# 1601339895/Image-Restoration

Measured on AMD Instinct MI355X. Metric: Mpixels/sec train (Restormer base 256x256, bs 32/GPU), higher is better.
Workload: dtype bf16; 1 GPU; Restormer base (dim 48, blocks [4,6,6,8], 26.13M params) train step: fwd + L1 + bwd + AdamW, 256x256 patches, bs 32/GPU, bf16 activations, fp32 params/grads/optimizer; per_gpu_batch=32, global_batch=32, patch=256, parallelism=dp1, hip_graph=False

## Files before the change

### image_restoration_amd/_lib.py

```python
from __future__ import annotations

import ctypes as C
import os
from typing import Optional

HERE = os.path.dirname(os.path.abspath(__file__))
LIB_PATH = os.environ.get("MI_RESTORE_LIB") or os.path.join(HERE, "libmi_restore.so")

MI_F32, MI_BF16 = 0, 1
MI_SSIM_TILE = 32
c_i64 = C.c_int64
vp = C.c_void_p
fp = C.c_void_p


class PwDesc(C.Structure):
    _fields_ = [("x1", vp), ("x1_bs", c_i64), ("x1_gs", c_i64), ("k1", C.c_int),
                ("x2", vp), ("x2_bs", c_i64), ("x2_gs", c_i64), ("k2", C.c_int),
                ("w", fp), ("w_bs", c_i64), ("w_gs", c_i64), ("w_sm", c_i64), ("w_sk", c_i64),
                ("bias", fp), ("bias_gs", c_i64),
                ("r", vp), ("r_bs", c_i64), ("r_gs", c_i64),
                ("y", vp), ("y_bs", c_i64), ("y_gs", c_i64),
                ("m", C.c_int), ("n", c_i64), ("batch", C.c_int), ("groups", C.c_int), ("dtype", C.c_int),
                ("ln_w", fp), ("ln_b", fp), ("ln_mean", fp), ("ln_rstd", fp), ("ln_mode", C.c_int),
                ("f8", C.c_int), ("f8_sx", C.c_float), ("f8_sw", C.c_float),
                ("y_split", C.c_int), ("y2", vp), ("y2_bs", c_i64), ("y2_gs", c_i64),
                ("w_b16", vp), ("w_b16_sm", c_i64)]


class GramDesc(C.Structure):
    _fields_ = [("a", vp), ("a_bs", c_i64), ("a_gs", c_i64), ("ma", C.c_int),
                ("b", vp), ("b_bs", c_i64), ("b_gs", c_i64), ("mb", C.c_int),
                ("n", c_i64), ("batch", C.c_int), ("groups", C.c_int), ("dtype", C.c_int),
                ("sum_batch", C.c_int), ("accumulate", C.c_int),
                ("out", fp), ("out_ld", c_i64), ("out_zs", c_i64), ("sumsq", fp)]


class MdtaShape(C.Structure):
    _fields_ = [("B", C.c_int), ("C", C.c_int), ("heads", C.c_int), ("H", C.c_int), ("W", C.c_int),
                ("dtype", C.c_int), ("ks", C.c_int)]


class MdtaParams(C.Structure):
    _fields_ = [("temperature", fp), ("qkv_w", fp), ("qkv_b", fp), ("dw_w", fp), ("dw_b", fp),
                ("proj_w", fp), ("proj_b", fp)]


class MdtaGrads(C.Structure):
    _fields_ = [("temperature", fp), ("qkv_w", fp), ("qkv_b", fp), ("dw_w", fp), ("dw_b", fp),
                ("proj_w", fp), ("proj_b", fp), ("accumulate", C.c_int)]


class XmdtaShape(C.Structure):
    _fields_ = [("B", C.c_int), ("C", C.c_int), ("heads", C.c_int), ("H", C.c_int), ("W", C.c_int),
                ("dtype", C.c_int), ("ks_q", C.c_int), ("ks_kv", C.c_int)]


class XmdtaParams(C.Structure):
    _fields_ = [(n, fp) for n in ("temperature", "q_w", "q_b", "q_dw_w", "q_dw_b", "kv_w", "kv_b", "kv_dw_w", "kv_dw_b",
                                  "proj_w", "proj_b")]


class XmdtaGrads(C.Structure):
    _fields_ = [(n, fp) for n in ("temperature", "q_w", "q_b", "q_dw_w", "q_dw_b", "kv_w", "kv_b", "kv_dw_w", "kv_dw_b",
                                  "proj_w", "proj_b")] + [("accumulate", C.c_int)]


class GdfnShape(C.Structure):
    _fields_ = [("B", C.c_int), ("C", C.c_int), ("hidden", C.c_int), ("H", C.c_int), ("W", C.c_int),
                ("dtype", C.c_int), ("ks", C.c_int), ("flags", C.c_int)]


class GdfnParams(C.Structure):
    _fields_ = [("in_w", fp), ("in_b", fp), ("dw_w", fp), ("dw_b", fp), ("out_w", fp), ("out_b", fp)]


class GdfnFusedShape(C.Structure):
    _fields_ = [("B", C.c_int), ("C", C.c_int), ("hidden", C.c_int), ("H", C.c_int), ("W", C.c_int),
                ("ln_with_bias", C.c_int)]


class LnHead(C.Structure):
    _fields_ = [("w", fp), ("b", fp), ("mean", fp), ("rstd", fp), ("with_bias", C.c_int)]


class F8Scales(C.Structure):
    _fields_ = [("x1", C.c_float), ("w1", C.c_float), ("x2", C.c_float), ("w2", C.c_float)]


class LnTail(C.Structure):
    _fields_ = [("w", fp), ("b", fp), ("mean", fp), ("rstd", fp), ("dres", vp), ("dw", fp), ("db", fp)]


class GroupedProblem(C.Structure):
    _fields_ = [("x", vp), ("x_rs", c_i64), ("w", fp), ("w_sm", c_i64), ("w_sk", c_i64), ("bias", fp), ("r", vp), ("r_rs", c_i64),
                ("y", vp), ("y_rs", c_i64), ("m", C.c_int), ("k", C.c_int), ("expert", C.c_int), ("x_local", C.c_int),
                ("y_local", C.c_int), ("r_local", C.c_int)]


class GdfnGrads(C.Structure):
    _fields_ = [("in_w", fp), ("in_b", fp), ("dw_w", fp), ("dw_b", fp), ("out_w", fp), ("out_b", fp),
                ("accumulate", C.c_int)]


class TksaShape(C.Structure):
    _fields_ = [("B", C.c_int), ("C", C.c_int), ("heads", C.c_int), ("H", C.c_int), ("W", C.c_int), ("dtype", C.c_int),
                ("k1", C.c_int), ("k2", C.c_int), ("k3", C.c_int), ("k4", C.c_int)]


class TksaParams(C.Structure):
    _fields_ = [(n, fp) for n in ("attn1", "attn2", "attn3", "attn4")]


class TksaGrads(C.Structure):
    _fields_ = [(n, fp) for n in ("attn1", "attn2", "attn3", "attn4")]


MSFN_PARAM_NAMES = ("in_w", "in_b", "dw3_w", "dw3_b", "dw5_w", "dw5_b", "g3_w", "g3_b", "g5_w", "g5_b", "out_w", "out_b")


class MsfnShape(C.Structure):
    _fields_ = [("B", C.c_int), ("C", C.c_int), ("hidden", C.c_int), ("H", C.c_int), ("W", C.c_int), ("dtype", C.c_int)]


class MsfnParams(C.Structure):
    _fields_ = [(n, fp) for n in MSFN_PARAM_NAMES]


class MsfnGrads(C.Structure):
    _fields_ = [(n, fp) for n in MSFN_PARAM_NAMES] + [("accumulate", C.c_int)]


class MefcShape(C.Structure):
    _fields_ = [("B", C.c_int), ("C", C.c_int), ("H", C.c_int), ("W", C.c_int), ("dtype", C.c_int), ("steps", C.c_int)]


MEFC_STEP_FIELDS = (("sep_dw1", 4), ("sep_pw1", 4), ("sep_dw2", 4), ("sep_pw2", 4), ("dil_dw", 3), ("dil_pw", 3), ("out_w", 1))


class MefcStepParams(C.Structure):
    _fields_ = [(n, fp * k) if k > 1 else (n, fp) for n, k in MEFC_STEP_FIELDS]


class MefcStepGrads(C.Structure):
    _fields_ = [(n, fp * k) if k > 1 else (n, fp) for n, k in MEFC_STEP_FIELDS]


class MefcParams(C.Structure):
    _fields_ = [(n, fp) for n in ("fc1_w", "fc1_b", "fc2_w", "fc2_b", "pre_w")] + [("step", C.POINTER(MefcStepParams))]


class MefcGrads(C.Structure):
    _fields_ = [(n, fp) for n in ("fc1_w", "fc1_b", "fc2_w", "fc2_b", "pre_w")] + [("step", C.POINTER(MefcStepGrads)),
                                                                                     ("accumulate", C.c_int)]


class DilgateParams(C.Structure):
    _fields_ = [("w", fp * 4), ("b", fp * 4)]


class DilgateGrads(C.Structure):
    _fields_ = [("w", fp * 4), ("b", fp * 4), ("accumulate", C.c_int)]


class DblockShape(C.Structure):
    _fields_ = [("B", C.c_int), ("C", C.c_int), ("H", C.c_int), ("W", C.c_int), ("dtype", C.c_int), ("n_dil", C.c_int),
                ("dil", C.c_int * 4), ("extra", C.c_int)]


DBLOCK_FIELDS = (("norm1_w", 1), ("norm1_b", 1), ("conv1_w", 1), ("conv1_b", 1), ("extra_w", 1), ("extra_b", 1), ("br_w", 4), ("br_b", 4),
                 ("sca_w", 1), ("sca_b", 1), ("conv3_w", 1), ("conv3_b", 1), ("beta", 1), ("norm2_w", 1), ("norm2_b", 1),
                 ("conv4_w", 1), ("conv4_b", 1), ("conv5_w", 1), ("conv5_b", 1), ("gamma", 1))


class DblockParams(C.Structure):
    _fields_ = [(n, fp * k) if k > 1 else (n, fp) for n, k in DBLOCK_FIELDS]


class DblockGrads(C.Structure):
    _fields_ = [(n, fp * k) if k > 1 else (n, fp) for n, k in DBLOCK_FIELDS] + [("accumulate", C.c_int)]


class FremlpShape(C.Structure):
    _fields_ = [("B", C.c_int), ("nc", C.c_int), ("expand", C.c_int), ("H", C.c_int), ("W", C.c_int), ("dtype", C.c_int)]


class FourierUnitShape(C.Structure):
    _fields_ = [("B", C.c_int), ("c", C.c_int), ("groups", C.c_int), ("H", C.c_int), ("W", C.c_int), ("dtype", C.c_int),
                ("training", C.c_int), ("eps", C.c_float), ("momentum", C.c_float)]


FOURIER_UNIT_FIELDS = ("bn_w", "bn_b", "fdc_w", "fdc_b", "gate_w", "gate_b", "fpe_w", "fpe_b")


class FourierUnitParams(C.Structure):
    _fields_ = [(n, fp) for n in FOURIER_UNIT_FIELDS]


class FourierUnitGrads(C.Structure):
    _fields_ = [(n, fp) for n in FOURIER_UNIT_FIELDS] + [("accumulate", C.c_int)]


class SfhFfnShape(C.Structure):
    _fields_ = [("B", C.c_int), ("dim", C.c_int), ("H", C.c_int), ("W", C.c_int), ("dtype", C.c_int)]


SFH_FFN_FIELDS = ("init_w", "init_b", "c1_w", "c1_b", "c2_w", "c2_b", "c3_w", "c3_b", "fina_w", "fina_b")
SFH_LOCAL_FIELDS = ("cd1_w", "cd1_b", "cd2_w", "cd2_b")


class SfhFfnParams(C.Structure):
    _fields_ = [(n, fp) for n in SFH_FFN_FIELDS]


class SfhFfnGrads(C.Structure):
    _fields_ = [(n, fp) for n in SFH_FFN_FIELDS] + [("accumulate", C.c_int)]


class SfhLocalShape(C.Structure):
    _fields_ = SfhFfnShape._fields_


class SfhLocalParams(C.Structure):
    _fields_ = [(n, fp) for n in SFH_LOCAL_FIELDS]


class SfhLocalGrads(C.Structure):
    _fields_ = [(n, fp) for n in SFH_LOCAL_FIELDS] + [("accumulate", C.c_int)]


class SfhMixerShape(C.Structure):
    _fields_ = [("B", C.c_int), ("dim", C.c_int), ("H", C.c_int), ("W", C.c_int), ("dtype", C.c_int), ("training", C.c_int),
                ("eps", C.c_float), ("momentum", C.c_float)]


SFH_GLOBAL_FIELDS = ("init_w", "init_b", "fina_w", "fina_b") + FOURIER_UNIT_FIELDS
SFH_MIXER_FIELDS = SFH_LOCAL_FIELDS + SFH_GLOBAL_FIELDS + ("cac_w", "cac_b", "ca1_w", "ca1_b", "ca2_w", "ca2_b", "conv_w", "conv_b")


class SfhGlobalParams(C.Structure):
    _fields_ = [(n, fp) for n in SFH_GLOBAL_FIELDS]


class SfhGlobalGrads(C.Structure):
    _fields_ = [(n, fp) for n in SFH_GLOBAL_FIELDS] + [("accumulate", C.c_int)]


class SfhMixerParams(C.Structure):
    _fields_ = [(n, fp) for n in SFH_MIXER_FIELDS]


class SfhMixerGrads(C.Structure):
    _fields_ = [(n, fp) for n in SFH_MIXER_FIELDS] + [("accumulate", C.c_int)]


class Bn2dShape(C.Structure):
    _fields_ = [("B", C.c_int), ("C", C.c_int), ("H", C.c_int), ("W", C.c_int), ("dtype", C.c_int), ("training", C.c_int),
                ("eps", C.c_float), ("momentum", C.c_float)]


class EblockShape(C.Structure):
    _fields_ = DblockShape._fields_


EBLOCK_FIELDS = (("norm1_w", 1), ("norm1_b", 1), ("extra_w", 1), ("extra_b", 1), ("conv1_w", 1), ("conv1_b", 1), ("br_w", 4), ("br_b", 4),
                 ("sca_w", 1), ("sca_b", 1), ("conv3_w", 1), ("conv3_b", 1), ("beta", 1), ("norm2_w", 1), ("norm2_b", 1),
                 ("fre_w1", 1), ("fre_b1", 1), ("fre_w2", 1), ("fre_b2", 1), ("gamma", 1))


class EblockParams(C.Structure):
    _fields_ = [(n, fp * k) if k > 1 else (n, fp) for n, k in EBLOCK_FIELDS]


class EblockGrads(C.Structure):
    _fields_ = [(n, fp * k) if k > 1 else (n, fp) for n, k in EBLOCK_FIELDS] + [("accumulate", C.c_int)]


SIGNATURES = {
    "mi_version": (C.c_int, []),
    "mi_last_error": (C.c_char_p, []),
    "mi_env_reload": (C.c_int, []),
    "mi_deferred_begin": (C.c_int, [vp, C.c_size_t]),
    "mi_deferred_record": (C.c_int, [C.c_int]),
    "mi_deferred_pending": (C.c_int, []),
    "mi_deferred_high_water": (C.c_size_t, []),
    "mi_deferred_flush": (C.c_int, [vp]),
    "mi_deferred_end": (C.c_int, []),
    "mi_ln_fwd": (C.c_int, [vp, fp, fp, vp, fp, fp, C.c_int, C.c_int, c_i64, C.c_int, C.c_int, vp]),
    "mi_ln_fwd_eps": (C.c_int, [vp, fp, fp, vp, fp, fp, C.c_int, C.c_int, c_i64, C.c_int, C.c_float, C.c_int, vp]),
    "mi_ln_bwd_workspace": (C.c_size_t, [C.c_int, C.c_int, c_i64]),
    "mi_ln_bwd": (C.c_int, [vp, vp, fp, fp, fp, vp, vp, fp, fp, C.c_int, C.c_int, c_i64, C.c_int, C.c_int, C.c_int,
                            vp, vp]),
    "mi_ln_plan": (C.c_int, [C.c_int, C.c_int, c_i64, C.c_int, C.c_int, C.c_int, C.POINTER(C.c_int)]),
    "mi_dwconv_fwd": (C.c_int, [vp, fp, fp, vp, C.c_int, C.c_int, C.c_int, C.c_int, C.c_int, C.c_int, vp]),
    "mi_dwconv_gate_fwd": (C.c_int, [vp, fp, fp, vp, vp, C.c_int, C.c_int, C.c_int, C.c_int, C.c_int, C.c_int, vp]),
    "mi_dwconv_bwd_workspace": (C.c_size_t, [C.c_int, C.c_int, C.c_int, C.c_int, C.c_int]),
    "mi_dwconv_bwd": (C.c_int, [vp, vp, fp, vp, fp, fp, C.c_int, C.c_int, C.c_int, C.c_int, C.c_int, C.c_int, C.c_int,
                                vp, vp]),
    "mi_dwconv_gate_bwd": (C.c_int, [vp, vp, vp, fp, vp, fp, fp, C.c_int, C.c_int, C.c_int, C.c_int, C.c_int, C.c_int,
                                     C.c_int, vp, vp]),
    "mi_dwconv_gate_recompute_ok": (C.c_int, [C.c_int, C.c_int, C.c_int]),
    "mi_dwconv_plan": (C.c_int, [C.c_int, C.c_int, C.c_int, C.c_int, C.c_int, C.c_int, C.POINTER(C.c_int)]),
    "mi_dwconv_gate_bwd_recompute": (C.c_int, [vp, vp, fp, fp, vp, fp, fp, C.c_int, C.c_int, C.c_int, C.c_int, C.c_int,
                                               C.c_int, C.c_int, vp, vp]),
    "mi_pw_gemm_workspace": (C.c_size_t, [C.POINTER(PwDesc)]),
    "mi_pw_gemm": (C.c_int, [C.POINTER(PwDesc), vp, vp]),
    "mi_pw_cache_enable": (C.c_int, [vp, C.c_size_t, vp, vp]),
    "mi_pw_cache_refresh": (C.c_int, [vp]),
    "mi_pw_cache_invalidate": (C.c_int, []),
    "mi_pw_cache_pending": (C.c_int, []),
    "mi_gram_workspace": (C.c_size_t, [C.POINTER(GramDesc)]),
    "mi_gram": (C.c_int, [C.POINTER(GramDesc), vp, vp]),
    "mi_gram_plan": (C.c_int, [C.POINTER(GramDesc), C.POINTER(c_i64)]),
    "mi_mdta_saved_bytes": (C.c_size_t, [C.POINTER(MdtaShape)]),
    "mi_mdta_workspace": (C.c_size_t, [C.POINTER(MdtaShape)]),
    "mi_mdta_fwd": (C.c_int, [C.POINTER(MdtaShape), C.POINTER(MdtaParams), vp, vp, vp, vp, vp, vp]),
    "mi_mdta_bwd": (C.c_int, [C.POINTER(MdtaShape), C.POINTER(MdtaParams), vp, vp, vp, C.POINTER(MdtaGrads), vp, vp,
                              vp]),
    "mi_xmdta_saved_bytes": (C.c_size_t, [C.POINTER(XmdtaShape)]),
    "mi_xmdta_workspace": (C.c_size_t, [C.POINTER(XmdtaShape)]),
    "mi_xmdta_fwd": (C.c_int, [C.POINTER(XmdtaShape), C.POINTER(XmdtaParams), vp, vp, vp, vp, vp, vp, vp]),
    "mi_xmdta_bwd": (C.c_int, [C.POINTER(XmdtaShape), C.POINTER(XmdtaParams), vp, vp, vp, vp, vp, C.POINTER(XmdtaGrads), vp,
                               vp, vp]),
    "mi_gdfn_saved_bytes": (C.c_size_t, [C.POINTER(GdfnShape)]),
    "mi_gdfn_workspace": (C.c_size_t, [C.POINTER(GdfnShape)]),
    "mi_pw_gemm_ln_ok": (C.c_int, [C.POINTER(PwDesc)]),
    "mi_mdta_fwd_ln_ok": (C.c_int, [C.POINTER(MdtaShape)]),
    "mi_mdta_fwd_ln": (C.c_int, [C.POINTER(MdtaShape), C.POINTER(MdtaParams), C.POINTER(LnHead), vp, vp, vp, vp, vp, vp]),
    "mi_gdfn_fwd_ln_ok": (C.c_int, [C.POINTER(GdfnShape)]),
    "mi_gdfn_fwd_ln": (C.c_int, [C.POINTER(GdfnShape), C.POINTER(GdfnParams), C.POINTER(LnHead), vp, vp, vp, vp, vp, vp]),
    "mi_pw_gemm_f8_ok": (C.c_int, [C.POINTER(PwDesc)]),
    "mi_pw_gemm_split_ok": (C.c_int, [C.POINTER(PwDesc)]),
    "mi_pw_plan": (C.c_int, [C.POINTER(PwDesc), C.POINTER(c_i64)]),
    "mi_mdta_fwd_f8_ok": (C.c_int, [C.POINTER(MdtaShape), C.c_int]),
    "mi_mdta_fwd_f8": (C.c_int, [C.POINTER(MdtaShape), C.POINTER(MdtaParams), C.POINTER(LnHead), C.POINTER(F8Scales), vp, vp, vp,
                                 vp, vp]),
    "mi_gdfn_fwd_f8_ok": (C.c_int, [C.POINTER(GdfnShape), C.c_int]),
    "mi_gdfn_fwd_f8": (C.c_int, [C.POINTER(GdfnShape), C.POINTER(GdfnParams), C.POINTER(LnHead), C.POINTER(F8Scales), vp, vp, vp,
                                 vp, vp]),
    "mi_box_down": (C.c_int, [vp, vp, C.c_int, C.c_int, C.c_int, C.c_int, C.c_int, C.c_int, vp]),
    "mi_fre_rect": (C.c_int, [fp, fp, fp, vp, C.c_int, C.c_int, C.c_int, C.c_int, C.c_int, C.c_int, vp]),
    "mi_fre_split_coef_bytes": (C.c_size_t, [C.c_int, C.c_int]),
    "mi_fre_split_workspace": (C.c_size_t, [C.c_int, C.c_int, C.c_int, C.c_int]),
    "mi_fre_split_max_hw": (C.c_int, []),
    "mi_fre_split_fwd": (C.c_int, [vp, vp, vp, vp, fp, C.c_int, C.c_int, C.c_int, C.c_int, C.c_int, vp]),
    "mi_fre_split_bwd": (C.c_int, [vp, vp, fp, vp, vp, vp, C.c_int, C.c_int, C.c_int, C.c_int, C.c_int, vp, vp]),
    "mi_chan_maxmean_fwd": (C.c_int, [vp, vp, vp, C.c_int, C.c_int, c_i64, C.c_int, vp]),
    "mi_chan_maxmean_bwd": (C.c_int, [vp, vp, vp, C.c_int, C.c_int, c_i64, C.c_int, vp]),
    "mi_plane_max_fwd": (C.c_int, [vp, fp, vp, C.c_int, c_i64, C.c_int, vp]),
    "mi_pool_pair_bwd": (C.c_int, [fp, fp, vp, vp, C.c_int, c_i64, C.c_int, vp]),
    "mi_chan_gate_fwd": (C.c_int, [fp, fp, fp, fp, fp, fp, C.c_int, C.c_int, C.c_int, vp]),
    "mi_chan_gate_bwd": (C.c_int, [fp, fp, fp, fp, fp, fp, fp, fp, fp, fp, fp, C.c_int, C.c_int, C.c_int, C.c_int, vp]),
    "mi_refine_mix_fwd": (C.c_int, [vp, vp, vp, fp, vp, C.c_int, C.c_int, c_i64, C.c_int, vp]),
    "mi_refine_mix_bwd": (C.c_int, [vp, vp, vp, fp, vp, vp, vp, vp, fp, C.c_int, C.c_int, c_i64, C.c_int, vp]),
    "mi_scale_add_fwd": (C.c_int, [vp, vp, fp, fp, vp, C.c_int, C.c_int, c_i64, C.c_int, vp]),
    "mi_scale_add_bwd": (C.c_int, [vp, vp, fp, fp, vp, vp, vp, fp, fp, C.c_int, C.c_int, c_i64, C.c_int, C.c_int, vp]),
    "mi_bwd_tail_ok": (C.c_int, [C.c_int, C.c_int, c_i64, C.c_int]),
    "mi_bwd_tail_workspace": (C.c_size_t, [C.c_int, C.c_int]),
    "mi_bwd_tail_plan": (C.c_int, [C.c_int, C.c_int, C.c_int, c_i64, C.c_int, C.POINTER(c_i64)]),
    "mi_bwd_tail": (C.c_int, [vp, C.c_int, vp, C.c_int, vp, fp, fp, fp, fp, fp, vp, fp, fp, fp, C.c_int, c_i64, C.c_int,
                              C.c_int, vp, vp]),
    "mi_mdta_bwd_ln_ok": (C.c_int, [C.POINTER(MdtaShape), C.c_int]),
    "mi_mdta_bwd_ln_workspace": (C.c_size_t, [C.POINTER(MdtaShape)]),
    "mi_mdta_bwd_ln": (C.c_int, [C.POINTER(MdtaShape), C.POINTER(MdtaParams), C.POINTER(LnTail), vp, vp, vp,
                                 C.POINTER(MdtaGrads), vp, vp, vp]),
    "mi_gdfn_bwd_ln_ok": (C.c_int, [C.POINTER(GdfnShape), C.c_int]),
    "mi_gdfn_bwd_ln_workspace": (C.c_size_t, [C.POINTER(GdfnShape)]),
    "mi_gdfn_bwd_ln": (C.c_int, [C.POINTER(GdfnShape), C.POINTER(GdfnParams), C.POINTER(LnTail), vp, vp, vp,
                                 C.POINTER(GdfnGrads), vp, vp, vp]),
    "mi_gdfn_fwd": (C.c_int, [C.POINTER(GdfnShape), C.POINTER(GdfnParams), vp, vp, vp, vp, vp, vp]),
    "mi_gdfn_bwd": (C.c_int, [C.POINTER(GdfnShape), C.POINTER(GdfnParams), vp, vp, vp, C.POINTER(GdfnGrads), vp, vp,
                              vp]),
    "mi_tksa_saved_bytes": (C.c_size_t, [C.POINTER(TksaShape)]),
    "mi_tksa_workspace": (C.c_size_t, [C.POINTER(TksaShape)]),
    "mi_tksa_fwd": (C.c_int, [C.POINTER(TksaShape), C.POINTER(MdtaParams), C.POINTER(TksaParams), vp, vp, vp, vp, vp, fp, vp]),
    "mi_tksa_bwd": (C.c_int, [C.POINTER(TksaShape), C.POINTER(MdtaParams), C.POINTER(TksaParams), vp, vp, vp, C.POINTER(MdtaGrads),
                              C.POINTER(TksaGrads), vp, vp, vp]),
    "mi_msfn_saved_bytes": (C.c_size_t, [C.POINTER(MsfnShape)]),
    "mi_msfn_workspace": (C.c_size_t, [C.POINTER(MsfnShape)]),
    "mi_msfn_fwd": (C.c_int, [C.POINTER(MsfnShape), C.POINTER(MsfnParams), vp, vp, vp, vp, vp, vp]),
    "mi_msfn_bwd": (C.c_int, [C.POINTER(MsfnShape), C.POINTER(MsfnParams), vp, vp, vp, C.POINTER(MsfnGrads), vp, vp, vp]),
    "mi_mefc_saved_bytes": (C.c_size_t, [C.POINTER(MefcShape)]),
    "mi_mefc_workspace": (C.c_size_t, [C.POINTER(MefcShape)]),
    "mi_mefc_fwd": (C.c_int, [C.POINTER(MefcShape), C.POINTER(MefcParams), vp, vp, vp, vp, vp]),
    "mi_mefc_bwd": (C.c_int, [C.POINTER(MefcShape), C.POINTER(MefcParams), vp, vp, vp, vp, C.POINTER(MefcGrads), vp, vp, vp]),
    "mi_dilgate_plan": (C.c_int, [C.c_int, C.c_int, C.c_int, C.c_int, C.c_int, C.c_int, C.POINTER(C.c_int), C.POINTER(c_i64)]),
    "mi_dilgate_fwd_workspace": (C.c_size_t, [C.c_int, C.c_int, C.c_int, C.c_int]),
    "mi_dilgate_fwd": (C.c_int, [vp, C.POINTER(DilgateParams), vp, fp, C.c_int, C.c_int, C.c_int, C.c_int, C.c_int, C.POINTER(C.c_int),
                                 C.c_int, vp, vp]),
    "mi_dilgate_bwd_workspace": (C.c_size_t, [C.c_int, C.c_int, C.c_int, C.c_int, C.c_int, C.c_int]),
    "mi_dilgate_bwd": (C.c_int, [vp, fp, vp, C.POINTER(DilgateParams), vp, C.POINTER(DilgateGrads), C.c_int, C.c_int, C.c_int, C.c_int,
                                 C.c_int, C.POINTER(C.c_int), C.c_int, vp, vp]),
    "mi_pairconv3x3_fwd": (C.c_int, [vp, fp, fp, vp, C.c_int, C.c_int, C.c_int, C.c_int, C.c_int, vp]),
    "mi_pairconv3x3_bwd_workspace": (C.c_size_t, [C.c_int, C.c_int, C.c_int, C.c_int]),
    "mi_pairconv3x3_bwd": (C.c_int, [vp, vp, fp, vp, fp, fp, C.c_int, C.c_int, C.c_int, C.c_int, C.c_int, C.c_int, vp, vp]),
    "mi_dblock_saved_bytes": (C.c_size_t, [C.POINTER(DblockShape)]),
    "mi_dblock_workspace": (C.c_size_t, [C.POINTER(DblockShape)]),
    "mi_dblock_fwd": (C.c_int, [C.POINTER(DblockShape), C.POINTER(DblockParams), vp, vp, vp, vp, vp]),
    "mi_dblock_bwd": (C.c_int, [C.POINTER(DblockShape), C.POINTER(DblockParams), vp, vp, vp, C.POINTER(DblockGrads), vp, vp, vp]),
    "mi_gdfn_fused_ok": (C.c_int, [C.POINTER(GdfnFusedShape)]),
    "mi_gdfn_fused_pack_bytes": (C.c_size_t, [C.POINTER(GdfnFusedShape)]),
    "mi_gdfn_fused_pack": (C.c_int, [C.POINTER(GdfnFusedShape), fp, fp, C.POINTER(GdfnParams), vp, vp]),
    "mi_gdfn_fused_fwd": (C.c_int, [C.POINTER(GdfnFusedShape), vp, vp, vp, fp, fp, vp]),
    "mi_gdfn_fused_fwd_train_ok": (C.c_int, [C.POINTER(GdfnFusedShape)]),
    "mi_gdfn_fused_fwd_train": (C.c_int, [C.POINTER(GdfnFusedShape), vp, vp, vp, fp, fp, vp, vp]),
    "mi_gdfn_fused_fwd_f8": (C.c_int, [C.POINTER(GdfnFusedShape), vp, C.POINTER(F8Scales), vp, vp, vp]),
    "mi_gdfn_fused_plan": (C.c_int, [C.POINTER(GdfnFusedShape), C.c_int, C.POINTER(c_i64)]),
    "mi_mdta_fused_ok": (C.c_int, [C.POINTER(MdtaShape)]),
    "mi_mdta_fused_pays": (C.c_int, [C.POINTER(MdtaShape)]),
    "mi_mdta_fused_pack_bytes": (C.c_size_t, [C.POINTER(MdtaShape)]),
    "mi_mdta_fused_pack": (C.c_int, [C.POINTER(MdtaShape), fp, fp, C.POINTER(MdtaParams), vp, vp]),
    "mi_mdta_fused_workspace": (C.c_size_t, [C.POINTER(MdtaShape)]),
    "mi_mdta_fused_plan": (C.c_int, [C.POINTER(MdtaShape), C.POINTER(c_i64)]),
    "mi_mdta_fused_fwd": (C.c_int, [C.POINTER(MdtaShape), C.POINTER(MdtaParams), vp, C.c_int, vp, vp, vp, fp, fp, vp, vp]),
    "mi_adamw_step": (C.c_int, [fp, fp, fp, fp, c_i64, C.c_float, C.c_float, C.c_float, C.c_float, C.c_float, C.c_int,
                                C.c_float, fp, vp]),
    "mi_grad_sumsq_workspace": (C.c_size_t, [c_i64]),
    "mi_grad_sumsq": (C.c_int, [fp, c_i64, fp, vp, vp]),
    "mi_adamw_step_ex": (C.c_int, [fp, fp, fp, fp, fp, c_i64, C.c_float, C.c_float, C.c_float, C.c_float, C.c_float, C.c_int,
                                   C.c_float, fp, fp, C.c_float, fp, C.c_float, vp]),
    "mi_rows_gather": (C.c_int, [vp, vp, vp, C.c_int, c_i64, C.c_int, vp]),
    "mi_rows_gather_scaled": (C.c_int, [fp, vp, fp, vp, C.c_int, c_i64, C.c_int, vp]),
    "mi_rows_scatter_add": (C.c_int, [vp, vp, fp, vp, C.c_int, C.c_int, c_i64, C.c_int, C.c_int, vp]),
    "mi_rows_dot_workspace": (C.c_size_t, [C.c_int, c_i64]),
    "mi_rows_dot": (C.c_int, [fp, vp, vp, fp, C.c_int, c_i64, C.c_int, vp, vp]),
    "mi_glue3x3_ok": (C.c_int, [C.c_int, C.c_int]),
    "mi_conv3x3_ok": (C.c_int, [C.c_int, C.c_int, C.c_int]),
    "mi_conv3x3_pack_bytes": (C.c_size_t, [C.c_int, C.c_int]),
    "mi_conv3x3_pack": (C.c_int, [fp, C.c_int, C.c_int, C.c_int, vp, vp]),
    "mi_conv3x3_fwd": (C.c_int, [vp, vp, C.c_int64, fp, vp, C.c_int64, vp, C.c_int64, C.c_int, C.c_int, C.c_int, C.c_int, C.c_int, vp]),
    "mi_conv3x3_wgrad_workspace": (C.c_size_t, [C.c_int, C.c_int, C.c_int, C.c_int, C.c_int]),
    "mi_conv3x3_wgrad": (C.c_int, [vp, C.c_int64, vp, C.c_int64, fp, C.c_int, C.c_int, C.c_int, C.c_int, C.c_int, C.c_int, vp, vp]),
    "mi_conv3x3_plan": (C.c_int, [C.c_int, C.c_int, C.c_int, C.c_int, C.c_int, C.POINTER(c_i64)]),
    "mi_chan_sum_workspace": (C.c_size_t, [C.c_int, C.c_int64]),
    "mi_chan_sum": (C.c_int, [vp, fp, C.c_int, C.c_int, C.c_int64, C.c_int, C.c_int, vp, vp]),
    "mi_chan_sum_plan": (C.c_int, [C.c_int, C.c_int, C.c_int64, C.c_int, C.c_int, C.POINTER(c_i64)]),
    "mi_attn_small_plan": (C.c_int, [C.c_int, C.c_int, C.c_int, C.POINTER(c_i64)]),
    "mi_attn_small_fwd": (C.c_int, [fp, fp, fp, fp, fp, fp, fp, fp, vp, vp, C.c_int, C.c_int, C.c_int, vp]),
    "mi_attn_small_bwd": (C.c_int, [fp, fp, fp, fp, fp, fp, fp, fp, fp, vp, C.c_int, C.c_int, C.c_int, vp]),
    "mi_im2col3x3": (C.c_int, [vp, vp, C.c_int, C.c_int, C.c_int, C.c_int, C.c_int, C.c_int, vp]),
    "mi_col2im3x3": (C.c_int, [vp, fp, vp, vp, C.c_int, C.c_int, C.c_int, C.c_int, C.c_int, C.c_int, vp]),
    "mi_glue3x3_plan": (C.c_int, [c_i64, C.c_int, C.c_int, C.c_int, C.c_int, C.POINTER(c_i64)]),
    "mi_grouped_pw_gemm": (C.c_int, [C.POINTER(GroupedProblem), C.c_int, vp, vp, C.c_int, c_i64, C.c_int, vp]),
    "mi_moe_route_fwd": (C.c_int, [fp, fp, fp, fp, fp, fp, fp, fp, vp, fp, fp, vp, vp, vp, fp, vp, vp, C.c_int, C.c_int, C.c_int,
                                   C.c_int, C.c_int, C.c_int, vp]),
    "mi_moe_route_bwd": (C.c_int, [fp, fp, fp, fp, fp, fp, fp, vp, fp, fp, vp, fp, fp, fp, fp, fp, C.c_int, C.c_int, C.c_int,
                                   C.c_int, C.c_int, C.c_int, vp]),
    "mi_patch_circconv": (C.c_int, [vp, c_i64, vp, c_i64, vp, c_i64, C.c_int, C.c_int, C.c_int, C.c_int, C.c_int, C.c_int, C.c_int, vp]),
    "mi_gelu_gap_fwd": (C.c_int, [vp, fp, C.c_int, C.c_int, c_i64, C.c_int, vp]),
    "mi_gelu_gap_bwd": (C.c_int, [vp, fp, vp, C.c_int, C.c_int, c_i64, C.c_int, vp]),
    "mi_ewise_fwd": (C.c_int, [vp, c_i64, vp, c_i64, vp, c_i64, c_i64, C.c_int, C.c_int, vp]),
    "mi_ewise_bwd": (C.c_int, [vp, c_i64, vp, c_i64, vp, vp, c_i64, vp, c_i64, c_i64, c_i64, C.c_int, C.c_int, vp]),
    "mi_pixel_shuffle2": (C.c_int, [vp, c_i64, vp, c_i64, C.c_int, C.c_int, C.c_int, C.c_int, C.c_int, C.c_int, vp]),
    "mi_copy_rows": (C.c_int, [vp, c_i64, vp, c_i64, c_i64, c_i64, C.c_int, vp]),
    "mi_pixel_shuffle2_plan": (C.c_int, [C.c_int, C.c_int, C.c_int, C.c_int, c_i64, c_i64, C.c_int, C.c_int, C.POINTER(c_i64)]),
    "mi_copy_rows_plan": (C.c_int, [c_i64, c_i64, c_i64, c_i64, C.c_int, C.c_int, C.POINTER(c_i64)]),
    "mi_patch_batch": (C.c_int, [vp, vp, vp, vp, vp, vp, vp, vp, fp, fp, vp, vp, C.c_int, C.c_int, C.c_int, vp]),
    "mi_psnr_ssim_workspace": (C.c_size_t, [C.c_int, C.c_int, C.c_int, C.c_int]),
    "mi_psnr_ssim": (C.c_int, [vp, vp, fp, fp, C.c_int, C.c_int, C.c_int, C.c_int, C.c_int, vp, vp]),
    "mi_gap_fwd": (C.c_int, [vp, fp, C.c_int, C.c_int, c_i64, C.c_int, vp]),
    "mi_gap_bwd": (C.c_int, [fp, vp, C.c_int, C.c_int, c_i64, C.c_int, vp]),
    "mi_cast": (C.c_int, [vp, C.c_int, vp, C.c_int, c_i64, vp]),
    "mi_l1_loss": (C.c_int, [vp, vp, vp, fp, c_i64, C.c_float, C.c_int, vp]),
    "mi_fft_l1_workspace": (C.c_size_t, [C.c_int, C.c_int, C.c_int, C.c_int]),
    "mi_fft_l1_plan": (C.c_int, [C.c_int, C.c_int, C.c_int, C.c_int, C.c_int, C.c_int, C.POINTER(c_i64)]),
    "mi_fft_l1_loss": (C.c_int, [vp, vp, vp, fp, C.c_int, C.c_int, C.c_int, C.c_int, C.c_float, C.c_int, vp, vp]),
# ... 85 lines not shown
```

### image_restoration_amd/csrc/common.h

```cpp
#pragma once
#include <hip/hip_runtime.h>
#include <stdint.h>
#include <stdio.h>
#include <string.h>
#include <type_traits>

#include "../../include/mi_restore.h"

namespace mi {

typedef __bf16 bf16;
typedef unsigned short u16;
typedef __attribute__((ext_vector_type(2))) float f32x2;
typedef __attribute__((ext_vector_type(4))) float f32x4;
typedef __attribute__((ext_vector_type(2))) unsigned int u32x2;
typedef __attribute__((ext_vector_type(4))) unsigned int u32x4;
typedef __attribute__((ext_vector_type(4))) short s16x4;
typedef __attribute__((ext_vector_type(8))) short s16x8;

template <bool F8> struct MfmaOp;
template <> struct MfmaOp<false> {
  using Frag = s16x8;
  static __device__ __forceinline__ void enter() {}
  static __device__ __forceinline__ Frag cvt(const s16x8 v, float) { return v; }
  static __device__ __forceinline__ f32x4 mma(Frag a, Frag b, f32x4 c) { return __builtin_amdgcn_mfma_f32_16x16x32_bf16(a, b, c, 0, 0, 0); }
};
template <> struct MfmaOp<true> {
  using Frag = long;
  typedef short s16x2_t __attribute__((ext_vector_type(2)));
  typedef __bf16 bf16x2_t __attribute__((ext_vector_type(2)));
  static __device__ __forceinline__ void enter() { __builtin_amdgcn_s_setreg((0 << 11) | (23 << 6) | 1, 1); }
  static __device__ __forceinline__ Frag cvt(const s16x8 v, float scale) {
    s16x2_t lo = {0, 0}, hi = {0, 0};
    lo = __builtin_amdgcn_cvt_scalef32_pk_fp8_bf16(lo, __builtin_bit_cast(bf16x2_t, (s16x2_t){v[0], v[1]}), scale, false);
    lo = __builtin_amdgcn_cvt_scalef32_pk_fp8_bf16(lo, __builtin_bit_cast(bf16x2_t, (s16x2_t){v[2], v[3]}), scale, true);
    hi = __builtin_amdgcn_cvt_scalef32_pk_fp8_bf16(hi, __builtin_bit_cast(bf16x2_t, (s16x2_t){v[4], v[5]}), scale, false);
    hi = __builtin_amdgcn_cvt_scalef32_pk_fp8_bf16(hi, __builtin_bit_cast(bf16x2_t, (s16x2_t){v[6], v[7]}), scale, true);
    return (long)(unsigned long)(unsigned)__builtin_bit_cast(int, lo) | ((long)__builtin_bit_cast(int, hi) << 32);
  }
  static __device__ __forceinline__ f32x4 mma(Frag a, Frag b, f32x4 c) { return __builtin_amdgcn_mfma_f32_16x16x32_fp8_fp8(a, b, c, 0, 0, 0); }
};

#define MI_ENV_LIST(X)                                                                                                       \
  X(MI_BT_WIDE) X(MI_BT_DEBUG) X(MI_DW_LDS) X(MI_FG_CFG) X(MI_FG_DEBUG) X(MI_FG_NOXCD) X(MI_GRAM_FOLD) X(MI_GRAM_WANT)      \
  X(MI_GRAM_RECT) X(MI_GRAM_LDS) X(MI_GRAM_STREAM_ALL) X(MI_LN_FORM) X(MI_CO_STREAM) X(MI_ATTN_DQK_SPLIT)    \
  X(MI_PW_DMA) X(MI_PW_TM_EVEN) X(MI_PW_WAVE) X(MI_PW_CHUNKED) X(MI_PW_XWIDE) X(MI_PW_WAVE_WIDE) X(MI_PW_DIRECT)             \
  X(MI_PW_WAVE_TPW) X(MI_PW_XCD) X(MI_PW_TPB) X(MI_PW_B16) X(MI_FM_DEBUG) X(MI_FM_CFG) X(MI_NO_FUSED_MDTA) X(MI_NO_PW_LDS) X(MI_PW_LDS)
enum EnvId {
#define MI_ENV_ENUM(n) E_##n,
  MI_ENV_LIST(MI_ENV_ENUM)
#undef MI_ENV_ENUM
  E_ENV_COUNT
};
const char* env_get(int id);
#define MI_ENV(n) ::mi::env_get(::mi::E_##n)

void set_error(const char* fmt, ...);
#define MI_CHECK_ARG(cond, ...)                \
  do {                                         \
    if (!(cond)) {                             \
      mi::set_error(__VA_ARGS__);              \
      return MI_ERR_ARG;                       \
    }                                          \
  } while (0)
#define MI_CHECK_HIP(expr)                                                          \
  do {                                                                              \
    hipError_t e_ = (expr);                                                         \
    if (e_ != hipSuccess) {                                                         \
      mi::set_error("%s failed: %s (%s:%d)", #expr, hipGetErrorString(e_), __FILE__, __LINE__); \
      return MI_ERR_HIP;                                                            \
    }                                                                               \
  } while (0)
#define MI_LAUNCH_CHECK() MI_CHECK_HIP(hipGetLastError())
#define MI_TRY(expr)          \
  do {                        \
    int rc_ = (expr);         \
    if (rc_ != MI_OK) return rc_; \
  } while (0)

static inline bool aligned16(const void* p) { return (reinterpret_cast<uintptr_t>(p) & 15u) == 0; }
static inline size_t align_up(size_t v, size_t a) { return (v + a - 1) / a * a; }
static inline int cdiv(int64_t a, int64_t b) { return (int)((a + b - 1) / b); }
static inline int cdiv_cap(int64_t a, int64_t b, int cap) { const int64_t n = (a + b - 1) / b; return n < cap ? (int)n : cap; }
static inline size_t dtype_size(int dt) { return dt == MI_BF16 ? 2 : 4; }

template <typename T, typename F> static inline int call_typed(F& f) {
  if constexpr (std::is_void<decltype(f(T{}))>::value) {
    f(T{});
    MI_LAUNCH_CHECK();
    return MI_OK;
  } else {
    return f(T{});
  }
}
template <typename F> static inline int with_dtype(int dtype, const char* who, F&& f) {
  if (dtype == MI_F32) return call_typed<float>(f);
  if (dtype == MI_BF16) return call_typed<bf16>(f);
  set_error("%s: bad dtype %d", who, dtype);
  return MI_ERR_ARG;
}

struct Carver {
  char* base;
  size_t off;
  explicit Carver(void* p) : base(static_cast<char*>(p)), off(0) {}
  template <typename U = void>
  U* take(size_t bytes) {
    size_t o = off;
    off = align_up(off + bytes, 256);
    return base ? reinterpret_cast<U*>(base + o) : nullptr;
  }
};

#if defined(__HIPCC__)

__device__ __forceinline__ float to_f32(float v) { return v; }
__device__ __forceinline__ float to_f32(bf16 v) { return (float)v; }
__device__ __forceinline__ float bf16_bits_to_f32(unsigned int bits16) { return __uint_as_float(bits16 << 16); }

template <typename T> struct Cvt;
template <> struct Cvt<float> {
  static __device__ __forceinline__ float from(float v) { return v; }
};
template <> struct Cvt<bf16> {
  static __device__ __forceinline__ bf16 from(float v) { return (bf16)v; }
};

__device__ __forceinline__ unsigned int cvt_pk_bf16(float a, float b) {
  typedef __bf16 bf16x2_t __attribute__((ext_vector_type(2)));
  const f32x2 v = {a, b};
  return __builtin_bit_cast(unsigned int, __builtin_convertvector(v, bf16x2_t));
}
template <typename T> __device__ __forceinline__ float ld1(const T* p) { return to_f32(*p); }
template <typename T> __device__ __forceinline__ void st1(T* p, float v) { *p = Cvt<T>::from(v); }

#ifndef MI_NT_ST
#define MI_NT_ST 1
#endif
#if MI_NT_ST
#define MI_STREAM_ST(ptr, val) __builtin_nontemporal_store((val), (ptr))
#else
#define MI_STREAM_ST(ptr, val) (*(ptr) = (val))
#endif
#ifndef MI_NT_LD
#define MI_NT_LD 1
#endif
#if MI_NT_LD
#define MI_STREAM_LD(ptr) __builtin_nontemporal_load(ptr)
#define MI_STREAM_DMA_AUX 2
#else
#define MI_STREAM_LD(ptr) (*(ptr))
#define MI_STREAM_DMA_AUX 0
#endif

template <typename T, int V> struct Vec;
template <> struct Vec<float, 1> {
  static __device__ __forceinline__ void ld(const float* p, float* o) { o[0] = p[0]; }
  static __device__ __forceinline__ void st(float* p, const float* v) { p[0] = v[0]; }
};
template <> struct Vec<float, 2> {
  static __device__ __forceinline__ void ld(const float* p, float* o) {
    f32x2 t = *reinterpret_cast<const f32x2*>(p); o[0] = t[0]; o[1] = t[1];
  }
  static __device__ __forceinline__ void st(float* p, const float* v) {
    f32x2 t = {v[0], v[1]}; *reinterpret_cast<f32x2*>(p) = t;
  }
};
template <> struct Vec<float, 4> {
  static __device__ __forceinline__ void ld(const float* p, float* o) {
    f32x4 t = MI_STREAM_LD(reinterpret_cast<const f32x4*>(p)); o[0] = t[0]; o[1] = t[1]; o[2] = t[2]; o[3] = t[3];
  }
  static __device__ __forceinline__ void st(float* p, const float* v) {
    f32x4 t = {v[0], v[1], v[2], v[3]}; MI_STREAM_ST(reinterpret_cast<f32x4*>(p), t);
  }
};
template <> struct Vec<bf16, 1> {
  static __device__ __forceinline__ void ld(const bf16* p, float* o) { o[0] = (float)p[0]; }
  static __device__ __forceinline__ void st(bf16* p, const float* v) { p[0] = (bf16)v[0]; }
};
template <> struct Vec<bf16, 2> {
  static __device__ __forceinline__ void ld(const bf16* p, float* o) {
    unsigned int t = *reinterpret_cast<const unsigned int*>(p);
    o[0] = bf16_bits_to_f32(t & 0xffffu); o[1] = bf16_bits_to_f32(t >> 16);
  }
  static __device__ __forceinline__ void st(bf16* p, const float* v) { *reinterpret_cast<unsigned int*>(p) = cvt_pk_bf16(v[0], v[1]); }
};
template <> struct Vec<bf16, 4> {
  static __device__ __forceinline__ void ld(const bf16* p, float* o) {
    u32x2 t = MI_STREAM_LD(reinterpret_cast<const u32x2*>(p));
    o[0] = bf16_bits_to_f32(t[0] & 0xffffu); o[1] = bf16_bits_to_f32(t[0] >> 16);
    o[2] = bf16_bits_to_f32(t[1] & 0xffffu); o[3] = bf16_bits_to_f32(t[1] >> 16);
  }
  static __device__ __forceinline__ void st(bf16* p, const float* v) {
    u32x2 t;
#pragma unroll
    for (int i = 0; i < 2; ++i) t[i] = cvt_pk_bf16(v[2 * i], v[2 * i + 1]);
    MI_STREAM_ST(reinterpret_cast<u32x2*>(p), t);
  }
};
template <> struct Vec<bf16, 8> {
  static __device__ __forceinline__ void ld(const bf16* p, float* o) {
    u32x4 t = MI_STREAM_LD(reinterpret_cast<const u32x4*>(p));
#pragma unroll
    for (int i = 0; i < 4; ++i) { o[2 * i] = bf16_bits_to_f32(t[i] & 0xffffu); o[2 * i + 1] = bf16_bits_to_f32(t[i] >> 16); }
  }
  static __device__ __forceinline__ void st(bf16* p, const float* v) {
    u32x4 t;
#pragma unroll
    for (int i = 0; i < 4; ++i) t[i] = cvt_pk_bf16(v[2 * i], v[2 * i + 1]);
    MI_STREAM_ST(reinterpret_cast<u32x4*>(p), t);
  }
};

__device__ __forceinline__ float wave_sum(float v) {
#define MI_DPP_ADD(ctrl, rmask)                                                                                   \
  v += __builtin_bit_cast(float, __builtin_amdgcn_update_dpp(0, __builtin_bit_cast(int, v), ctrl, rmask, 0xf, false))
  MI_DPP_ADD(0x111, 0xf);
  MI_DPP_ADD(0x112, 0xf);
  MI_DPP_ADD(0x114, 0xf);
  MI_DPP_ADD(0x118, 0xf);
  MI_DPP_ADD(0x142, 0xa);
  MI_DPP_ADD(0x143, 0xc);
#undef MI_DPP_ADD
  return __builtin_bit_cast(float, __builtin_amdgcn_readlane(__builtin_bit_cast(int, v), 63));
}
__device__ __forceinline__ float wave_max(float v) {
#define MI_DPP_MAX(ctrl, rmask)                                                                                    \
  v = fmaxf(v, __builtin_bit_cast(float, __builtin_amdgcn_update_dpp(__builtin_bit_cast(int, v), __builtin_bit_cast(int, v), \
                                                                     ctrl, rmask, 0xf, false)))
  MI_DPP_MAX(0x111, 0xf);
  MI_DPP_MAX(0x112, 0xf);
  MI_DPP_MAX(0x114, 0xf);
  MI_DPP_MAX(0x118, 0xf);
  MI_DPP_MAX(0x142, 0xa);
  MI_DPP_MAX(0x143, 0xc);
#undef MI_DPP_MAX
  return __builtin_bit_cast(float, __builtin_amdgcn_readlane(__builtin_bit_cast(int, v), 63));
}

#define MI_ROW16_STEP(OP, ctrl)                                                                                    \
  v = OP(v, __builtin_bit_cast(float, __builtin_amdgcn_update_dpp(__builtin_bit_cast(int, v), __builtin_bit_cast(int, v), \
                                                                  ctrl, 0xf, 0xf, true)))
__device__ __forceinline__ float row16_sum(float v) {
#define MI_ADDF(a, b) ((a) + (b))
  MI_ROW16_STEP(MI_ADDF, 0xB1); MI_ROW16_STEP(MI_ADDF, 0x4E); MI_ROW16_STEP(MI_ADDF, 0x141); MI_ROW16_STEP(MI_ADDF, 0x140);
#undef MI_ADDF
  return v;
}
__device__ __forceinline__ float row16_max(float v) {
  MI_ROW16_STEP(fmaxf, 0xB1); MI_ROW16_STEP(fmaxf, 0x4E); MI_ROW16_STEP(fmaxf, 0x141); MI_ROW16_STEP(fmaxf, 0x140);
  return v;
}
#undef MI_ROW16_STEP

__device__ __forceinline__ void gelu_parts(float x, float& cdf, float& pdf) {
  const float z = fabsf(x) * 0.70710678118654752440f;
  const float t = __builtin_amdgcn_rcpf(1.0f + 0.3275911f * z);
  const float e = __expf(-z * z);
  const float poly = t * (0.254829592f + t * (-0.284496736f + t * (1.421413741f + t * (-1.453152027f + t * 1.061405429f))));
  const float q = 0.5f * poly * e;
  cdf = x >= 0.f ? 1.0f - q : q;
  pdf = 0.39894228040143267794f * e;
}
__device__ __forceinline__ void gelu_parts2(f32x2 x, f32x2& cdf, f32x2& pdf) {
#pragma clang fp contract(off)
  const f32x2 ax = {fabsf(x[0]), fabsf(x[1])};
  const f32x2 z = ax * 0.70710678118654752440f;
  const f32x2 den = __builtin_elementwise_fma(z, (f32x2){0.3275911f, 0.3275911f}, (f32x2){1.0f, 1.0f});
  const f32x2 t = {__builtin_amdgcn_rcpf(den[0]), __builtin_amdgcn_rcpf(den[1])};
  const f32x2 a = (z * -z) * 1.44269504088896340736f;
  const f32x2 e = {__builtin_amdgcn_exp2f(a[0]), __builtin_amdgcn_exp2f(a[1])};
  f32x2 p = __builtin_elementwise_fma(t, (f32x2){1.061405429f, 1.061405429f}, (f32x2){-1.453152027f, -1.453152027f});
  p = __builtin_elementwise_fma(t, p, (f32x2){1.421413741f, 1.421413741f});
  p = __builtin_elementwise_fma(t, p, (f32x2){-0.284496736f, -0.284496736f});
  p = __builtin_elementwise_fma(t, p, (f32x2){0.254829592f, 0.254829592f});
  const f32x2 hp = (t * p) * 0.5f;
  const f32x2 q = hp * e;
  const f32x2 omq = __builtin_elementwise_fma(-e, hp, (f32x2){1.0f, 1.0f});
  cdf[0] = x[0] >= 0.f ? omq[0] : q[0];
  cdf[1] = x[1] >= 0.f ? omq[1] : q[1];
  pdf = e * 0.39894228040143267794f;
}
__device__ __forceinline__ float gelu_erf(float x) {
  float cdf, pdf;
  gelu_parts(x, cdf, pdf);
  return x * cdf;
}
template <typename T> __device__ __forceinline__ float gelu_fwd(float x) { return gelu_erf(x); }
#ifndef MI_GELU_EXACT
template <> __device__ __forceinline__ float gelu_fwd<bf16>(float x) {
  const float u = x * (-2.3083120f - 0.1004116f * x * x);
  return x * __builtin_amdgcn_rcpf(1.0f + __builtin_amdgcn_exp2f(u));
}
#endif
__device__ __forceinline__ float gelu_erf_grad(float x) {
  float cdf, pdf;
  gelu_parts(x, cdf, pdf);
  return cdf + x * pdf;
}

#endif

enum KernelId {
  K_LN_FWD = 0, K_LN_BWD, K_DW_FWD, K_DW_GATE_FWD, K_DW_BWD_DATA, K_DW_GATE_BWD_DATA, K_DW_WGRAD, K_PW_GEMM, K_GRAM,
  K_GRAM_REDUCE, K_ATTN_FOLD, K_ATTN_BWD_SMALL, K_REDUCE_ROWS, K_CHAN_SUM, K_ADAMW, K_CAST, K_L1, K_PW_PACK, K_GAP,
  K_IM2COL, K_COL2IM, K_GDFN_FUSED_FWD, K_GDFN_FUSED_BWD, K_MDTA_FUSED_A, K_FUSED_PACK, K_MOE_ROUTE, K_CIRCCONV, K_EWISE, K_CONV3X3, K_GRAM_QK, K_PW_AV, K_BWD_TAIL, K_BWD_TAIL_FIN, K_ADAIR, K_SUMSQ, K_ADAMW_CLIP, K_ADAMW_EMA,
  K_TKSA_ATTN, K_TKSA_FOLD, K_TKSA_BWD, K_TKSA_DWO, K_MSFN_S1, K_MSFN_S2, K_MSFN_S1_BWD, K_MSFN_S2_BWD,
  K_MEFC_STA, K_MEFC_STB, K_MEFC_STA_BWD, K_MEFC_STB_BWD, K_MEFC_WGRAD, K_MEFC_FOLD, K_MEFC_FOLD_BWD, K_MEFC_HEAD, K_MEFC_HEAD_BWD,
  K_MEFC_EW, K_DK_GATE_FWD, K_DK_GATE_BWD_DZ, K_DK_GATE_BWD_DX, K_DK_PAIR, K_DK_PAIR_WGRAD, K_DK_FOLD, K_DK_FOLD_BWD, K_COUNT
};
struct ProfScope {
  hipStream_t st; int kid; bool on;
  ProfScope(hipStream_t stream, int kernel_id, double bytes, double flops);
  ~ProfScope();
};

float* deferred_take(size_t nfloats, hipStream_t st);
bool deferred_owns(const void* p);
bool deferred_reduce_rows(const float* part, float* out, int64_t rows, int64_t cols, int64_t part_ld, int accumulate, float scale,
                          float* out2 = nullptr, int64_t split = 0);

constexpr int REDUCE_GROUPS = 32;
static inline bool reduce_rows_two_stage(int64_t rows) { return rows > 4 * REDUCE_GROUPS; }
int launch_reduce_rows(const float* part, float* out, int64_t rows, int64_t cols, int64_t part_ld,
                       int accumulate, float scale, hipStream_t st, float* tmp = nullptr, float* out2 = nullptr,
                       int64_t split = 0);

}
```

### image_restoration_amd/csrc/internal.h

```cpp
#pragma once
#include <initializer_list>

#include "common.h"

namespace mi {
struct PwK {
  const void* x1; int64_t x1_bs, x1_gs; int k1;
  const void* x2; int64_t x2_bs, x2_gs; int k2;
  const float* w; int64_t w_bs, w_gs, w_sm, w_sk;
  const float* bias; int64_t bias_gs;
  const void* r; int64_t r_bs, r_gs;
  void* y; int64_t y_bs, y_gs;
  int m; int64_t n; int groups; int vec_ok;
  void* y2; int64_t y2_bs, y2_gs; int y_split;
};
enum PwFamily { PW_CHUNKED = 0, PW_RESIDENT, PW_DMA, PW_XRES, PW_STREAM, PW_XWIDE, PW_LDS };
enum PwWeights { PW_W_PACK = 0, PW_W_B16, PW_W_F32 };
struct PwPlan {
  int family;
  int tm, m_tiles, k_chunks;
  bool f8, ln;
  bool vec_ok;
  int slices, per_batch, per_group, chunk_elems;
  int64_t slice_elems;
  size_t bytes;
  size_t lds_image;
  dim3 grid, block; size_t lds;
  int tpw, tpb, n_slabs, slabs_per, xcd_map;
  int weights;
  bool cacheable;
  size_t ws_bytes() const { return family == PW_LDS ? align_up(lds_image, 256) : bytes; }
};
enum GramFamily { GRAM_LDS = 0, GRAM_STREAM };
enum GramFinish { GRAM_DIRECT = 0, GRAM_REDUCE_FEW4, GRAM_REDUCE_FEW16, GRAM_REDUCE };
struct GramPlan {
  int family;
  int fa, fb; bool ss;
  int unit, units, per_split;
  int splits, tiles_a, tiles_b, Z, fold;
  bool vec_ok;
  dim3 grid, block;
  size_t part_bytes, ss_bytes;
  int finish;
  bool deferrable;
  int images, total, zo;
  size_t ws_bytes() const { return part_bytes + ss_bytes; }
};
template <typename... P, typename... A>
static inline int launch_dyn_lds(void (*kernel)(P...), dim3 grid, dim3 block, size_t lds, hipStream_t st, A... args) {
  if (lds > 64 * 1024) MI_CHECK_HIP(hipFuncSetAttribute((const void*)kernel, hipFuncAttributeMaxDynamicSharedMemorySize, (int)lds));
  hipLaunchKernelGGL(kernel, grid, block, lds, st, args...);
  MI_LAUNCH_CHECK();
  return MI_OK;
}
int launch_attn_fold(const float* graw, const float* ss, const float* temperature, const float* wo, float* P, float* A,
                     float* nrm, float* M, int B, int C, int heads, hipStream_t st, void* Mb = nullptr, void* Mtb = nullptr);
int launch_attn_bwd_small(const float* dM, const float* A, const float* P, const float* nrm, const float* temperature,
                          const float* wo, float* dwo_part, float* dtemp_part, float* wd, float* scratch,
                          int B, int C, int heads, hipStream_t st, void* wdb = nullptr);
size_t attn_bwd_scratch_floats(int B, int C, int heads);
struct TopkArgs { const float* w[4]; int k[4]; };
int tksa_check(int C, int heads, const int* k);
int launch_tksa_fold(const float* graw, const float* ss, const float* temperature, const TopkArgs& tk, const float* wo, float* P,
                     float* S, float* A, float* nrm, float* M, float* scores, int B, int C, int heads, hipStream_t st, void* Mb,
                     void* Mtb);
int launch_tksa_bwd(const float* dM, const float* A, const float* S, const float* P, const float* nrm, const float* temperature,
                    const TopkArgs& tk, const float* wo, float* dwo_part, float* dtemp_part, float* dattn_part, float* wd, int B,
                    int C, int heads, hipStream_t st, void* wdb);
int msfn_splits(int H, int W);
size_t msfn_part_floats(int B, int hd, int H, int W);
int launch_msfn_s1_fwd(const void* h0, const float* w3, const float* b3, const float* w5, const float* b5, void* a, void* b, int B,
                       int hd, int H, int W, int dtype, hipStream_t st);
int launch_msfn_s2_fwd(const void* a, const void* b, const float* g3w, const float* g3b, const float* g5w, const float* g5b, void* y,
                       int B, int hd, int H, int W, int dtype, hipStream_t st);
int launch_msfn_s2_bwd(const void* dY, const void* y, const void* a, const void* b, const float* g3w, const float* g5w, void* dza,
                       void* dzb, float* g_g3w, float* g_g3b, float* g_g5w, float* g_g5b, int accumulate, float* part, int B, int hd,
                       int H, int W, int dtype, hipStream_t st);
int launch_msfn_s1_bwd(const void* dza, const void* dzb, const void* h0, const float* w3, const float* w5, void* dh0, float* g_w3,
                       float* g_b3, float* g_w5, float* g_b5, int accumulate, float* part, int B, int hd, int H, int W, int dtype,
                       hipStream_t st);
size_t chan_sum_workspace(int C, int64_t N);
int launch_chan_sum(const void* x, float* out, int B, int C, int64_t N, int dtype, int accumulate, void* ws, hipStream_t st);
#if defined(__HIPCC__)
template <int NV>
__device__ __forceinline__ float block_sum4(const float (&v)[NV], float* red) {
  const int wv = threadIdx.x >> 6, lane = threadIdx.x & 63;
#pragma unroll
  for (int n = 0; n < NV; ++n) {
    const float s = wave_sum(v[n]);
    if (lane == 0) red[wv * NV + n] = s;
  }
  __syncthreads();
  const int n = threadIdx.x;
  return n < NV ? (red[n] + red[NV + n]) + (red[2 * NV + n] + red[3 * NV + n]) : 0.f;
}
#endif

enum { IN_PLAIN = 0, IN_GATE_BWD = 1 };
struct DwArgs {
  const void* in;
  const void* gy;
  const float* w;
  const float* bias;
  void* out;
  void* gate;
  int Cc, H, W, hidden, tiles_x;
};
bool dws_eligible(int H, int W, int ks);
int dws_partial_rows(int B, int H, int W, int64_t planes);
void dws_plan(int H, int W, int64_t planes, int* band, int* nb, int* lpr, int* uni);
int dws_fwd(const DwArgs& a, int B, bool gate, bool flip, int dtype, hipStream_t st);
int dws_bwd(const DwArgs& dya, const void* xin, float* part, int B, bool want_dx, int* rows_out, int dtype, hipStream_t st);
int dws_gate_bwd(const DwArgs& a, const void* xin, float* part, int B, bool want_dw, int* rows_out, int dtype,
                 hipStream_t st);
int dws_gate_bwd_recompute(const DwArgs& a, float* part, int B, bool want_dw, int* rows_out, int dtype, hipStream_t st);
struct BtPlan {
  bool covered, pays;
  int C, NW, MPW, rows, mpad;
  int grid, launch;
  int64_t tiles_per_image, tiles;
  int passes, active;
  size_t lds, ws_bytes;
};
BtPlan bwd_tail_plan(int M, int C, int B, int64_t N, int dtype);
bool bwd_tail_ok(int M, int C, int64_t N, int dtype);
bool bwd_tail_pays(int M, int C);
size_t bwd_tail_workspace(int M, int C);
int launch_bwd_tail(const void* dy, int M, const void* x, int C, const void* dres, const float* mean, const float* rstd,
                    const float* w, const float* gamma, const float* beta, void* dx, float* dw, float* dgamma, float* dbeta,
                    int B, int64_t N, int accumulate, void* ws, hipStream_t st);
#define MI_HIDDEN __attribute__((visibility("hidden")))
MI_HIDDEN int pw_lds_tm(int M);
MI_HIDDEN size_t pw_lds_lds_bytes(int tm);
MI_HIDDEN int pw_lds_launch(const mi_pw_desc* d, const PwPlan& pl, void* ws, hipStream_t st);
int fused_gdfn_fwd_save(const mi_gdfn_fused_shape* s, const void* pack, const void* y, void* out, float* mean, float* rstd,
                        void* h0, void* g, hipStream_t st);
enum FgEntry { FG_INFER = 0, FG_TRAIN, FG_F8 };
enum FgFamily { FG_TILE = 0, FG_FOURTH };
struct FgPlan {
  bool covered;
  int family;
  int C, th, tw, pc, nw; bool save, f8;
  int nch, ngr;
  int tiles_x, tiles_y, S;
  int64_t grid; int block; size_t lds;
  bool xcd_pairs;
  size_t pack_bytes; int pack_pc;
};
MI_HIDDEN FgPlan fg_plan(const mi_gdfn_fused_shape* s, int entry);
enum FmForm { FM_ROUND3 = 0, FM_FOURTH };
struct FmPlan {
  bool covered, pays;
  int kind, form;
  int C, heads, th, nw;
  int tiles_x, tiles_y, S;
  int64_t grid; int block; size_t lds;
  int part_mult;
  size_t part_bytes, ws_bytes, pack_bytes;
};
MI_HIDDEN FmPlan fm_plan(const mi_mdta_shape* s);

static inline size_t fbytes(size_t n) { return align_up(n * sizeof(float), 256); }
static inline size_t tbytes(size_t n, int dt) { return align_up(n * dtype_size(dt), 256); }
static inline size_t max_of(std::initializer_list<size_t> v) {
  size_t m = 0;
  for (size_t x : v) m = x > m ? x : m;
  return m;
}
static inline mi_pw_desc conv1x1(const void* x, int K, const float* w, bool transposed, int w_ld, const float* bias,
                                 const void* res, void* y, int M, int B, int64_t N, int dtype, int64_t x_bs = 0, int64_t y_bs = 0) {
  mi_pw_desc d;
  memset(&d, 0, sizeof(d));
  d.x1 = x; d.x1_bs = x_bs ? x_bs : (int64_t)K * N; d.k1 = K;
  d.w = w;
  if (transposed) { d.w_sm = 1; d.w_sk = w_ld; } else { d.w_sm = w_ld; d.w_sk = 1; }
  d.bias = bias;
  d.r = res; d.r_bs = (int64_t)M * N;
  d.y = y; d.y_bs = y_bs ? y_bs : (int64_t)M * N;
  d.m = M; d.n = N; d.batch = B; d.groups = 1; d.dtype = dtype;
  return d;
}
static inline mi_pw_desc per_image(mi_pw_desc d, const void* w_b16 = nullptr) {
  d.w_bs = (int64_t)d.m * d.k1;
  if (w_b16) { d.w_b16 = w_b16; d.w_b16_sm = d.k1; }
  return d;
}
static inline mi_gram_desc wgrad_gram(const void* dy, int m, const void* x, int k, int B, int64_t N, int dtype, float* out,
                                      int accumulate, int sum_batch = 1, int64_t dy_bs = 0, int64_t x_bs = 0) {
  mi_gram_desc g;
  memset(&g, 0, sizeof(g));
  g.a = dy; g.a_bs = dy_bs ? dy_bs : (int64_t)m * N; g.ma = m;
  g.b = x; g.b_bs = x_bs ? x_bs : (int64_t)k * N; g.mb = k;
  g.n = N; g.batch = B; g.groups = 1; g.dtype = dtype;
  g.sum_batch = sum_batch; g.accumulate = accumulate; g.out = out; g.out_ld = k; g.out_zs = sum_batch ? 0 : (int64_t)m * k;
  return g;
}
static void* const PROBE_PTR = (void*)256;
static inline mi_pw_desc probe1x1(int K, int M, bool transposed, int B, int64_t N, int dtype, int64_t x_bs = 0, int64_t y_bs = 0) {
  return conv1x1(PROBE_PTR, K, (const float*)PROBE_PTR, transposed, transposed ? M : K, nullptr, nullptr, PROBE_PTR, M, B, N, dtype,
                 x_bs, y_bs);
}
static inline mi_gram_desc probe_wgrad(int m, int k, int B, int64_t N, int dtype, int sum_batch = 1, int64_t dy_bs = 0,
                                       int64_t x_bs = 0) {
  return wgrad_gram(PROBE_PTR, m, PROBE_PTR, k, B, N, dtype, (float*)PROBE_PTR, 0, sum_batch, dy_bs, x_bs);
}
static inline size_t pw_ws_bytes(const mi_pw_desc& d) { return mi_pw_gemm_workspace(&d); }
static inline size_t gram_ws_bytes(const mi_gram_desc& d) { return mi_gram_workspace(&d); }
__attribute__((visibility("hidden")))
int conv1x1_bwd_input(const void* dy, int M, const void* x, int K, const float* w, float* dw, float* db, void* dx, int B, int64_t N,
                      int dtype, int accumulate, void* gram_ws, void* cs_ws, void* pw_ws, hipStream_t st, bool fork);
}
```

### image_restoration_amd/csrc/modules.hip

```cpp
#include <stdlib.h>

#include "internal.h"

namespace mi {

struct CoStream {
  hipStream_t side = nullptr;
  hipEvent_t fork = nullptr, join = nullptr;
};
static bool co_stream_enabled() {
  const char* e = MI_ENV(MI_CO_STREAM);
  return e && atoi(e) == 1;
}
static CoStream* co_stream() {
  static thread_local CoStream cs[16];
  int dev = 0;
  if (hipGetDevice(&dev) != hipSuccess || dev < 0 || dev >= 16) return nullptr;
  CoStream& c = cs[dev];
  if (!c.side) {
    if (hipStreamCreateWithFlags(&c.side, hipStreamNonBlocking) != hipSuccess) return nullptr;
    if (hipEventCreateWithFlags(&c.fork, hipEventDisableTiming) != hipSuccess) return nullptr;
    if (hipEventCreateWithFlags(&c.join, hipEventDisableTiming) != hipSuccess) return nullptr;
  }
  return &c;
}
static hipStream_t co_fork(hipStream_t st) {
  if (!co_stream_enabled()) return st;
  CoStream* c = co_stream();
  if (!c) return st;
  if (hipEventRecord(c->fork, st) != hipSuccess || hipStreamWaitEvent(c->side, c->fork, 0) != hipSuccess) return st;
  return c->side;
}
static int co_join(hipStream_t side, hipStream_t st) {
  if (side == st) return MI_OK;
  CoStream* c = co_stream();
  MI_CHECK_ARG(c != nullptr, "co_join: side stream lost");
  MI_CHECK_HIP(hipEventRecord(c->join, side));
  MI_CHECK_HIP(hipStreamWaitEvent(st, c->join, 0));
  return MI_OK;
}
int conv1x1_bwd_input(const void* dy, int M, const void* x, int K, const float* w, float* dw, float* db, void* dx, int B, int64_t N,
                      int dtype, int accumulate, void* gram_ws, void* cs_ws, void* pw_ws, hipStream_t st, bool fork) {
  const mi_gram_desc g = wgrad_gram(dy, M, x, K, B, N, dtype, dw, accumulate);
  const mi_pw_desc d = conv1x1(dy, M, w, true, K, nullptr, nullptr, dx, K, B, N, dtype);
  const hipStream_t sd = fork ? co_fork(st) : st;
  int rc = mi_gram(&g, gram_ws, sd);
  if (rc == MI_OK && db) rc = launch_chan_sum(dy, db, B, M, N, dtype, accumulate, cs_ws, sd);
  if (rc == MI_OK) rc = mi_pw_gemm(&d, pw_ws, st);
  const int joined = co_join(sd, st);
  return rc != MI_OK ? rc : joined;
}
static int conv1x1_bwd_output(const void* dy, int M, const void* x, int K, const float* w, float* dw, float* db, void* dx, int B,
                              int64_t N, int dtype, int accumulate, void* gram_ws, void* cs_ws, void* pw_ws, hipStream_t st) {
  if (db) MI_TRY(launch_chan_sum(dy, db, B, M, N, dtype, accumulate, cs_ws, st));
  const mi_gram_desc g = wgrad_gram(dy, M, x, K, B, N, dtype, dw, accumulate);
  MI_TRY(mi_gram(&g, gram_ws, st));
  const mi_pw_desc d = conv1x1(dy, M, w, true, K, nullptr, nullptr, dx, K, B, N, dtype);
  return mi_pw_gemm(&d, pw_ws, st);
}

struct QkvView { const void* q; int64_t q_bs; const void* k; int64_t k_bs; const void* v; int64_t v_bs; };
struct AttnDims { int B, C, heads, dtype; int64_t N; };
struct AttnSaved { float* A; float* P; float* nrm; float* M; void* Mb; void* Mtb; };
struct AttnScratch {
  float* graw; float* ss; float* dM; float* dwo_part; float* dtemp_part; float* wd; float* attn_scr; void* wdb;
  void* gram_ws; void* pw_ws; void* cs_ws;
};

static void attn_saved_carve(Carver& cv, const AttnDims& d, AttnSaved* r) {
  const size_t C = d.C, B = d.B, c = C / d.heads, Z = B * d.heads;
  r->A = cv.take<float>(fbytes(Z * c * c));
  r->P = cv.take<float>(fbytes(Z * c * c));
  r->nrm = cv.take<float>(fbytes(Z * 2 * c));
  r->M = cv.take<float>(fbytes(B * C * C));
  r->Mb = cv.take(B * C * C * 2);
  r->Mtb = cv.take(B * C * C * 2);
}

static mi_gram_desc attn_qk_gram(const AttnDims& d, const QkvView& v, float* graw, float* ss) {
  const int c = d.C / d.heads;
  mi_gram_desc g;
  memset(&g, 0, sizeof(g));
  g.a = v.q; g.a_bs = v.q_bs; g.a_gs = (int64_t)c * d.N; g.ma = c;
  g.b = v.k; g.b_bs = v.k_bs; g.b_gs = (int64_t)c * d.N; g.mb = c;
  g.n = d.N; g.batch = d.B; g.groups = d.heads; g.dtype = d.dtype;
  g.out = graw; g.out_ld = c; g.out_zs = (int64_t)c * c; g.sumsq = ss;
  return g;
}
static mi_gram_desc attn_dm_gram(const AttnDims& d, const void* dout, const QkvView& v, float* dM) {
  mi_gram_desc g;
  memset(&g, 0, sizeof(g));
  g.a = dout; g.a_bs = (int64_t)d.C * d.N; g.ma = d.C;
  g.b = v.v; g.b_bs = v.v_bs; g.mb = d.C;
  g.n = d.N; g.batch = d.B; g.groups = 1; g.dtype = d.dtype;
  g.out = dM; g.out_ld = d.C; g.out_zs = (int64_t)d.C * d.C;
  return g;
}
static mi_pw_desc attn_dqk_desc(const AttnDims& d, const QkvView& v, const float* w, int row0, int rows, void* y, int64_t y_bs,
                                const void* wb = nullptr) {
  const int c = d.C / d.heads;
  mi_pw_desc dd;
  memset(&dd, 0, sizeof(dd));
  dd.x1 = v.k; dd.x1_bs = v.k_bs; dd.x1_gs = (int64_t)c * d.N; dd.k1 = c;
  dd.x2 = v.q; dd.x2_bs = v.q_bs; dd.x2_gs = (int64_t)c * d.N; dd.k2 = c;
  dd.w = w + (int64_t)row0 * 2 * c; dd.w_bs = (int64_t)d.heads * 2 * c * 2 * c; dd.w_gs = (int64_t)2 * c * 2 * c; dd.w_sm = 2 * c; dd.w_sk = 1;
  if (wb) { dd.w_b16 = (const char*)wb + (int64_t)row0 * 2 * c * 2; dd.w_b16_sm = 2 * c; }
  dd.y = y; dd.y_bs = y_bs; dd.y_gs = (int64_t)c * d.N;
  dd.m = rows; dd.n = d.N; dd.batch = d.B; dd.groups = d.heads; dd.dtype = d.dtype;
  return dd;
}
static mi_pw_desc attn_dqk_merged(const AttnDims& d, const QkvView& v, const float* w, void* dq, int64_t dq_bs, void* dk, int64_t dk_bs,
                                  const void* wb = nullptr) {
  const int c = d.C / d.heads;
  mi_pw_desc dd = attn_dqk_desc(d, v, w, 0, 2 * c, dq, dq_bs, wb);
  dd.y_split = c; dd.y2 = dk; dd.y2_bs = dk_bs; dd.y2_gs = (int64_t)c * d.N;
  return dd;
}

static void attn_scratch_carve(Carver& cv, const AttnDims& d, AttnScratch* w) {
  const size_t C = d.C, B = d.B, c = C / d.heads, Z = B * d.heads;
  w->graw = cv.take<float>(fbytes(Z * c * c));
  w->ss = cv.take<float>(fbytes(Z * 2 * c));
  w->dM = cv.take<float>(fbytes(B * C * C));
  w->dwo_part = cv.take<float>(fbytes(B * C * C));
  w->dtemp_part = cv.take<float>(fbytes(Z));
  w->wd = cv.take<float>(fbytes(Z * 2 * c * 2 * c));
  w->wdb = cv.take(Z * 2 * c * 2 * c * 2);
  w->attn_scr = cv.take<float>(fbytes(attn_bwd_scratch_floats((int)B, (int)C, d.heads)));
  w->gram_ws = nullptr; w->pw_ws = nullptr; w->cs_ws = nullptr;
}
static const QkvView PROBE_QKV{PROBE_PTR, 0, PROBE_PTR, 0, PROBE_PTR, 0};
static size_t attn_gram_ws_bytes(const AttnDims& d) {
  float* const p = (float*)PROBE_PTR;
  return max_of({gram_ws_bytes(attn_qk_gram(d, PROBE_QKV, p, p)), gram_ws_bytes(attn_dm_gram(d, PROBE_PTR, PROBE_QKV, p))});
}
static size_t attn_pw_ws_bytes(const AttnDims& d) {
  const float* const p = (const float*)PROBE_PTR;
  return max_of({pw_ws_bytes(per_image(probe1x1(d.C, d.C, false, d.B, d.N, d.dtype))),
                 pw_ws_bytes(attn_dqk_desc(d, PROBE_QKV, p, 0, d.C / d.heads, PROBE_PTR, 0)),
                 pw_ws_bytes(attn_dqk_merged(d, PROBE_QKV, p, PROBE_PTR, 0, PROBE_PTR, 0))});
}

struct TopkHook { TopkArgs tk; float* S; float* scores; float* dattn_part; float* g_attn[4]; };

static int attn_core_fwd(const AttnDims& d, const QkvView& v, const float* temperature, const float* proj_w,
                         const float* proj_b, const void* residual, void* out, const AttnSaved& sv, const AttnScratch& w,
                         void* stream, const mi_f8_scales* f8 = nullptr, const TopkHook* tk = nullptr) {
  hipStream_t st = (hipStream_t)stream;
  mi_gram_desc g = attn_qk_gram(d, v, w.graw, w.ss);
  MI_TRY(mi_gram(&g, w.gram_ws, stream));
  if (tk)
    MI_TRY(launch_tksa_fold(w.graw, w.ss, temperature, tk->tk, proj_w, sv.P, tk->S, sv.A, sv.nrm, sv.M, tk->scores, d.B, d.C,
                            d.heads, st, sv.Mb, sv.Mtb));
  else
    MI_TRY(launch_attn_fold(w.graw, w.ss, temperature, proj_w, sv.P, sv.A, sv.nrm, sv.M, d.B, d.C, d.heads, st, sv.Mb, sv.Mtb));
  mi_pw_desc d2 = per_image(conv1x1(v.v, d.C, sv.M, false, d.C, proj_b, residual, out, d.C, d.B, d.N, d.dtype, v.v_bs), sv.Mb);
  if (f8) { d2.f8 = 1; d2.f8_sx = f8->x2; d2.f8_sw = f8->w2; }
  return mi_pw_gemm(&d2, w.pw_ws, stream);
}

static int attn_core_bwd(const AttnDims& d, const QkvView& v, const void* dout, void* dq, int64_t dq_bs, void* dk,
                         int64_t dk_bs, void* dv, int64_t dv_bs, const AttnSaved& sv, const float* temperature,
                         const float* proj_w, float* g_temperature, float* g_proj_w, float* g_proj_b, int acc,
                         const AttnScratch& w, void* stream, const TopkHook* tk = nullptr) {
  hipStream_t st = (hipStream_t)stream;
  const int B = d.B, C = d.C, hd = d.heads;
  if (g_proj_b) MI_TRY(launch_chan_sum(dout, g_proj_b, B, C, d.N, d.dtype, acc, w.cs_ws, st));
  mi_gram_desc g1 = attn_dm_gram(d, dout, v, w.dM);
  MI_TRY(mi_gram(&g1, w.gram_ws, stream));
  float* dwo_part = w.dwo_part;
  float* dtemp_part = w.dtemp_part;
  if (acc) {
    float* a1 = deferred_take((size_t)B * C * C, st);
    float* a2 = a1 ? deferred_take((size_t)B * hd, st) : nullptr;
    if (a1 && a2) { dwo_part = a1; dtemp_part = a2; }
  }
  if (tk) {
    MI_TRY(launch_tksa_bwd(w.dM, sv.A, tk->S, sv.P, sv.nrm, temperature, tk->tk, proj_w, dwo_part, dtemp_part, tk->dattn_part, w.wd,
                           B, C, hd, st, w.wdb));
    for (int m = 0; m < 4; ++m)
      MI_TRY(launch_reduce_rows(tk->dattn_part + m, tk->g_attn[m], (int64_t)B * hd, 1, 4, acc, 1.0f, st));
  } else {
    MI_TRY(launch_attn_bwd_small(w.dM, sv.A, sv.P, sv.nrm, temperature, proj_w, dwo_part, dtemp_part, w.wd,
                                 w.attn_scr, B, C, hd, st, w.wdb));
  }
  MI_TRY(launch_reduce_rows(dwo_part, g_proj_w, B, (int64_t)C * C, (int64_t)C * C, acc, 1.0f, st));
  MI_TRY(launch_reduce_rows(dtemp_part, g_temperature, B, hd, hd, acc, 1.0f, st));
  const int c = C / hd;
  mi_pw_desc dd = attn_dqk_merged(d, v, w.wd, dq, dq_bs, dk, dk_bs, w.wdb);
  if (mi_pw_gemm_split_ok(&dd) && !MI_ENV(MI_ATTN_DQK_SPLIT)) {
    MI_TRY(mi_pw_gemm(&dd, w.pw_ws, stream));
  } else {
    dd = attn_dqk_desc(d, v, w.wd, 0, c, dq, dq_bs, w.wdb);
    MI_TRY(mi_pw_gemm(&dd, w.pw_ws, stream));
    dd = attn_dqk_desc(d, v, w.wd, c, c, dk, dk_bs, w.wdb);
    MI_TRY(mi_pw_gemm(&dd, w.pw_ws, stream));
  }
  mi_pw_desc dvd = per_image(conv1x1(dout, C, sv.M, true, C, nullptr, nullptr, dv, C, B, d.N, d.dtype, 0, dv_bs), sv.Mtb);
  return mi_pw_gemm(&dvd, w.pw_ws, stream);
}

struct MdtaSaved { void* qkv0; void* qkv; AttnSaved at; size_t bytes; };
static AttnDims mdta_dims(const mi_mdta_shape* s) { return AttnDims{s->B, s->C, s->heads, s->dtype, (int64_t)s->H * s->W}; }
static MdtaSaved mdta_saved_layout(const mi_mdta_shape* s, void* base) {
  const size_t N = (size_t)s->H * s->W, C = s->C, B = s->B;
  Carver cv(base);
  MdtaSaved r;
  r.qkv0 = cv.take(tbytes(B * 3 * C * N, s->dtype));
  r.qkv = cv.take(tbytes(B * 3 * C * N, s->dtype));
  attn_saved_carve(cv, mdta_dims(s), &r.at);
  r.bytes = cv.off;
  return r;
}
static QkvView mdta_view(const mi_mdta_shape* s, const void* qkv) {
  const int64_t N = (int64_t)s->H * s->W, bs = 3 * (int64_t)s->C * N;
  const size_t es = dtype_size(s->dtype), plane = (size_t)s->C * N * es;
  return QkvView{qkv, bs, (const char*)qkv + plane, bs, (const char*)qkv + 2 * plane, bs};
}

struct MdtaWs { AttnScratch at; MdtaSaved inf; void* dqkv; void* dqkv0; void* dw_ws; size_t bytes; };
static MdtaWs mdta_ws_layout(const mi_mdta_shape* s, void* base) {
  const size_t N = (size_t)s->H * s->W, C = s->C, B = s->B;
  const AttnDims d = mdta_dims(s);
  Carver cv(base);
  MdtaWs w;
  attn_scratch_carve(cv, d, &w.at);
  w.at.gram_ws = cv.take(max_of({attn_gram_ws_bytes(d), gram_ws_bytes(probe_wgrad(3 * d.C, d.C, d.B, d.N, d.dtype))}));
  w.at.pw_ws = cv.take(max_of({pw_ws_bytes(probe1x1(d.C, 3 * d.C, false, d.B, d.N, d.dtype)),
                               pw_ws_bytes(probe1x1(3 * d.C, d.C, true, d.B, d.N, d.dtype)), attn_pw_ws_bytes(d)}));
  w.dw_ws = cv.take(mi_dwconv_bwd_workspace((int)B, 3 * (int)C, s->H, s->W, s->ks));
  w.at.cs_ws = cv.take(chan_sum_workspace(3 * (int)C, (int64_t)N));
  size_t mark = cv.off;
  w.inf = mdta_saved_layout(s, base ? (char*)base + mark : nullptr);
  w.dqkv = base ? (char*)base + mark : nullptr;
  w.dqkv0 = base ? (char*)base + mark + tbytes(B * 3 * C * N, s->dtype) : nullptr;
  size_t bwd_big = 2 * tbytes(B * 3 * C * N, s->dtype);
  w.bytes = mark + max_of({w.inf.bytes, bwd_big});
  return w;
}

static int mdta_check(const mi_mdta_shape* s) {
  MI_CHECK_ARG(s, "mdta: null shape");
  MI_CHECK_ARG(s->B > 0 && s->C > 0 && s->heads > 0 && s->H > 0 && s->W > 0, "mdta: bad shape");
  MI_CHECK_ARG(s->C % s->heads == 0, "mdta: C=%d not divisible by heads=%d", s->C, s->heads);
  MI_CHECK_ARG(s->dtype == MI_F32 || s->dtype == MI_BF16, "mdta: bad dtype %d", s->dtype);
  MI_CHECK_ARG(s->ks == 3 || s->ks == 5 || s->ks == 7, "mdta: bad depthwise kernel size %d", s->ks);
  return MI_OK;
}

struct XmdtaSaved { void* q0; void* q; void* kv0; void* kv; AttnSaved at; size_t bytes; };
static AttnDims xmdta_dims(const mi_xmdta_shape* s) { return AttnDims{s->B, s->C, s->heads, s->dtype, (int64_t)s->H * s->W}; }
static XmdtaSaved xmdta_saved_layout(const mi_xmdta_shape* s, void* base) {
  const size_t N = (size_t)s->H * s->W, C = s->C, B = s->B;
  Carver cv(base);
  XmdtaSaved r;
  r.q0 = cv.take(tbytes(B * C * N, s->dtype));
  r.q = cv.take(tbytes(B * C * N, s->dtype));
  r.kv0 = cv.take(tbytes(B * 2 * C * N, s->dtype));
  r.kv = cv.take(tbytes(B * 2 * C * N, s->dtype));
  attn_saved_carve(cv, xmdta_dims(s), &r.at);
  r.bytes = cv.off;
  return r;
}
static QkvView xmdta_view(const mi_xmdta_shape* s, const void* q, const void* kv) {
  const int64_t N = (int64_t)s->H * s->W;
  const size_t plane = (size_t)s->C * N * dtype_size(s->dtype);
  return QkvView{q, (int64_t)s->C * N, kv, 2 * (int64_t)s->C * N, (const char*)kv + plane, 2 * (int64_t)s->C * N};
}
struct XmdtaWs { AttnScratch at; XmdtaSaved inf; void* dq; void* dq0; void* dkv; void* dkv0; void* dw_ws; size_t bytes; };
static XmdtaWs xmdta_ws_layout(const mi_xmdta_shape* s, void* base) {
  const size_t N = (size_t)s->H * s->W, C = s->C, B = s->B;
  const AttnDims d = xmdta_dims(s);
  Carver cv(base);
  XmdtaWs w;
  attn_scratch_carve(cv, d, &w.at);
  w.at.gram_ws = cv.take(max_of({attn_gram_ws_bytes(d), gram_ws_bytes(probe_wgrad(2 * d.C, d.C, d.B, d.N, d.dtype))}));
  w.at.pw_ws = cv.take(max_of({pw_ws_bytes(probe1x1(d.C, 2 * d.C, false, d.B, d.N, d.dtype)),
                               pw_ws_bytes(probe1x1(2 * d.C, d.C, true, d.B, d.N, d.dtype)), attn_pw_ws_bytes(d)}));
  const int ksm = s->ks_q > s->ks_kv ? s->ks_q : s->ks_kv;
  w.dw_ws = cv.take(mi_dwconv_bwd_workspace((int)B, 2 * (int)C, s->H, s->W, ksm));
  w.at.cs_ws = cv.take(chan_sum_workspace(2 * (int)C, (int64_t)N));
  size_t mark = cv.off;
  w.inf = xmdta_saved_layout(s, base ? (char*)base + mark : nullptr);
  Carver big(base ? (char*)base + mark : nullptr);
  w.dq = big.take(tbytes(B * C * N, s->dtype));
  w.dq0 = big.take(tbytes(B * C * N, s->dtype));
  w.dkv = big.take(tbytes(B * 2 * C * N, s->dtype));
  w.dkv0 = big.take(tbytes(B * 2 * C * N, s->dtype));
  w.bytes = mark + max_of({w.inf.bytes, big.off});
  return w;
}
static int xmdta_check(const mi_xmdta_shape* s) {
  MI_CHECK_ARG(s, "xmdta: null shape");
  MI_CHECK_ARG(s->B > 0 && s->C > 0 && s->heads > 0 && s->H > 0 && s->W > 0, "xmdta: bad shape");
  MI_CHECK_ARG(s->C % s->heads == 0, "xmdta: C=%d not divisible by heads=%d", s->C, s->heads);
  MI_CHECK_ARG(s->dtype == MI_F32 || s->dtype == MI_BF16, "xmdta: bad dtype %d", s->dtype);
  MI_CHECK_ARG((s->ks_q == 3 || s->ks_q == 5 || s->ks_q == 7) && (s->ks_kv == 3 || s->ks_kv == 5 || s->ks_kv == 7),
               "xmdta: bad depthwise kernel sizes %d/%d", s->ks_q, s->ks_kv);
  return MI_OK;
}

struct GdfnSaved { void* h0; void* h1; void* g; size_t bytes; };
static bool gdfn_recompute(const mi_gdfn_shape* s) {
  return !(s->flags & 1) && mi_dwconv_gate_recompute_ok(s->H, s->W, s->ks) != 0;
}
static GdfnSaved gdfn_saved_layout(const mi_gdfn_shape* s, void* base) {
  const size_t N = (size_t)s->H * s->W, B = s->B, h = s->hidden;
  Carver cv(base);
  GdfnSaved r;
  r.h0 = cv.take(tbytes(B * 2 * h * N, s->dtype));
  r.h1 = gdfn_recompute(s) ? nullptr : cv.take(tbytes(B * 2 * h * N, s->dtype));
  r.g = cv.take(tbytes(B * h * N, s->dtype));
  r.bytes = cv.off;
  return r;
}
struct GdfnWs { void* gram_ws; void* pw_ws; void* dw_ws; void* cs_ws; GdfnSaved inf; void* dg; void* dh0; size_t bytes; };
static GdfnWs gdfn_ws_layout(const mi_gdfn_shape* s, void* base) {
  const int B = s->B, C = s->C, h = s->hidden, dt = s->dtype;
  const int64_t N = (int64_t)s->H * s->W;
  Carver cv(base);
  GdfnWs w;
  w.gram_ws = cv.take(max_of({gram_ws_bytes(probe_wgrad(C, h, B, N, dt)), gram_ws_bytes(probe_wgrad(2 * h, C, B, N, dt))}));
  w.pw_ws = cv.take(max_of({pw_ws_bytes(probe1x1(C, 2 * h, false, B, N, dt)), pw_ws_bytes(probe1x1(2 * h, C, true, B, N, dt))}));
  w.dw_ws = cv.take(mi_dwconv_bwd_workspace(B, 2 * h, s->H, s->W, s->ks));
  w.cs_ws = cv.take(chan_sum_workspace(2 * h > C ? 2 * h : C, N));
  size_t mark = cv.off;
  w.inf = gdfn_saved_layout(s, base ? (char*)base + mark : nullptr);
  w.dg = base ? (char*)base + mark : nullptr;
  w.dh0 = base ? (char*)base + mark + tbytes((size_t)B * h * N, dt) : nullptr;
  size_t bwd_big = tbytes((size_t)B * h * N, dt) + tbytes((size_t)B * 2 * h * N, dt);
  w.bytes = mark + max_of({w.inf.bytes, bwd_big});
  return w;
}
static int gdfn_check(const mi_gdfn_shape* s) {
  MI_CHECK_ARG(s, "gdfn: null shape");
  MI_CHECK_ARG(s->B > 0 && s->C > 0 && s->hidden > 0 && s->H > 0 && s->W > 0, "gdfn: bad shape");
  MI_CHECK_ARG(s->dtype == MI_F32 || s->dtype == MI_BF16, "gdfn: bad dtype %d", s->dtype);
  MI_CHECK_ARG(s->ks == 3 || s->ks == 5 || s->ks == 7, "gdfn: bad depthwise kernel size %d", s->ks);
  return MI_OK;
}

static mi_mdta_shape tksa_mdta_shape(const mi_tksa_shape* s) { return mi_mdta_shape{s->B, s->C, s->heads, s->H, s->W, s->dtype, 3}; }
static int tksa_shape_check(const mi_tksa_shape* s) {
  MI_CHECK_ARG(s, "tksa: null shape");
  const mi_mdta_shape m = tksa_mdta_shape(s);
  MI_TRY(mdta_check(&m));
  const int k[4] = {s->k1, s->k2, s->k3, s->k4};
  return tksa_check(s->C, s->heads, k);
}
static size_t tksa_scores_bytes(const mi_mdta_shape* s) {
  const size_t c = s->C / s->heads;
  return fbytes((size_t)s->B * s->heads * c * c);
}
struct TksaWs { float* S_inf; float* dattn_part; size_t bytes; };
static TksaWs tksa_ws_tail(const mi_mdta_shape* s, size_t m_bytes, void* base) {
  Carver cv(base ? (char*)base + align_up(m_bytes, 256) : nullptr);
  TksaWs w;
  w.S_inf = cv.take<float>(tksa_scores_bytes(s));
  w.dattn_part = cv.take<float>(fbytes((size_t)s->B * s->heads * 4));
  w.bytes = align_up(m_bytes, 256) + cv.off;
  return w;
}

}

using namespace mi;

extern "C" size_t mi_mdta_saved_bytes(const mi_mdta_shape* s) {
  if (mdta_check(s) != MI_OK) return 0;
  return mdta_saved_layout(s, nullptr).bytes;
}
extern "C" size_t mi_mdta_workspace(const mi_mdta_shape* s) {
  if (mdta_check(s) != MI_OK) return 0;
  return mdta_ws_layout(s, nullptr).bytes;
}

static void ln_head_apply(mi_pw_desc* d, const mi_ln_head* ln) {
  if (!ln) return;
  d->ln_w = ln->w; d->ln_b = ln->with_bias ? ln->b : nullptr; d->ln_mean = ln->mean; d->ln_rstd = ln->rstd;
  d->ln_mode = ln->with_bias ? 1 : 2;
}
static int ln_head_check(const mi_ln_head* ln, const char* who) {
  MI_CHECK_ARG(ln && ln->w && (!ln->with_bias || ln->b) && ((ln->mean == nullptr) == (ln->rstd == nullptr)),
               "%s: LayerNorm head needs w (and b for WithBias); mean / rstd both or neither", who);
  return MI_OK;
}
static int mdta_fwd_impl(const char* who, const mi_mdta_shape* s, const mi_mdta_params* p, const void* x, const void* residual,
                         void* out, void* saved, void* ws, void* stream, const mi_ln_head* ln, const mi_f8_scales* f8 = nullptr,
                         const TopkHook* topk = nullptr) {
  MI_TRY(mdta_check(s));
  MI_CHECK_ARG(p && x && out && ws, "%s: null pointer", who);
  MI_CHECK_ARG(p->temperature && p->qkv_w && p->dw_w && p->proj_w, "%s: null parameter", who);
  const int B = s->B, C = s->C, dt = s->dtype;
  const int64_t N = (int64_t)s->H * s->W;
  MdtaWs w = mdta_ws_layout(s, ws);
  MdtaSaved sv = saved ? mdta_saved_layout(s, saved) : w.inf;
  TopkHook hk;
  if (topk) {
    hk = *topk;
    hk.S = saved ? (float*)((char*)saved + sv.bytes) : tksa_ws_tail(s, w.bytes, ws).S_inf;
    topk = &hk;
  }
  mi_pw_desc d1 = conv1x1(x, C, p->qkv_w, false, C, p->qkv_b, nullptr, sv.qkv0, 3 * C, B, N, dt);
  ln_head_apply(&d1, ln);
  if (f8) { d1.f8 = 1; d1.f8_sx = f8->x1; d1.f8_sw = f8->w1; }
  MI_TRY(mi_pw_gemm(&d1, w.at.pw_ws, stream));
  MI_TRY(mi_dwconv_fwd(sv.qkv0, p->dw_w, p->dw_b, sv.qkv, B, 3 * C, s->H, s->W, s->ks, dt, stream));
  return attn_core_fwd(mdta_dims(s), mdta_view(s, sv.qkv), p->temperature, p->proj_w, p->proj_b, residual, out, sv.at, w.at,
                       stream, f8, topk);
}
extern "C" int mi_mdta_fwd(const mi_mdta_shape* s, const mi_mdta_params* p, const void* x, const void* residual, void* out,
                           void* saved, void* ws, void* stream) {
  return mdta_fwd_impl("mdta_fwd", s, p, x, residual, out, saved, ws, stream, nullptr);
}
extern "C" int mi_mdta_fwd_ln_ok(const mi_mdta_shape* s) {
  if (mdta_check(s) != MI_OK) return 0;
  const mi_pw_desc d = probe1x1(s->C, 3 * s->C, false, s->B, (int64_t)s->H * s->W, s->dtype);
  return mi_pw_gemm_ln_ok(&d);
}
extern "C" int mi_mdta_fwd_ln(const mi_mdta_shape* s, const mi_mdta_params* p, const mi_ln_head* ln, const void* x,
                              const void* residual, void* out, void* saved, void* ws, void* stream) {
  MI_TRY(ln_head_check(ln, "mdta_fwd_ln"));
  MI_CHECK_ARG(mi_mdta_fwd_ln_ok(s), "mdta_fwd_ln: shape not covered (bf16, C <= 128, H*W %% 64 == 0)");
  return mdta_fwd_impl("mdta_fwd", s, p, x, residual, out, saved, ws, stream, ln);
}

static int f8_check(const mi_f8_scales* f, const char* who) {
  MI_CHECK_ARG(f && f->x1 > 0.f && f->w1 > 0.f && f->x2 > 0.f && f->w2 > 0.f, "%s: fp8 scales must be positive", who);
  return MI_OK;
}
extern "C" int mi_mdta_fwd_f8_ok(const mi_mdta_shape* s, int with_ln) {
  if (mdta_check(s) != MI_OK || s->dtype != MI_BF16) return 0;
  const int64_t N = (int64_t)s->H * s->W;
  const mi_pw_desc d1 = probe1x1(s->C, 3 * s->C, false, s->B, N, s->dtype);
  const mi_pw_desc d2 = per_image(probe1x1(s->C, s->C, false, s->B, N, s->dtype, 3 * (int64_t)s->C * N));
  if (with_ln && !mi_pw_gemm_ln_ok(&d1)) return 0;
  return mi_pw_gemm_f8_ok(&d1) && mi_pw_gemm_f8_ok(&d2);
}
extern "C" int mi_mdta_fwd_f8(const mi_mdta_shape* s, const mi_mdta_params* p, const mi_ln_head* ln, const mi_f8_scales* f8,
                              const void* x, const void* residual, void* out, void* ws, void* stream) {
  MI_TRY(f8_check(f8, "mdta_fwd_f8"));
  if (ln) MI_TRY(ln_head_check(ln, "mdta_fwd_f8"));
  MI_CHECK_ARG(mi_mdta_fwd_f8_ok(s, ln != nullptr), "mdta_fwd_f8: shape not covered (bf16, both projections on a wave-owned form)");
  return mdta_fwd_impl("mdta_fwd", s, p, x, residual, out, nullptr, ws, stream, ln, f8);
}

static int mdta_bwd_impl(const char* who, const mi_mdta_shape* s, const mi_mdta_params* p, const void* x, const void* dout,
                         void* dx, const mi_mdta_grads* gr, const void* saved, void* ws, void* stream, const mi_ln_tail* ln,
                         const TopkHook* topk = nullptr) {
  MI_TRY(mdta_check(s));
  MI_CHECK_ARG(p && x && dout && dx && gr && saved && ws, "%s: null pointer", who);
  MI_CHECK_ARG(gr->temperature && gr->qkv_w && gr->dw_w && gr->proj_w, "%s: null gradient buffer", who);
  hipStream_t st = (hipStream_t)stream;
  const int B = s->B, C = s->C, dt = s->dtype, acc = gr->accumulate;
  const int64_t N = (int64_t)s->H * s->W, bs = 3 * (int64_t)C * N;
  const size_t plane = (size_t)C * N * dtype_size(dt);
  MdtaWs w = mdta_ws_layout(s, ws);
  MdtaSaved sv = mdta_saved_layout(s, const_cast<void*>(saved));
  TopkHook hk;
  if (topk) {
    hk = *topk;
    hk.S = (float*)((char*)const_cast<void*>(saved) + sv.bytes);
    hk.dattn_part = tksa_ws_tail(s, w.bytes, ws).dattn_part;
    topk = &hk;
  }
  char* dq = (char*)w.dqkv;
  MI_TRY(attn_core_bwd(mdta_dims(s), mdta_view(s, sv.qkv), dout, dq, bs, dq + plane, bs, dq + 2 * plane, bs, sv.at,
                       p->temperature, p->proj_w, gr->temperature, gr->proj_w, gr->proj_b, acc, w.at, stream, topk));
  MI_TRY(mi_dwconv_bwd(w.dqkv, sv.qkv0, p->dw_w, w.dqkv0, gr->dw_w, gr->dw_b, B, 3 * C, s->H, s->W, s->ks, acc, dt, w.dw_ws,
                       stream));
  if (ln)
    return launch_bwd_tail(w.dqkv0, 3 * C, x, C, ln->dres, ln->mean, ln->rstd, p->qkv_w, ln->w, ln->b, dx, gr->qkv_w, ln->dw,
                           ln->db, B, N, acc, (char*)ws + align_up(w.bytes, 256), st);
  return conv1x1_bwd_input(w.dqkv0, 3 * C, x, C, p->qkv_w, gr->qkv_w, gr->qkv_b, dx, B, N, dt, acc, w.at.gram_ws, w.at.cs_ws,
                           w.at.pw_ws, st, true);
// ... 100 lines not shown
  MI_TRY(mi_dwconv_gate_fwd(sv.h0, p->dw_w, p->dw_b, (saved && !gdfn_recompute(s)) ? sv.h1 : nullptr, sv.g, B, 2 * h, s->H,
                            s->W, s->ks, dt, stream));
  mi_pw_desc d2 = conv1x1(sv.g, h, p->out_w, false, h, p->out_b, residual, out, C, B, N, dt);
  if (f8) { d2.f8 = 1; d2.f8_sx = f8->x2; d2.f8_sw = f8->w2; }
  MI_TRY(mi_pw_gemm(&d2, w.pw_ws, stream));
  return MI_OK;
}
extern "C" int mi_gdfn_fwd(const mi_gdfn_shape* s, const mi_gdfn_params* p, const void* x, const void* residual, void* out,
                           void* saved, void* ws, void* stream) {
  return gdfn_fwd_impl(s, p, x, residual, out, saved, ws, stream, nullptr);
}
extern "C" int mi_gdfn_fwd_ln_ok(const mi_gdfn_shape* s) {
  if (gdfn_check(s) != MI_OK) return 0;
  const mi_pw_desc d = probe1x1(s->C, 2 * s->hidden, false, s->B, (int64_t)s->H * s->W, s->dtype);
  return mi_pw_gemm_ln_ok(&d);
}
extern "C" int mi_gdfn_fwd_ln(const mi_gdfn_shape* s, const mi_gdfn_params* p, const mi_ln_head* ln, const void* x,
                              const void* residual, void* out, void* saved, void* ws, void* stream) {
  MI_TRY(ln_head_check(ln, "gdfn_fwd_ln"));
  MI_CHECK_ARG(mi_gdfn_fwd_ln_ok(s), "gdfn_fwd_ln: shape not covered (bf16, C <= 128, H*W %% 64 == 0)");
  return gdfn_fwd_impl(s, p, x, residual, out, saved, ws, stream, ln);
}

extern "C" int mi_gdfn_fwd_f8_ok(const mi_gdfn_shape* s, int with_ln) {
  if (gdfn_check(s) != MI_OK || s->dtype != MI_BF16) return 0;
  const int64_t N = (int64_t)s->H * s->W;
  const mi_pw_desc d1 = probe1x1(s->C, 2 * s->hidden, false, s->B, N, s->dtype);
  const mi_pw_desc d2 = probe1x1(s->hidden, s->C, false, s->B, N, s->dtype);
  if (with_ln && !mi_pw_gemm_ln_ok(&d1)) return 0;
  return mi_pw_gemm_f8_ok(&d1) && mi_pw_gemm_f8_ok(&d2);
}
extern "C" int mi_gdfn_fwd_f8(const mi_gdfn_shape* s, const mi_gdfn_params* p, const mi_ln_head* ln, const mi_f8_scales* f8,
                              const void* x, const void* residual, void* out, void* ws, void* stream) {
  MI_TRY(f8_check(f8, "gdfn_fwd_f8"));
  if (ln) MI_TRY(ln_head_check(ln, "gdfn_fwd_f8"));
  MI_CHECK_ARG(mi_gdfn_fwd_f8_ok(s, ln != nullptr), "gdfn_fwd_f8: shape not covered (bf16, both projections on a wave-owned form)");
  return gdfn_fwd_impl(s, p, x, residual, out, nullptr, ws, stream, ln, f8);
}

extern "C" int mi_gdfn_fused_fwd_train_ok(const mi_gdfn_fused_shape* f) {
  return fg_plan(f, FG_TRAIN).covered ? 1 : 0;
}
extern "C" int mi_gdfn_fused_fwd_train(const mi_gdfn_fused_shape* f, const void* pack, const void* y, void* out, float* mean,
                                       float* rstd, void* saved, void* stream) {
  MI_CHECK_ARG(mi_gdfn_fused_fwd_train_ok(f), "gdfn_fused_fwd_train: shape not covered (mi_gdfn_fused_fwd_train_ok)");
  MI_CHECK_ARG(saved, "gdfn_fused_fwd_train: null saved blob");
  mi_gdfn_shape s = {f->B, f->C, f->hidden, f->H, f->W, MI_BF16, 3, 0};
  GdfnSaved sv = gdfn_saved_layout(&s, saved);
  return fused_gdfn_fwd_save(f, pack, y, out, mean, rstd, sv.h0, sv.g, (hipStream_t)stream);
}

static int gdfn_bwd_impl(const mi_gdfn_shape* s, const mi_gdfn_params* p, const void* x, const void* dout, void* dx,
                         const mi_gdfn_grads* gr, const void* saved, void* ws, void* stream, const mi_ln_tail* ln) {
  MI_TRY(gdfn_check(s));
  MI_CHECK_ARG(p && x && dout && dx && gr && saved && ws, "gdfn_bwd: null pointer");
  MI_CHECK_ARG(gr->in_w && gr->dw_w && gr->out_w, "gdfn_bwd: null gradient buffer");
  hipStream_t st = (hipStream_t)stream;
  const int B = s->B, C = s->C, h = s->hidden, dt = s->dtype, acc = gr->accumulate;
  const int64_t N = (int64_t)s->H * s->W;
  GdfnWs w = gdfn_ws_layout(s, ws);
  GdfnSaved sv = gdfn_saved_layout(s, const_cast<void*>(saved));
  MI_TRY(conv1x1_bwd_output(dout, C, sv.g, h, p->out_w, gr->out_w, gr->out_b, w.dg, B, N, dt, acc, w.gram_ws, w.cs_ws, w.pw_ws, st));
  if (gdfn_recompute(s))
    MI_TRY(mi_dwconv_gate_bwd_recompute(w.dg, sv.h0, p->dw_w, p->dw_b, w.dh0, gr->dw_w, gr->dw_b, B, 2 * h, s->H, s->W, s->ks,
                                        acc, dt, w.dw_ws, stream));
  else
    MI_TRY(mi_dwconv_gate_bwd(w.dg, sv.h1, sv.h0, p->dw_w, w.dh0, gr->dw_w, gr->dw_b, B, 2 * h, s->H, s->W, s->ks, acc, dt,
                              w.dw_ws, stream));
  if (ln)
    return launch_bwd_tail(w.dh0, 2 * h, x, C, ln->dres, ln->mean, ln->rstd, p->in_w, ln->w, ln->b, dx, gr->in_w, ln->dw, ln->db,
                           B, N, acc, (char*)ws + align_up(w.bytes, 256), st);
  return conv1x1_bwd_input(w.dh0, 2 * h, x, C, p->in_w, gr->in_w, gr->in_b, dx, B, N, dt, acc, w.gram_ws, w.cs_ws, w.pw_ws, st, true);
}
extern "C" int mi_gdfn_bwd(const mi_gdfn_shape* s, const mi_gdfn_params* p, const void* x, const void* dout, void* dx,
                           const mi_gdfn_grads* gr, const void* saved, void* ws, void* stream) {
  return gdfn_bwd_impl(s, p, x, dout, dx, gr, saved, ws, stream, nullptr);
}
extern "C" int mi_gdfn_bwd_ln_ok(const mi_gdfn_shape* s, int in_bias) {
  if (gdfn_check(s) != MI_OK || in_bias) return 0;
  return bwd_tail_ok(2 * s->hidden, s->C, (int64_t)s->H * s->W, s->dtype) && bwd_tail_pays(2 * s->hidden, s->C) ? 1 : 0;
}
extern "C" size_t mi_gdfn_bwd_ln_workspace(const mi_gdfn_shape* s) {
  if (!mi_gdfn_bwd_ln_ok(s, 0)) return 0;
  return align_up(gdfn_ws_layout(s, nullptr).bytes, 256) + bwd_tail_workspace(2 * s->hidden, s->C);
}
extern "C" int mi_gdfn_bwd_ln(const mi_gdfn_shape* s, const mi_gdfn_params* p, const mi_ln_tail* ln, const void* x,
                              const void* dout, void* dx, const mi_gdfn_grads* gr, const void* saved, void* ws, void* stream) {
  MI_TRY(ln_tail_check(ln, "gdfn_bwd_ln"));
  MI_CHECK_ARG(gr && !gr->in_b && mi_gdfn_bwd_ln_ok(s, 0), "gdfn_bwd_ln: shape not covered (bf16, C 48/96, H*W %% 64 == 0, no project_in bias)");
  return gdfn_bwd_impl(s, p, x, dout, dx, gr, saved, ws, stream, ln);
}

static TopkHook tksa_hook(const mi_tksa_shape* s, const mi_tksa_params* tp, float* scores, const mi_tksa_grads* tg) {
  TopkHook hk;
  memset(&hk, 0, sizeof(hk));
  hk.tk.w[0] = tp->attn1; hk.tk.w[1] = tp->attn2; hk.tk.w[2] = tp->attn3; hk.tk.w[3] = tp->attn4;
  hk.tk.k[0] = s->k1; hk.tk.k[1] = s->k2; hk.tk.k[2] = s->k3; hk.tk.k[3] = s->k4;
  hk.scores = scores;
  if (tg) { hk.g_attn[0] = tg->attn1; hk.g_attn[1] = tg->attn2; hk.g_attn[2] = tg->attn3; hk.g_attn[3] = tg->attn4; }
  return hk;
}

extern "C" size_t mi_tksa_saved_bytes(const mi_tksa_shape* s) {
  if (tksa_shape_check(s) != MI_OK) return 0;
  const mi_mdta_shape ms = tksa_mdta_shape(s);
  return mdta_saved_layout(&ms, nullptr).bytes + tksa_scores_bytes(&ms);
}
extern "C" size_t mi_tksa_workspace(const mi_tksa_shape* s) {
  if (tksa_shape_check(s) != MI_OK) return 0;
  const mi_mdta_shape ms = tksa_mdta_shape(s);
  return tksa_ws_tail(&ms, mdta_ws_layout(&ms, nullptr).bytes, nullptr).bytes;
}

extern "C" int mi_tksa_fwd(const mi_tksa_shape* s, const mi_mdta_params* p, const mi_tksa_params* tp, const void* x,
                           const void* residual, void* out, void* saved, void* ws, float* scores, void* stream) {
  MI_TRY(tksa_shape_check(s));
  MI_CHECK_ARG(tp, "tksa_fwd: null pointer");
  MI_CHECK_ARG(tp->attn1 && tp->attn2 && tp->attn3 && tp->attn4, "tksa_fwd: null attn1..4");
  const mi_mdta_shape ms = tksa_mdta_shape(s);
  const TopkHook hk = tksa_hook(s, tp, scores, nullptr);
  return mdta_fwd_impl("tksa_fwd", &ms, p, x, residual, out, saved, ws, stream, nullptr, nullptr, &hk);
}

extern "C" int mi_tksa_bwd(const mi_tksa_shape* s, const mi_mdta_params* p, const mi_tksa_params* tp, const void* x,
                           const void* dout, void* dx, const mi_mdta_grads* gr, const mi_tksa_grads* tg, const void* saved, void* ws,
                           void* stream) {
  MI_TRY(tksa_shape_check(s));
  MI_CHECK_ARG(tp && tg, "tksa_bwd: null pointer");
  MI_CHECK_ARG(tp->attn1 && tp->attn2 && tp->attn3 && tp->attn4, "tksa_bwd: null attn1..4");
  MI_CHECK_ARG(tg->attn1 && tg->attn2 && tg->attn3 && tg->attn4, "tksa_bwd: null attn1..4 gradient buffer");
  const mi_mdta_shape ms = tksa_mdta_shape(s);
  const TopkHook hk = tksa_hook(s, tp, nullptr, tg);
  return mdta_bwd_impl("tksa_bwd", &ms, p, x, dout, dx, gr, saved, ws, stream, nullptr, &hk);
}

struct MsfnSaved { void* h0; void* a; void* b; void* y; size_t bytes; };
static MsfnSaved msfn_saved_layout(const mi_msfn_shape* s, void* base) {
  const size_t n = (size_t)s->B * 2 * s->hidden * s->H * s->W;
  Carver cv(base);
  MsfnSaved r;
  r.h0 = cv.take(tbytes(n, s->dtype));
  r.a = cv.take(tbytes(n, s->dtype));
  r.b = cv.take(tbytes(n, s->dtype));
  r.y = cv.take(tbytes(n, s->dtype));
  r.bytes = cv.off;
  return r;
}
struct MsfnWs { void* gram_ws; void* pw_ws; void* cs_ws; float* part; MsfnSaved inf; void* dY; void* dza; void* dzb; size_t bytes; };
static MsfnWs msfn_ws_layout(const mi_msfn_shape* s, void* base) {
  const int B = s->B, C = s->C, h2 = 2 * s->hidden, dt = s->dtype;
  const int64_t N = (int64_t)s->H * s->W;
  Carver cv(base);
  MsfnWs w;
  w.gram_ws = cv.take(max_of({gram_ws_bytes(probe_wgrad(C, h2, B, N, dt)), gram_ws_bytes(probe_wgrad(h2, C, B, N, dt))}));
  w.pw_ws = cv.take(max_of({pw_ws_bytes(probe1x1(C, h2, false, B, N, dt)), pw_ws_bytes(probe1x1(h2, C, false, B, N, dt)),
                            pw_ws_bytes(probe1x1(C, h2, true, B, N, dt)), pw_ws_bytes(probe1x1(h2, C, true, B, N, dt))}));
  w.cs_ws = cv.take(chan_sum_workspace(h2 > C ? h2 : C, N));
  w.part = cv.take<float>(fbytes(msfn_part_floats(B, s->hidden, s->H, s->W)));
  const size_t mark = cv.off;
  w.inf = msfn_saved_layout(s, base ? (char*)base + mark : nullptr);
  Carver big(base ? (char*)base + mark : nullptr);
  const size_t plane = tbytes((size_t)B * h2 * N, dt);
  w.dY = big.take(plane);
  w.dza = big.take(plane);
  w.dzb = big.take(plane);
  w.bytes = mark + max_of({w.inf.bytes, big.off});
  return w;
}
static int msfn_check(const mi_msfn_shape* s) {
  MI_CHECK_ARG(s, "msfn: null shape");
  MI_CHECK_ARG(s->B > 0 && s->C > 0 && s->hidden > 0 && s->H > 0 && s->W > 0, "msfn: bad shape");
  MI_CHECK_ARG(2 * s->hidden <= 65535, "msfn: hidden=%d too large (2*hidden <= 65535)", s->hidden);
  MI_CHECK_ARG(s->dtype == MI_F32 || s->dtype == MI_BF16, "msfn: bad dtype %d", s->dtype);
  return MI_OK;
}

extern "C" size_t mi_msfn_saved_bytes(const mi_msfn_shape* s) {
  if (msfn_check(s) != MI_OK) return 0;
  return msfn_saved_layout(s, nullptr).bytes;
}
extern "C" size_t mi_msfn_workspace(const mi_msfn_shape* s) {
  if (msfn_check(s) != MI_OK) return 0;
  return msfn_ws_layout(s, nullptr).bytes;
}

extern "C" int mi_msfn_fwd(const mi_msfn_shape* s, const mi_msfn_params* p, const void* x, const void* residual, void* out,
                           void* saved, void* ws, void* stream) {
  MI_TRY(msfn_check(s));
  MI_CHECK_ARG(p && x && out && ws, "msfn_fwd: null pointer");
  MI_CHECK_ARG(p->in_w && p->dw3_w && p->dw5_w && p->g3_w && p->g5_w && p->out_w, "msfn_fwd: null parameter");
  hipStream_t st = (hipStream_t)stream;
  const int B = s->B, C = s->C, hd = s->hidden, dt = s->dtype;
  const int64_t N = (int64_t)s->H * s->W;
  MsfnWs w = msfn_ws_layout(s, ws);
  MsfnSaved sv = saved ? msfn_saved_layout(s, saved) : w.inf;
  mi_pw_desc d1 = conv1x1(x, C, p->in_w, false, C, p->in_b, nullptr, sv.h0, 2 * hd, B, N, dt);
  MI_TRY(mi_pw_gemm(&d1, w.pw_ws, stream));
  MI_TRY(launch_msfn_s1_fwd(sv.h0, p->dw3_w, p->dw3_b, p->dw5_w, p->dw5_b, sv.a, sv.b, B, hd, s->H, s->W, dt, st));
  MI_TRY(launch_msfn_s2_fwd(sv.a, sv.b, p->g3_w, p->g3_b, p->g5_w, p->g5_b, sv.y, B, hd, s->H, s->W, dt, st));
  mi_pw_desc d2 = conv1x1(sv.y, 2 * hd, p->out_w, false, 2 * hd, p->out_b, residual, out, C, B, N, dt);
  return mi_pw_gemm(&d2, w.pw_ws, stream);
}

extern "C" int mi_msfn_bwd(const mi_msfn_shape* s, const mi_msfn_params* p, const void* x, const void* dout, void* dx,
                           const mi_msfn_grads* gr, const void* saved, void* ws, void* stream) {
  MI_TRY(msfn_check(s));
  MI_CHECK_ARG(p && x && dout && dx && gr && saved && ws, "msfn_bwd: null pointer");
  MI_CHECK_ARG(p->in_w && p->dw3_w && p->dw5_w && p->g3_w && p->g5_w && p->out_w, "msfn_bwd: null parameter");
  MI_CHECK_ARG(gr->in_w && gr->dw3_w && gr->dw5_w && gr->g3_w && gr->g5_w && gr->out_w, "msfn_bwd: null gradient buffer");
  hipStream_t st = (hipStream_t)stream;
  const int B = s->B, C = s->C, hd = s->hidden, dt = s->dtype, acc = gr->accumulate;
  const int64_t N = (int64_t)s->H * s->W;
  MsfnWs w = msfn_ws_layout(s, ws);
  MsfnSaved sv = msfn_saved_layout(s, const_cast<void*>(saved));
  MI_TRY(conv1x1_bwd_output(dout, C, sv.y, 2 * hd, p->out_w, gr->out_w, gr->out_b, w.dY, B, N, dt, acc, w.gram_ws, w.cs_ws, w.pw_ws,
                            st));
  MI_TRY(launch_msfn_s2_bwd(w.dY, sv.y, sv.a, sv.b, p->g3_w, p->g5_w, w.dza, w.dzb, gr->g3_w, gr->g3_b, gr->g5_w, gr->g5_b, acc,
                            w.part, B, hd, s->H, s->W, dt, st));
  void* dh0 = w.dY;
  MI_TRY(launch_msfn_s1_bwd(w.dza, w.dzb, sv.h0, p->dw3_w, p->dw5_w, dh0, gr->dw3_w, gr->dw3_b, gr->dw5_w, gr->dw5_b, acc, w.part,
                            B, hd, s->H, s->W, dt, st));
  return conv1x1_bwd_input(dh0, 2 * hd, x, C, p->in_w, gr->in_w, gr->in_b, dx, B, N, dt, acc, w.gram_ws, w.cs_ws, w.pw_ws, st, true);
}
```

### image_restoration_amd/csrc/util.hip

```cpp
#include <stdarg.h>
#include <stdlib.h>

#include <atomic>
#include <algorithm>
#include <mutex>
#include <unordered_map>
#include <vector>

#include "common.h"

namespace mi {

static thread_local char g_err[512] = "";
void set_error(const char* fmt, ...) {
  va_list ap;
  va_start(ap, fmt);
  vsnprintf(g_err, sizeof(g_err), fmt, ap);
  va_end(ap);
}

struct EnvTable { char val[E_ENV_COUNT][48]; bool set[E_ENV_COUNT]; };
static EnvTable g_env;
static std::once_flag g_env_once;
static void env_load() {
  static const char* const names[E_ENV_COUNT] = {
#define MI_ENV_NAME(n) #n,
      MI_ENV_LIST(MI_ENV_NAME)
#undef MI_ENV_NAME
  };
  for (int i = 0; i < E_ENV_COUNT; ++i) {
    const char* e = getenv(names[i]);
    g_env.set[i] = e != nullptr && e[0] != 0;
    g_env.val[i][0] = 0;
    if (e) { strncpy(g_env.val[i], e, sizeof(g_env.val[i]) - 1); g_env.val[i][sizeof(g_env.val[i]) - 1] = 0; }
  }
}
const char* env_get(int id) {
  std::call_once(g_env_once, env_load);
  return (id >= 0 && id < E_ENV_COUNT && g_env.set[id]) ? g_env.val[id] : nullptr;
}

struct ProfRec { int kid; double bytes, flops; hipEvent_t e0, e1; };
static std::mutex g_prof_mu;
static std::vector<ProfRec> g_prof_recs;
static std::atomic<int> g_prof_on{0};
static const char* const g_kernel_names[K_COUNT] = {
    "ln_fwd", "ln_bwd", "dwconv_fwd", "dwconv_gate_fwd", "dwconv_bwd_data", "dwconv_gate_bwd_data", "dwconv_wgrad",
    "pw_gemm", "gram", "gram_reduce", "attn_fold", "attn_bwd_small", "reduce_rows", "chan_sum", "adamw", "cast", "l1_loss",
    "pw_pack", "gap", "im2col3x3", "col2im3x3", "gdfn_fused_fwd", "gdfn_fused_bwd", "mdta_fused_a", "fused_pack", "moe_route", "patch_circconv", "ewise", "conv3x3", "mdta_qk", "mdta_av", "bwd_tail", "bwd_tail_finish", "adair_fre", "grad_sumsq",
    "adamw_clip", "adamw_clip_ema", "tksa_attn", "tksa_fold", "tksa_bwd", "tksa_dwo", "msfn_stencil1", "msfn_stencil2",
    "msfn_stencil1_bwd", "msfn_stencil2_bwd", "mefc_stencil_a", "mefc_stencil_b", "mefc_stencil_a_bwd", "mefc_stencil_b_bwd",
    "mefc_dw_wgrad", "mefc_fold", "mefc_fold_bwd", "mefc_head", "mefc_head_bwd", "mefc_ewise",
    "darkir_dilgate_fwd", "darkir_dilgate_bwd_dz", "darkir_dilgate_bwd_dx", "darkir_pairconv", "darkir_pairconv_wgrad", "darkir_fold",
    "darkir_fold_bwd"};

ProfScope::ProfScope(hipStream_t stream, int kernel_id, double bytes, double flops)
    : st(stream), kid(kernel_id), on(g_prof_on.load(std::memory_order_relaxed) != 0) {
  if (!on) return;
  ProfRec r{kernel_id, bytes, flops, nullptr, nullptr};
  if (hipEventCreate(&r.e0) != hipSuccess || hipEventCreate(&r.e1) != hipSuccess) { on = false; return; }
  (void)hipEventRecord(r.e0, st);
  std::lock_guard<std::mutex> lk(g_prof_mu);
  g_prof_recs.push_back(r);
  kid = (int)g_prof_recs.size() - 1;
}
ProfScope::~ProfScope() {
  if (!on) return;
  std::lock_guard<std::mutex> lk(g_prof_mu);
  if (kid >= 0 && kid < (int)g_prof_recs.size()) (void)hipEventRecord(g_prof_recs[kid].e1, st);
}

__global__ __launch_bounds__(256) void reduce_rows_kernel(const float* __restrict__ part, float* __restrict__ out,
                                                          int64_t rows, int64_t cols, int64_t ld, int accumulate,
                                                          float scale, int64_t rpg, int64_t out_gs,
                                                          float* __restrict__ out2, int64_t split) {
  __shared__ float sm[8][32];
  const int cx = threadIdx.x & 31, ph = threadIdx.x >> 5;
  const int64_t c = (int64_t)blockIdx.x * 32 + cx;
  const int64_t r_begin = (int64_t)blockIdx.y * rpg;
  int64_t r_end = r_begin + rpg;
  if (r_end > rows) r_end = rows;
  float a0 = 0.f, a1 = 0.f, a2 = 0.f, a3 = 0.f;
  if (c < cols) {
    int64_t r = r_begin + ph;
    for (; r + 24 < r_end; r += 32) {
      a0 += part[r * ld + c];
      a1 += part[(r + 8) * ld + c];
      a2 += part[(r + 16) * ld + c];
      a3 += part[(r + 24) * ld + c];
    }
    for (; r < r_end; r += 8) a0 += part[r * ld + c];
  }
  sm[ph][cx] = (a0 + a1) + (a2 + a3);
  __syncthreads();
  if (ph == 0 && c < cols) {
    float t = 0.f;
#pragma unroll
    for (int k = 0; k < 8; ++k) t += sm[k][cx];
    float* o = (out2 && c >= split) ? out2 + (c - split) : out + (int64_t)blockIdx.y * out_gs + c;
    *o = (accumulate ? *o : 0.f) + scale * t;
  }
}

int launch_reduce_rows(const float* part, float* out, int64_t rows, int64_t cols, int64_t part_ld, int accumulate,
                       float scale, hipStream_t st, float* tmp, float* out2, int64_t split) {
  if (cols <= 0) return MI_OK;
  if (deferred_reduce_rows(part, out, rows, cols, part_ld, accumulate, scale, out2, split)) return MI_OK;
  if (tmp && reduce_rows_two_stage(rows)) {
    const int64_t rpg = (rows + REDUCE_GROUPS - 1) / REDUCE_GROUPS;
    {
      ProfScope ps(st, K_REDUCE_ROWS, (double)(rows + REDUCE_GROUPS) * cols * 4, (double)rows * cols);
      hipLaunchKernelGGL(reduce_rows_kernel, dim3(cdiv(cols, 32), REDUCE_GROUPS), dim3(256), 0, st, part, tmp, rows, cols,
                         part_ld, 0, 1.0f, rpg, cols, (float*)nullptr, (int64_t)0);
    }
    MI_LAUNCH_CHECK();
    part = tmp; rows = REDUCE_GROUPS; part_ld = cols;
  }
  ProfScope ps(st, K_REDUCE_ROWS, (double)(rows + 1) * cols * 4, (double)rows * cols);
  hipLaunchKernelGGL(reduce_rows_kernel, dim3(cdiv(cols, 32), 1), dim3(256), 0, st, part, out, rows, cols, part_ld,
                     accumulate, scale, rows, (int64_t)0, out2, split);
  MI_LAUNCH_CHECK();
  return MI_OK;
}

struct DrJob {
  const float* part; float* tmp; float* out; float* out2;
  int64_t rows, cols, ld, split, rpg;
  int groups, accumulate; float scale;
  int blk1, blk2;
};
constexpr int DR_MAX_JOBS = 2048;
constexpr size_t DR_TABLE_BYTES = DR_MAX_JOBS * sizeof(DrJob);
static struct {
  std::mutex mu;
  bool active = false;
  bool recording = false;
  char* arena = nullptr;
  size_t bytes = 0, off = 0;
  std::vector<DrJob> jobs;
  DrJob* host_tab[2] = {nullptr, nullptr};
  hipEvent_t copied[2] = {nullptr, nullptr};
  int flip = 0;
  int nblk1 = 0, nblk2 = 0;
  size_t high = 0;
  std::unordered_map<const float*, int> out_gen;
  std::vector<int> gen_blocks;
} g_dr;

static bool stream_capturing(hipStream_t st) {
  hipStreamCaptureStatus cs = hipStreamCaptureStatusNone;
  if (hipStreamIsCapturing(st, &cs) != hipSuccess) { (void)hipGetLastError(); return false; }
  return cs != hipStreamCaptureStatusNone;
}

float* deferred_take(size_t nfloats, hipStream_t st) {
  {
    std::lock_guard<std::mutex> lk(g_dr.mu);
    if (!g_dr.active || !g_dr.recording) return nullptr;
  }
  if (stream_capturing(st)) return nullptr;
  std::lock_guard<std::mutex> lk(g_dr.mu);
  if (!g_dr.active || !g_dr.recording || g_dr.jobs.size() + 1 >= (size_t)DR_MAX_JOBS) return nullptr;
  const size_t need = align_up(nfloats * sizeof(float), 256);
  if (g_dr.off + need > g_dr.bytes) return nullptr;
  float* p = reinterpret_cast<float*>(g_dr.arena + g_dr.off);
  g_dr.off += need;
  if (g_dr.off > g_dr.high) g_dr.high = g_dr.off;
  return p;
}
bool deferred_owns(const void* p) {
  std::lock_guard<std::mutex> lk(g_dr.mu);
  return g_dr.active && (const char*)p >= g_dr.arena + DR_TABLE_BYTES && (const char*)p < g_dr.arena + g_dr.bytes;
}
bool deferred_reduce_rows(const float* part, float* out, int64_t rows, int64_t cols, int64_t part_ld, int accumulate, float scale,
                          float* out2, int64_t split) {
  if (cols <= 0 || rows <= 0) return false;
  if (!deferred_owns(part)) return false;
  DrJob j;
  j.part = part; j.out = out; j.out2 = out2; j.rows = rows; j.cols = cols; j.ld = part_ld; j.split = split;
  j.accumulate = accumulate; j.scale = scale;
  j.groups = 1; j.rpg = rows; j.tmp = nullptr;
  std::lock_guard<std::mutex> lk(g_dr.mu);
  if (!g_dr.active || g_dr.jobs.size() >= (size_t)DR_MAX_JOBS) return false;
  int gen = 0;
  for (const float* o : {(const float*)out, (const float*)out2}) {
    if (!o) continue;
    auto it = g_dr.out_gen.find(o);
    if (it != g_dr.out_gen.end() && it->second + 1 > gen) gen = it->second + 1;
  }
  g_dr.out_gen[out] = gen;
  if (out2) g_dr.out_gen[out2] = gen;
  if ((int)g_dr.gen_blocks.size() <= gen) g_dr.gen_blocks.resize(gen + 1, 0);
  j.blk2 = gen;
  j.blk1 = g_dr.gen_blocks[gen];
  g_dr.gen_blocks[gen] += (int)cdiv(cols, 256);
  g_dr.nblk1 += (int)cdiv(cols, 256);
  g_dr.jobs.push_back(j);
  return true;
}

__global__ __launch_bounds__(256) void deferred_reduce_kernel(const DrJob* __restrict__ jobs, int njobs) {
  const int bid = blockIdx.x;
  int lo = 0, hi = njobs - 1;
  while (lo < hi) {
    const int mid = (lo + hi + 1) >> 1;
    if (jobs[mid].blk1 <= bid) lo = mid; else hi = mid - 1;
  }
// ... 387 lines not shown
```

### image_restoration_amd/ops.py

```python
from __future__ import annotations

import ctypes as C
import functools
import os
from typing import Optional, Sequence, Tuple

import torch

from . import _lib as L

Tensor = torch.Tensor


def _dtype_code(dtype: torch.dtype) -> int:
    if dtype == torch.float32:
        return L.MI_F32
    if dtype == torch.bfloat16:
        return L.MI_BF16
    raise TypeError(f"activations must be float32 or bfloat16, got {dtype}")


def _dt(t: Tensor) -> int:
    return _dtype_code(t.dtype)

# ... 158 lines not shown
    L.check(L.lib().mi_dwconv_gate_bwd(_p(dg), _p(y), _p(x), _p(w), _p(dx), _p(dw), _p(db), B, C2, H, W, ks, 0, _dt(x),
                                       _p(ws), _stream()), "dwconv_gate_bwd")
    return dx, dw, db


def dwconv_gate_recompute_ok(H: int, W: int, ks: int) -> bool:
    return bool(L.lib().mi_dwconv_gate_recompute_ok(H, W, ks))


DWCONV_PLAN_OPS = {"fwd": 0, "gate_fwd": 1, "bwd": 2, "gate_bwd": 3}


def dwconv_plan(B: int, C: int, H: int, W: int, ks: int, op: str) -> dict:
    out = (L.C.c_int * 6)()
    L.check(L.lib().mi_dwconv_plan(B, C, H, W, ks, DWCONV_PLAN_OPS[op], out), "dwconv_plan")
    if out[0] == 1:
        return {"family": "stream", "band": out[1], "nb": out[2], "lpr": out[3], "uni": bool(out[4]), "rows": out[5]}
    return {"family": "lds", "th": out[1], "bands": out[2], "tw": out[3], "uni": False, "rpt": out[5]}


def dwconv_gate_bwd_recompute(dg: Tensor, x: Tensor, w: Tensor, bias: Optional[Tensor]):
    _gpu(dg, x, w, bias)
    B, C2, H, W = x.shape
    ks = w.shape[-1]
    dx = torch.empty_like(x)
    dw = torch.empty_like(w)
    db = torch.empty(C2, dtype=torch.float32, device=x.device) if bias is not None else None
    ws = _ws(L.lib().mi_dwconv_bwd_workspace(B, C2, H, W, ks), x.device)
    L.check(L.lib().mi_dwconv_gate_bwd_recompute(_p(dg), _p(x), _p(w), _p(bias), _p(dx), _p(dw), _p(db), B, C2, H, W, ks, 0,
                                                 _dt(x), _p(ws), _stream()), "dwconv_gate_bwd_recompute")
    return dx, dw, db


def conv1x1(x: Tensor, w: Tensor, bias: Optional[Tensor] = None, residual: Optional[Tensor] = None,
            transposed: bool = False, x2: Optional[Tensor] = None, out: Optional[Tensor] = None,
            f8: Optional[Tuple[float, float]] = None) -> Tensor:
    _gpu(x, w, bias, residual, x2)
    _f32(w, "1x1 weight"); _f32(bias, "1x1 bias")
    B, K1, H, W = x.shape
    K2 = 0 if x2 is None else x2.shape[1]
    N = H * W
    w2 = w.reshape(w.shape[0], -1)
    M = w2.shape[1] if transposed else w2.shape[0]
    assert (w2.shape[0] if transposed else w2.shape[1]) == K1 + K2, "weight/input channel mismatch"
    y = torch.empty((B, M, H, W), dtype=x.dtype, device=x.device) if out is None else out
    assert y.shape == (B, M, H, W) and y.is_contiguous() and y.dtype == x.dtype
    d = L.PwDesc()
    d.x1, d.x1_bs, d.x1_gs, d.k1 = _p(x), K1 * N, 0, K1
    d.x2, d.x2_bs, d.x2_gs, d.k2 = _p(x2), K2 * N, 0, K2
    d.w, d.w_bs, d.w_gs = _p(w2), 0, 0
    d.w_sm, d.w_sk = (1, w2.shape[1]) if transposed else (w2.shape[1], 1)
    d.bias, d.bias_gs = _p(bias), 0
    d.r, d.r_bs, d.r_gs = _p(residual), M * N, 0
    d.y, d.y_bs, d.y_gs = _p(y), M * N, 0
    d.m, d.n, d.batch, d.groups, d.dtype = M, N, B, 1, _dt(x)
    if f8 is not None:
        d.f8, d.f8_sx, d.f8_sw = 1, float(f8[0]), float(f8[1])
    pw_gemm_desc(d, x.device)
    return y


def pw_gemm_desc(d: "L.PwDesc", device) -> None:
    ws = _ws(L.lib().mi_pw_gemm_workspace(C.byref(d)), device)
    L.check(L.lib().mi_pw_gemm(C.byref(d), _p(ws), _stream()), "pw_gemm")


PW_FAMILIES = ("chunked", "resident", "dma", "xres", "stream", "xwide", "lds")
PW_WEIGHTS = ("pack", "b16", "f32")
PW_PROBE = 256


def pw_probe(M: int, K: int, N: int, dtype: torch.dtype, B: int = 1, groups: int = 1, K2: int = 0, per_image: bool = False,
             transposed: bool = False, residual: bool = False, misalign: int = 0) -> "L.PwDesc":
    d = L.PwDesc()
    kt = K + K2
    d.x1, d.x1_bs, d.x1_gs, d.k1 = PW_PROBE + misalign, groups * K * N, K * N, K
    if K2:
        d.x2, d.x2_bs, d.x2_gs, d.k2 = PW_PROBE, groups * K2 * N, K2 * N, K2
    d.w, d.w_bs, d.w_gs = PW_PROBE, (groups * M * kt if per_image else 0), (M * kt if groups > 1 else 0)
    d.w_sm, d.w_sk = (1, M) if transposed else (kt, 1)
    if residual:
        d.r = PW_PROBE + misalign
    d.r_bs, d.r_gs = groups * M * N, M * N
    d.y, d.y_bs, d.y_gs = PW_PROBE + misalign, groups * M * N, M * N
    d.m, d.n, d.batch, d.groups, d.dtype = M, N, B, groups, _dtype_code(dtype)
    return d


def pw_plan(d: "L.PwDesc") -> dict:
    out = (L.c_i64 * 18)()
    L.check(L.lib().mi_pw_plan(C.byref(d), out), "pw_plan")
    return {"family": PW_FAMILIES[out[0]], "tm": out[1], "kb": out[2], "f8": bool(out[3]), "ln": bool(out[4]),
            "grid": (out[5], out[6], out[7]), "block": out[8], "lds": out[9], "tpw": out[10], "tpb": out[11], "n_slabs": out[12],
            "slabs_per": out[13], "xcd_map": bool(out[14]), "weights": PW_WEIGHTS[out[15]], "cacheable": bool(out[16]),
            "workspace": out[17]}


GRAM_FAMILIES = ("lds", "stream")
GRAM_FINISH = ("direct", "few4", "few16", "general")


def gram_probe(ma: int, mb: int, N: int, dtype: torch.dtype, B: int = 1, groups: int = 1, sum_batch: bool = False, sumsq: bool = False,
               accumulate: bool = False, out_ld: int = 0, misalign: int = 0) -> "L.GramDesc":
    d = L.GramDesc()
    d.a, d.a_bs, d.a_gs, d.ma = PW_PROBE + misalign, groups * ma * N, ma * N, ma
    d.b, d.b_bs, d.b_gs, d.mb = PW_PROBE, groups * mb * N, mb * N, mb
    d.n, d.batch, d.groups, d.dtype = N, B, groups, _dtype_code(dtype)
    d.sum_batch, d.accumulate = int(sum_batch), int(accumulate)
    d.out, d.out_ld, d.out_zs, d.sumsq = PW_PROBE, out_ld or mb, ma * mb, (PW_PROBE if sumsq else None)
    return d


def gram_desc(a: Tensor, b: Tensor, groups: int = 1, sum_batch: bool = False, want_sumsq: bool = False, out: Optional[Tensor] = None,
              accumulate: bool = False, ss: Optional[Tensor] = None) -> "L.GramDesc":
    B, Ca, H, W = a.shape
    d = gram_probe(Ca // groups, b.shape[1] // groups, H * W, a.dtype, B=B, groups=groups, sum_batch=sum_batch, sumsq=want_sumsq,
                   accumulate=accumulate)
    d.a, d.b = _p(a), _p(b)
    if out is not None:
        d.out = _p(out)
    if ss is not None:
        d.sumsq = _p(ss)
    return d


def gram_plan(d: "L.GramDesc") -> dict:
    out = (L.c_i64 * 22)()
    L.check(L.lib().mi_gram_plan(C.byref(d), out), "gram_plan")
    return {"family": GRAM_FAMILIES[out[0]], "fa": out[1], "fb": out[2], "sumsq": bool(out[3]), "unit": out[4], "units": out[5],
            "per_split": out[6], "splits": out[7], "tiles_a": out[8], "tiles_b": out[9], "Z": out[10], "fold": out[11],
            "vec_ok": bool(out[12]), "grid": (out[13], out[14], out[15]), "block": out[16], "part_bytes": out[17], "ss_bytes": out[18],
            "finish": GRAM_FINISH[out[19]], "deferrable": bool(out[20]), "workspace": out[21]}


def gram(a: Tensor, b: Tensor, groups: int = 1, sum_batch: bool = False, want_sumsq: bool = False,
         out: Optional[Tensor] = None, accumulate: bool = False):
    _gpu(a, b, out)
    B, Ca, H, W = a.shape
    ma, mb = Ca // groups, b.shape[1] // groups
    Z = groups if sum_batch else B * groups
    if out is None:
        if accumulate:
            raise ValueError("gram: accumulate needs the output buffer")
        out = torch.empty((Z, ma, mb), dtype=torch.float32, device=a.device)
    elif out.dtype != torch.float32 or out.numel() != Z * ma * mb:
        raise ValueError(f"gram: out must be float32 with {Z * ma * mb} elements")
    ss = torch.empty((B * groups, ma + mb), dtype=torch.float32, device=a.device) if want_sumsq else None
    d = gram_desc(a, b, groups, sum_batch, want_sumsq, out, accumulate, ss)
    ws = _ws(L.lib().mi_gram_workspace(C.byref(d)), a.device)
    L.check(L.lib().mi_gram(C.byref(d), _p(ws), _stream()), "gram")
    return (out, ss) if want_sumsq else out


def conv1x1_dgrad_panel(dy: Tensor, w2: Tensor, k0: int, k: int) -> Tensor:
    B, M, H, W = dy.shape
    N = H * W
    dx = torch.empty((B, k, H, W), dtype=dy.dtype, device=dy.device)
    d = L.PwDesc()
    d.x1, d.x1_bs, d.k1 = _p(dy), M * N, M
    d.w = _p(w2) + 4 * k0
    d.w_sm, d.w_sk = 1, w2.shape[1]
    d.y, d.y_bs = _p(dx), k * N
    d.m, d.n, d.batch, d.groups, d.dtype = k, N, B, 1, _dt(dy)
    pw_gemm_desc(d, dy.device)
    return dx


def wgrad_panel_desc(dy: Tensor, xp: Tensor, dw2: Tensor, k0: int, accumulate: bool) -> "L.GramDesc":
    d = gram_desc(dy, xp, 1, True, accumulate=accumulate)
    d.out, d.out_ld = _p(dw2) + 4 * k0, dw2.shape[1]
    return d


def conv1x1_wgrad_panels(dy: Tensor, x1: Tensor, x2: Optional[Tensor], dw2: Tensor, accumulate: bool) -> None:
    B, M, H, W = dy.shape
    N = H * W
    k0 = 0
    for xp in (x1, x2):
        if xp is None:
            continue
        k = xp.shape[1]
        d = wgrad_panel_desc(dy, xp, dw2, k0, accumulate)
        ws = _blob(L.lib().mi_gram_workspace(C.byref(d)), dy.device)
        L.check(L.lib().mi_gram(C.byref(d), _p(ws), _stream()), "gram(wgrad panel)")
        k0 += k


MdtaParamsT = Tuple[Tensor, Tensor, Optional[Tensor], Tensor, Optional[Tensor], Tensor, Optional[Tensor]]
GdfnParamsT = Tuple[Tensor, Optional[Tensor], Tensor, Optional[Tensor], Tensor, Optional[Tensor]]


def _mdta_shape(x: Tensor, heads: int, ks: int) -> L.MdtaShape:
    B, Cc, H, W = x.shape
    return L.MdtaShape(B, Cc, heads, H, W, _dt(x), ks)


def _mdta_params(p: Sequence[Optional[Tensor]]) -> L.MdtaParams:
    return _f32_struct(L.MdtaParams, p, "MDTA parameter")


def mdta_saved_bytes(x: Tensor, heads: int, ks: int) -> int:
    return int(L.lib().mi_mdta_saved_bytes(C.byref(_mdta_shape(x, heads, ks))))


LnHeadT = Tuple[Tensor, Optional[Tensor], bool]


def _ln_head(ln: LnHeadT, x: Tensor):
    w, b, want_stats = ln
    _gpu(w, b)
    _f32(w, "LayerNorm weight"); _f32(b, "LayerNorm bias")
    mean = rstd = None
    if want_stats:
        mean = torch.empty((x.shape[0], x.shape[2] * x.shape[3]), dtype=torch.float32, device=x.device)
        rstd = torch.empty_like(mean)
    return L.LnHead(_p(w), _p(b), _p(mean), _p(rstd), int(b is not None)), mean, rstd


def mdta_fwd_ln_ok(x: Tensor, heads: int, ks: int) -> bool:
    if not x.is_cuda:
        return False
    s = _mdta_shape(x, heads, ks)
    return bool(L.lib().mi_mdta_fwd_ln_ok(C.byref(s)))


F8ScalesT = Tuple[float, float, float, float]


def mdta_fwd_f8_ok(x: Tensor, heads: int, ks: int, with_ln: bool) -> bool:
    if not x.is_cuda or x.dtype != torch.bfloat16:
        return False
    s = _mdta_shape(x, heads, ks)
    return bool(L.lib().mi_mdta_fwd_f8_ok(C.byref(s), int(with_ln)))


def mdta_fwd(x: Tensor, residual: Optional[Tensor], params: MdtaParamsT, heads: int, need_saved: bool,
             ln: Optional[LnHeadT] = None, f8: Optional[F8ScalesT] = None):
    _gpu(x, residual, *params)
    ks = params[3].shape[-1]
    s = _mdta_shape(x, heads, ks)
    lib = L.lib()
    out = torch.empty_like(x)
    if f8 is not None:
        if need_saved or (ln is not None and ln[2]):
            raise ValueError("fp8 projections are an inference path: nothing can be saved")
        ws = _ws(lib.mi_mdta_workspace(C.byref(s)), x.device)
        lh = _ln_head(ln, x)[0] if ln is not None else None
        L.check(lib.mi_mdta_fwd_f8(C.byref(s), C.byref(_mdta_params(params)), C.byref(lh) if lh is not None else None,
                                   C.byref(L.F8Scales(*[float(v) for v in f8])), _p(x), _p(residual), _p(out), _p(ws),
                                   _stream()), "mdta_fwd_f8")
        return out
    saved = _blob(lib.mi_mdta_saved_bytes(C.byref(s)), x.device) if need_saved else None
    ws = _ws(lib.mi_mdta_workspace(C.byref(s)), x.device)
    pp = _mdta_params(params)
    if ln is None:
        L.check(lib.mi_mdta_fwd(C.byref(s), C.byref(pp), _p(x), _p(residual), _p(out), _p(saved), _p(ws), _stream()),
                "mdta_fwd")
        return out, saved
    lh, mean, rstd = _ln_head(ln, x)
    L.check(lib.mi_mdta_fwd_ln(C.byref(s), C.byref(pp), C.byref(lh), _p(x), _p(residual), _p(out), _p(saved), _p(ws),
                               _stream()), "mdta_fwd_ln")
    return out, saved, mean, rstd


LnTailT = Tuple[Tensor, Tensor, Tensor, Tensor, Optional[Tensor], Tensor, Tensor]


def _ln_tail(ln: LnTailT, like: Tensor) -> L.LnTail:
    w, b, mean, rstd, dres, dw, db = ln
    _gpu(w, b, mean, rstd, dres, dw, db)
    for t_ in (w, b, mean, rstd, dw, db):
        _f32(t_, "LayerNorm tail tensor")
    if dres is not None and (dres.shape != like.shape or dres.dtype != like.dtype):
        raise ValueError("LayerNorm tail: dres must match the block input")
    return L.LnTail(_p(w), _p(b), _p(mean), _p(rstd), _p(dres), _p(dw), _p(db))


def mdta_bwd_ln_ok(x: Tensor, heads: int, ks: int, qkv_bias: bool) -> bool:
    if not x.is_cuda:
        return False
    s = _mdta_shape(x, heads, ks)
    return bool(L.lib().mi_mdta_bwd_ln_ok(C.byref(s), int(qkv_bias)))


def mdta_bwd(x: Tensor, dout: Tensor, params: MdtaParamsT, heads: int, saved: Tensor,
             grads: Sequence[Optional[Tensor]], accumulate: bool, ln: Optional[LnTailT] = None) -> Tensor:
    _gpu(x, dout, saved, *params, *grads)
    ks = params[3].shape[-1]
    s = _mdta_shape(x, heads, ks)
    lib = L.lib()
    dx = torch.empty_like(x)
    pp = _mdta_params(params)
    gg = _f32_struct(L.MdtaGrads, grads, "MDTA gradient", int(accumulate))
    if ln is None:
        ws = _ws(lib.mi_mdta_workspace(C.byref(s)), x.device)
        L.check(lib.mi_mdta_bwd(C.byref(s), C.byref(pp), _p(x), _p(dout), _p(dx), C.byref(gg), _p(saved), _p(ws), _stream()),
                "mdta_bwd")
    else:
        lt = _ln_tail(ln, x)
        ws = _ws(lib.mi_mdta_bwd_ln_workspace(C.byref(s)), x.device)
        L.check(lib.mi_mdta_bwd_ln(C.byref(s), C.byref(pp), C.byref(lt), _p(x), _p(dout), _p(dx), C.byref(gg), _p(saved),
                                   _p(ws), _stream()), "mdta_bwd_ln")
    return dx


def _xmdta_shape(x: Tensor, heads: int, ks_q: int, ks_kv: int) -> L.XmdtaShape:
# ... 1985 lines not shown
```

### include/mi_restore.h

```cpp
#ifndef MI_RESTORE_H
#define MI_RESTORE_H

#include <stddef.h>
#include <stdint.h>

#ifdef __cplusplus
extern "C" {
#endif

#define MI_RESTORE_VERSION 100

typedef enum { MI_F32 = 0, MI_BF16 = 1 } mi_dtype;

enum {
  MI_OK = 0,
  MI_ERR_ARG = -1,
  MI_ERR_ALIGN = -2,
  MI_ERR_HIP = -3
};

int mi_version(void);
const char* mi_last_error(void);
int mi_env_reload(void);

// ... 122 lines not shown
  const float* dw3_w; const float* dw3_b;
  const float* dw5_w; const float* dw5_b;
  const float* g3_w;  const float* g3_b;
  const float* g5_w;  const float* g5_b;
  const float* out_w; const float* out_b;
} mi_msfn_params;
typedef struct {
  float* in_w; float* in_b; float* dw3_w; float* dw3_b; float* dw5_w; float* dw5_b; float* g3_w; float* g3_b; float* g5_w;
  float* g5_b; float* out_w; float* out_b; int accumulate;
} mi_msfn_grads;
size_t mi_msfn_saved_bytes(const mi_msfn_shape* s);
size_t mi_msfn_workspace(const mi_msfn_shape* s);
int mi_msfn_fwd(const mi_msfn_shape* s, const mi_msfn_params* p, const void* x, const void* residual,
                void* out, void* saved, void* ws, void* stream);
int mi_msfn_bwd(const mi_msfn_shape* s, const mi_msfn_params* p, const void* x, const void* dout,
                void* dx, const mi_msfn_grads* g, const void* saved, void* ws, void* stream);

typedef struct { int B, C, H, W, dtype, steps; } mi_mefc_shape;
typedef struct {
  const float* sep_dw1[4]; const float* sep_pw1[4];
  const float* sep_dw2[4]; const float* sep_pw2[4];
  const float* dil_dw[3];  const float* dil_pw[3];
  const float* out_w;
} mi_mefc_step_params;
typedef struct {
  float* sep_dw1[4]; float* sep_pw1[4]; float* sep_dw2[4]; float* sep_pw2[4]; float* dil_dw[3]; float* dil_pw[3]; float* out_w;
} mi_mefc_step_grads;
typedef struct {
  const float* fc1_w; const float* fc1_b;
  const float* fc2_w; const float* fc2_b;
  const float* pre_w;
  const mi_mefc_step_params* step;
} mi_mefc_params;
typedef struct {
  float* fc1_w; float* fc1_b; float* fc2_w; float* fc2_b; float* pre_w;
  const mi_mefc_step_grads* step;
  int accumulate;
} mi_mefc_grads;
size_t mi_mefc_saved_bytes(const mi_mefc_shape* s);
size_t mi_mefc_workspace(const mi_mefc_shape* s);
int mi_mefc_fwd(const mi_mefc_shape* s, const mi_mefc_params* p, const void* x, void* out, void* saved, void* ws, void* stream);
int mi_mefc_bwd(const mi_mefc_shape* s, const mi_mefc_params* p, const void* x, const void* out, const void* dout, void* dx,
                const mi_mefc_grads* g, const void* saved, void* ws, void* stream);

typedef struct { const float* w[4]; const float* b[4]; } mi_dilgate_params;
typedef struct { float* w[4]; float* b[4]; int accumulate; } mi_dilgate_grads;
int mi_dilgate_plan(int B, int c, int H, int W, int dtype, int n_dil, const int* dil, int64_t* out);
size_t mi_dilgate_fwd_workspace(int B, int c, int H, int W);
int mi_dilgate_fwd(const void* x, const mi_dilgate_params* p, void* g, float* pool, int B, int c, int H, int W, int n_dil,
                   const int* dil, int dtype, void* ws, void* stream);
size_t mi_dilgate_bwd_workspace(int B, int c, int H, int W, int n_dil, int dtype);
int mi_dilgate_bwd(const void* dg, const float* dg_add, const void* x, const mi_dilgate_params* p, void* dx,
                   const mi_dilgate_grads* gr, int B, int c, int H, int W, int n_dil, const int* dil, int dtype, void* ws,
                   void* stream);
int mi_pairconv3x3_fwd(const void* x, const float* w, const float* bias, void* y, int B, int c, int H, int W, int dtype,
                       void* stream);
size_t mi_pairconv3x3_bwd_workspace(int B, int c, int H, int W);
int mi_pairconv3x3_bwd(const void* dy, const void* x, const float* w, void* dx, float* dw, float* db, int B, int c, int H, int W,
                       int accumulate, int dtype, void* ws, void* stream);

typedef struct { int B, C, H, W, dtype, n_dil; int dil[4]; int extra; } mi_dblock_shape;
typedef struct {
  const float* norm1_w; const float* norm1_b; const float* conv1_w; const float* conv1_b; const float* extra_w; const float* extra_b;
  const float* br_w[4]; const float* br_b[4];
  const float* sca_w; const float* sca_b; const float* conv3_w; const float* conv3_b; const float* beta;
  const float* norm2_w; const float* norm2_b; const float* conv4_w; const float* conv4_b; const float* conv5_w; const float* conv5_b;
  const float* gamma;
} mi_dblock_params;
typedef struct {
  float* norm1_w; float* norm1_b; float* conv1_w; float* conv1_b; float* extra_w; float* extra_b;
  float* br_w[4]; float* br_b[4];
  float* sca_w; float* sca_b; float* conv3_w; float* conv3_b; float* beta;
  float* norm2_w; float* norm2_b; float* conv4_w; float* conv4_b; float* conv5_w; float* conv5_b;
  float* gamma;
  int accumulate;
} mi_dblock_grads;
size_t mi_dblock_saved_bytes(const mi_dblock_shape* s);
size_t mi_dblock_workspace(const mi_dblock_shape* s);
int mi_dblock_fwd(const mi_dblock_shape* s, const mi_dblock_params* p, const void* inp, void* out, void* saved, void* ws,
                  void* stream);
int mi_dblock_bwd(const mi_dblock_shape* s, const mi_dblock_params* p, const void* inp, const void* dout, void* dinp,
                  const mi_dblock_grads* g, const void* saved, void* ws, void* stream);

typedef struct { int B, C, hidden, H, W, dtype, ks, flags; } mi_gdfn_shape;
typedef struct {
  const float* in_w;  const float* in_b;
  const float* dw_w;  const float* dw_b;
  const float* out_w; const float* out_b;
} mi_gdfn_params;
typedef struct { float* in_w; float* in_b; float* dw_w; float* dw_b; float* out_w; float* out_b; int accumulate; } mi_gdfn_grads;
size_t mi_gdfn_saved_bytes(const mi_gdfn_shape* s);
size_t mi_gdfn_workspace(const mi_gdfn_shape* s);
int mi_gdfn_fwd(const mi_gdfn_shape* s, const mi_gdfn_params* p, const void* x, const void* residual,
                void* out, void* saved, void* ws, void* stream);
int mi_gdfn_bwd(const mi_gdfn_shape* s, const mi_gdfn_params* p, const void* x, const void* dout,
                void* dx, const mi_gdfn_grads* g, const void* saved, void* ws, void* stream);

typedef struct { int B, C, hidden, H, W, ln_with_bias; } mi_gdfn_fused_shape;
int mi_gdfn_fused_ok(const mi_gdfn_fused_shape* s);
size_t mi_gdfn_fused_pack_bytes(const mi_gdfn_fused_shape* s);
int mi_gdfn_fused_pack(const mi_gdfn_fused_shape* s, const float* ln_w, const float* ln_b, const mi_gdfn_params* p,
                       void* pack, void* stream);
int mi_gdfn_fused_fwd(const mi_gdfn_fused_shape* s, const void* pack, const void* y, void* out, float* mean,
                      float* rstd, void* stream);
int mi_gdfn_fused_fwd_train_ok(const mi_gdfn_fused_shape* s);
int mi_gdfn_fused_fwd_train(const mi_gdfn_fused_shape* s, const void* pack, const void* y, void* out, float* mean,
                            float* rstd, void* saved, void* stream);
int mi_gdfn_fused_plan(const mi_gdfn_fused_shape* s, int entry, int64_t* out);

typedef struct {
  const float* w; const float* b;
  const float* mean; const float* rstd;
  const void* dres;
  float* dw; float* db;
} mi_ln_tail;
typedef struct { const float* w; const float* b; float* mean; float* rstd; int with_bias; } mi_ln_head;
int mi_mdta_fwd_ln_ok(const mi_mdta_shape* s);
int mi_mdta_fwd_ln(const mi_mdta_shape* s, const mi_mdta_params* p, const mi_ln_head* ln, const void* x, const void* residual,
                   void* out, void* saved, void* ws, void* stream);
int mi_gdfn_fwd_ln_ok(const mi_gdfn_shape* s);
int mi_gdfn_fwd_ln(const mi_gdfn_shape* s, const mi_gdfn_params* p, const mi_ln_head* ln, const void* x, const void* residual,
                   void* out, void* saved, void* ws, void* stream);
typedef struct { float x1, w1, x2, w2; } mi_f8_scales;
int mi_mdta_fwd_f8_ok(const mi_mdta_shape* s, int with_ln);
int mi_mdta_fwd_f8(const mi_mdta_shape* s, const mi_mdta_params* p, const mi_ln_head* ln, const mi_f8_scales* f8, const void* x,
                   const void* residual, void* out, void* ws, void* stream);
int mi_gdfn_fwd_f8_ok(const mi_gdfn_shape* s, int with_ln);
int mi_gdfn_fwd_f8(const mi_gdfn_shape* s, const mi_gdfn_params* p, const mi_ln_head* ln, const mi_f8_scales* f8, const void* x,
                   const void* residual, void* out, void* ws, void* stream);
int mi_gdfn_fused_fwd_f8(const mi_gdfn_fused_shape* s, const void* pack, const mi_f8_scales* f8, const void* y, void* out,
                         void* stream);

int mi_mdta_fused_ok(const mi_mdta_shape* s);
int mi_mdta_fused_pays(const mi_mdta_shape* s);
size_t mi_mdta_fused_pack_bytes(const mi_mdta_shape* s);
int mi_mdta_fused_pack(const mi_mdta_shape* s, const float* ln_w, const float* ln_b, const mi_mdta_params* p, void* pack,
                       void* stream);
size_t mi_mdta_fused_workspace(const mi_mdta_shape* s);
int mi_mdta_fused_plan(const mi_mdta_shape* s, int64_t* out);
int mi_mdta_fused_fwd(const mi_mdta_shape* s, const mi_mdta_params* p, const void* pack, int ln_with_bias, const void* x,
                      const void* residual, void* out, float* mean, float* rstd, void* ws, void* stream);
int mi_attn_small_plan(int B, int C, int heads, int64_t* out);
int mi_attn_small_fwd(const float* graw, const float* ss, const float* temperature, const float* wo, float* P, float* A,
                      float* nrm, float* M, void* Mb, void* Mtb, int B, int C, int heads, void* stream);
int mi_attn_small_bwd(const float* dM, const float* A, const float* P, const float* nrm, const float* temperature,
                      const float* wo, float* dwo_part, float* dtemp_part, float* wd, void* wdb, int B, int C, int heads,
                      void* stream);
int mi_bwd_tail_ok(int M, int C, int64_t N, int dtype);
size_t mi_bwd_tail_workspace(int M, int C);
int mi_bwd_tail_plan(int M, int C, int B, int64_t N, int dtype, int64_t* out);
int mi_bwd_tail(const void* dy, int M, const void* x, int C, const void* dres, const float* mean, const float* rstd,
                const float* w, const float* gamma, const float* beta, void* dx, float* dw, float* dgamma, float* dbeta,
                int B, int64_t N, int accumulate, int dtype, void* ws, void* stream);
int mi_mdta_bwd_ln_ok(const mi_mdta_shape* s, int qkv_bias);
size_t mi_mdta_bwd_ln_workspace(const mi_mdta_shape* s);
int mi_mdta_bwd_ln(const mi_mdta_shape* s, const mi_mdta_params* p, const mi_ln_tail* ln, const void* x, const void* dout,
                   void* dx, const mi_mdta_grads* gr, const void* saved, void* ws, void* stream);
int mi_gdfn_bwd_ln_ok(const mi_gdfn_shape* s, int in_bias);
size_t mi_gdfn_bwd_ln_workspace(const mi_gdfn_shape* s);
int mi_gdfn_bwd_ln(const mi_gdfn_shape* s, const mi_gdfn_params* p, const mi_ln_tail* ln, const void* x, const void* dout,
                   void* dx, const mi_gdfn_grads* gr, const void* saved, void* ws, void* stream);

int mi_box_down(const void* img, void* out, int B, int C, int Hi, int Wi, int factor, int dtype, void* stream);
int mi_fre_rect(const float* pooled, const float* w0, const float* w2, int* half, int B, int C, int R, int H, int W, int n,
                void* stream);
size_t mi_fre_split_coef_bytes(int B, int C);
size_t mi_fre_split_workspace(int B, int C, int H, int W);
int mi_fre_split_max_hw(void);
int mi_fre_split_fwd(const void* feat, const int* half, void* high, void* low, float* coef, int B, int C, int H, int W, int dtype,
                     void* stream);
int mi_fre_split_bwd(const void* feat, const int* half, const float* coef, const void* dhigh, const void* dlow, void* dfeat, int B,
                     int C, int H, int W, int dtype, void* ws, void* stream);
int mi_chan_maxmean_fwd(const void* x, void* out, int* idx, int B, int C, int64_t N, int dtype, void* stream);
int mi_chan_maxmean_bwd(const void* dout, const int* idx, void* dx, int B, int C, int64_t N, int dtype, void* stream);
int mi_plane_max_fwd(const void* x, float* out, int* idx, int planes, int64_t N, int dtype, void* stream);
int mi_pool_pair_bwd(const float* davg, const float* dmax, const int* idx, void* dx, int planes, int64_t N, int dtype, void* stream);
int mi_chan_gate_fwd(const float* avg, const float* mx, const float* w1, const float* w2, float* cw, float* hid, int B, int C, int R,
                     void* stream);
int mi_chan_gate_bwd(const float* avg, const float* mx, const float* w1, const float* w2, const float* cw, const float* hid,
                     const float* dcw, float* davg, float* dmx, float* dw1, float* dw2, int B, int C, int R, int accumulate,
                     void* stream);
int mi_refine_mix_fwd(const void* low, const void* high, const void* s, const float* cw, void* out, int B, int C, int64_t N,
                      int dtype, void* stream);
int mi_refine_mix_bwd(const void* low, const void* high, const void* s, const float* cw, const void* dout, void* dlow, void* dhigh,
                      void* ds, float* dcw, int B, int C, int64_t N, int dtype, void* stream);
int mi_scale_add_fwd(const void* a, const void* y, const float* p1, const float* p2, void* out, int B, int C, int64_t N, int dtype,
                     void* stream);
int mi_scale_add_bwd(const void* a, const void* y, const float* p1, const float* p2, const void* dout, void* da, void* dy, float* dp1,
                     float* dp2, int B, int C, int64_t N, int accumulate, int dtype, void* stream);

int mi_adamw_step(float* p, const float* g, float* m, float* v, int64_t n, float lr, float beta1,
                  float beta2, float eps, float weight_decay, int step, float grad_scale,
                  const float* dev_scalars, void* stream);

size_t mi_grad_sumsq_workspace(int64_t n);
int mi_grad_sumsq(const float* x, int64_t n, float* out, void* workspace, void* stream);
int mi_adamw_step_ex(float* p, const float* g, float* m, float* v, float* ema, int64_t n, float lr,
                     float beta1, float beta2, float eps, float weight_decay, int step, float grad_scale,
                     const float* dev_scalars, const float* sumsq, float max_norm, float* norm_out,
                     float ema_decay, void* stream);

int mi_rows_gather(const void* x, const int64_t* idx, void* out, int n_out, int64_t row, int dtype, void* stream);
int mi_rows_gather_scaled(const float* x, const int64_t* idx, const float* scale, void* out, int n_out, int64_t row,
                          int out_dtype, void* stream);
int mi_rows_scatter_add(const void* src, const int64_t* idx, const float* scale, void* out, int n_src, int n_rows,
                        int64_t row, int dtype, int out_f32, void* stream);
size_t mi_rows_dot_workspace(int n_src, int64_t row);
int mi_rows_dot(const float* g, const void* src, const int64_t* idx, float* out, int n_src, int64_t row, int dtype,
                void* ws, void* stream);

typedef struct {
  const void* x; int64_t x_rs;
  const float* w; int64_t w_sm, w_sk;
  const float* bias;
  const void* r; int64_t r_rs;
  void* y; int64_t y_rs;
  int m, k;
  int expert;
  int x_local, y_local, r_local;
} mi_grouped_problem;
int mi_grouped_pw_gemm(const mi_grouped_problem* probs, int np, const int* dev_counts, const int* dev_offsets, int max_rows,
                       int64_t N, int dtype, void* stream);

int mi_moe_route_fwd(const float* pooled, const float* freq, const float* wg, const float* wf, const float* noise,
                     const float* complexity, float* logits, float* gates, int64_t* topk_idx, float* topk_val, float* aux,
                     int* counts, int* offsets, int64_t* perm, float* perm_gate, int* perm_expert, int* row_of, int B, int C, int F,
                     int E, int k, int training, void* stream);
int mi_moe_route_bwd(const float* pooled, const float* freq, const float* wg, const float* wf, const float* noise,
                     const float* complexity, const float* logits, const int64_t* topk_idx, const float* dgates,
                     const float* drow, const int* row_of, const float* daux, float* dpooled, float* dfreq, float* dwg, float* dwf,
                     int B, int C, int F, int E, int k, int training, void* stream);

int mi_patch_circconv(const void* x, int64_t x_bs, const void* y, int64_t y_bs, void* out, int64_t out_bs, int B, int C, int H,
                      int W, int patch, int flip, int dtype, void* stream);

int mi_gelu_gap_fwd(const void* x, float* out, int B, int C, int64_t N, int dtype, void* stream);
int mi_gelu_gap_bwd(const void* x, const float* dout, void* dx, int B, int C, int64_t N, int dtype, void* stream);

int mi_ewise_fwd(const void* a, int64_t a_rs, const void* b, int64_t b_rs, void* out, int64_t rows, int64_t L, int op, int dtype,
                 void* stream);
int mi_ewise_bwd(const void* a, int64_t a_rs, const void* b, int64_t b_rs, const void* dout, void* da, int64_t da_rs, void* db,
                 int64_t db_rs, int64_t rows, int64_t L, int op, int dtype, void* stream);

int mi_glue3x3_ok(int H, int W);
int mi_im2col3x3(const void* x, void* out, int B, int C, int H, int W, int flip, int dtype, void* stream);
int mi_col2im3x3(const void* z, const float* bias, const void* residual, void* y, int B, int M, int H, int W, int flip,
                 int dtype, void* stream);
int mi_glue3x3_plan(int64_t planes, int H, int W, int dtype, int aligned, int64_t* out);

int mi_conv3x3_ok(int H, int W, int dtype);
size_t mi_conv3x3_pack_bytes(int M, int K);
int mi_conv3x3_pack(const float* w, int M, int K, int transpose_flip, void* pack, void* stream);
int mi_conv3x3_fwd(const void* pack, const void* x, int64_t x_bs, const float* bias, const void* residual, int64_t r_bs,
                   void* y, int64_t y_bs, int B, int M, int K, int H, int W, void* stream);
size_t mi_conv3x3_wgrad_workspace(int B, int M, int K, int H, int W);
int mi_conv3x3_wgrad(const void* dy, int64_t dy_bs, const void* x, int64_t x_bs, float* dw, int accumulate, int B, int M, int K,
                     int H, int W, void* ws, void* stream);
int mi_conv3x3_plan(int B, int M, int K, int H, int W, int64_t* out);

int mi_pixel_shuffle2(const void* in, int64_t in_bs, void* out, int64_t out_bs, int B, int c, int H, int W, int unshuffle,
                      int dtype, void* stream);
int mi_copy_rows(const void* src, int64_t src_rs, void* dst, int64_t dst_rs, int64_t rows, int64_t L, int dtype, void* stream);
int mi_pixel_shuffle2_plan(int B, int c, int H, int W, int64_t in_bs, int64_t out_bs, int dtype, int aligned, int64_t* out);
int mi_copy_rows_plan(int64_t rows, int64_t L, int64_t src_rs, int64_t dst_rs, int dtype, int aligned, int64_t* out);

int mi_gap_fwd(const void* x, float* out, int B, int C, int64_t N, int dtype, void* stream);
size_t mi_chan_sum_workspace(int C, int64_t N);
int mi_chan_sum_plan(int B, int C, int64_t N, int dtype, int aligned, int64_t* out);
int mi_chan_sum(const void* x, float* out, int B, int C, int64_t N, int dtype, int accumulate, void* ws, void* stream);
int mi_gap_bwd(const float* dout, void* dx, int B, int C, int64_t N, int dtype, void* stream);

int mi_patch_batch(const unsigned char* pool, const int64_t* src_off, const int* src_h, const int* src_w, const int* sample,
                   const int* top, const int* left, const int* mode, const float* sigma, const float* noise, void* clean,
                   void* degraded, int B, int P, int dtype, void* stream);

size_t mi_psnr_ssim_workspace(int B, int C, int H, int W);
int mi_psnr_ssim(const void* restored, const void* clean, float* psnr, float* ssim, int B, int C, int H, int W, int dtype,
                 void* ws, void* stream);

int mi_cast(const void* src, int src_dtype, void* dst, int dst_dtype, int64_t n, void* stream);
int mi_l1_loss(const void* a, const void* b, void* da, float* loss, int64_t n, float scale, int dtype,
               void* stream);

size_t mi_fft_l1_workspace(int B, int C, int H, int W);
int mi_fft_l1_plan(int B, int C, int H, int W, int dtype, int want_grad, int64_t* out);
int mi_fft_l1_loss(const void* pred, const void* target, void* dpred, float* loss, int B, int C, int H, int W,
                   float loss_weight, int dtype, void* ws, void* stream);

typedef struct { int B, nc, expand, H, W, dtype; } mi_fremlp_shape;
size_t mi_dft2_workspace(int B, int C, int H, int W);
int mi_dft2_r2c(const void* x, float* zre, float* zim, int B, int C, int H, int W, int dtype, void* ws, void* stream);
int mi_dft2_c2r(const float* yre, const float* yim, void* out, int B, int C, int H, int W, int dtype, void* ws, void* stream);
size_t mi_fremlp_workspace(const mi_fremlp_shape* s);
size_t mi_fremlp_saved_bytes(const mi_fremlp_shape* s);
int mi_fremlp_plan(const mi_fremlp_shape* s, int64_t* out);
int mi_fremlp_fwd(const mi_fremlp_shape* s, const float* w1, const float* b1, const float* w2, const float* b2, const void* x,
                  void* out, void* saved, void* ws, void* stream);
int mi_fremlp_bwd(const mi_fremlp_shape* s, const float* w1, const float* w2, const float* b2, const void* dout, void* dx,
                  float* g_w1, float* g_b1, float* g_w2, float* g_b2, int accumulate, const void* saved, void* ws, void* stream);

typedef struct { int B, c, groups, H, W, dtype, training; float eps, momentum; } mi_fourier_unit_shape;
typedef struct {
  const float* bn_w; const float* bn_b; const float* fdc_w; const float* fdc_b; const float* gate_w; const float* gate_b;
  const float* fpe_w; const float* fpe_b;
} mi_fourier_unit_params;
typedef struct {
// ... 145 lines not shown
```

Measured before the change: 15.92 Mpixels/s.

## Fuse weight-grad gram and data-grad GEMM into a single-pass dy kernel

Adds a dy_once kernel that reads the upstream gradient tile once, computing both the weight-gradient gram (dy x input^T, accumulated per block then row-reduced) and the data-gradient 1x1 GEMM output from the same LDS-staged tile. It is wired into the attention backward path in place of separate mi_gram and mi_pw_gemm calls, and workspaces are sized for GDFN/MSFN, with an env switch to disable it. The aim is to halve global reads of the large bf16 dy activation in backward, at the cost of a partial-sum reduction pass and more register and LDS pressure.

```diff
diff --git a/image_restoration_amd/_lib.py b/image_restoration_amd/_lib.py
--- a/image_restoration_amd/_lib.py
+++ b/image_restoration_amd/_lib.py
@@ -34,6 +34,16 @@
                 ("n", c_i64), ("batch", C.c_int), ("groups", C.c_int), ("dtype", C.c_int),
                 ("sum_batch", C.c_int), ("accumulate", C.c_int),
                 ("out", fp), ("out_ld", c_i64), ("out_zs", c_i64), ("sumsq", fp)]
+
+
+class DyOnceDesc(C.Structure):
+    _fields_ = [("s", vp), ("s_bs", c_i64), ("ks", C.c_int),
+                ("r", vp), ("r_bs", c_i64), ("mr", C.c_int),
+                ("w", fp), ("w_sr", c_i64), ("w_sk", c_i64),
+                ("w_b16", vp), ("w_b16_bs", c_i64), ("w_b16_ld", c_i64),
+                ("o", vp), ("o_bs", c_i64),
+                ("g", fp),
+                ("n", c_i64), ("batch", C.c_int), ("dtype", C.c_int), ("per_image", C.c_int), ("accumulate", C.c_int)]
 
 
 class MdtaShape(C.Structure):
@@ -312,6 +322,11 @@
     "mi_gram_workspace": (C.c_size_t, [C.POINTER(GramDesc)]),
     "mi_gram": (C.c_int, [C.POINTER(GramDesc), vp, vp]),
     "mi_gram_plan": (C.c_int, [C.POINTER(GramDesc), C.POINTER(c_i64)]),
+    "mi_dy_once_ok": (C.c_int, [C.POINTER(DyOnceDesc)]),
+    "mi_dy_once_workspace": (C.c_size_t, [C.POINTER(DyOnceDesc)]),
+    "mi_dy_once_plan": (C.c_int, [C.POINTER(DyOnceDesc), C.POINTER(c_i64)]),
+    "mi_dy_once_instances": (C.c_int, [C.POINTER(C.c_int), C.c_int]),
+    "mi_dy_once": (C.c_int, [C.POINTER(DyOnceDesc), vp, vp]),
     "mi_mdta_saved_bytes": (C.c_size_t, [C.POINTER(MdtaShape)]),
     "mi_mdta_workspace": (C.c_size_t, [C.POINTER(MdtaShape)]),
     "mi_mdta_fwd": (C.c_int, [C.POINTER(MdtaShape), C.POINTER(MdtaParams), vp, vp, vp, vp, vp, vp]),
diff --git a/image_restoration_amd/csrc/common.h b/image_restoration_amd/csrc/common.h
--- a/image_restoration_amd/csrc/common.h
+++ b/image_restoration_amd/csrc/common.h
@@ -45,7 +45,8 @@
   X(MI_BT_WIDE) X(MI_BT_DEBUG) X(MI_DW_LDS) X(MI_FG_CFG) X(MI_FG_DEBUG) X(MI_FG_NOXCD) X(MI_GRAM_FOLD) X(MI_GRAM_WANT)      \
   X(MI_GRAM_RECT) X(MI_GRAM_LDS) X(MI_GRAM_STREAM_ALL) X(MI_LN_FORM) X(MI_CO_STREAM) X(MI_ATTN_DQK_SPLIT)    \
   X(MI_PW_DMA) X(MI_PW_TM_EVEN) X(MI_PW_WAVE) X(MI_PW_CHUNKED) X(MI_PW_XWIDE) X(MI_PW_WAVE_WIDE) X(MI_PW_DIRECT)             \
-  X(MI_PW_WAVE_TPW) X(MI_PW_XCD) X(MI_PW_TPB) X(MI_PW_B16) X(MI_FM_DEBUG) X(MI_FM_CFG) X(MI_NO_FUSED_MDTA) X(MI_NO_PW_LDS) X(MI_PW_LDS)
+  X(MI_PW_WAVE_TPW) X(MI_PW_XCD) X(MI_PW_TPB) X(MI_PW_B16) X(MI_FM_DEBUG) X(MI_FM_CFG) X(MI_NO_FUSED_MDTA) X(MI_NO_PW_LDS) X(MI_PW_LDS) \
+  X(MI_NO_DY_ONCE)
 enum EnvId {
 #define MI_ENV_ENUM(n) E_##n,
   MI_ENV_LIST(MI_ENV_ENUM)
@@ -307,7 +308,7 @@
   K_IM2COL, K_COL2IM, K_GDFN_FUSED_FWD, K_GDFN_FUSED_BWD, K_MDTA_FUSED_A, K_FUSED_PACK, K_MOE_ROUTE, K_CIRCCONV, K_EWISE, K_CONV3X3, K_GRAM_QK, K_PW_AV, K_BWD_TAIL, K_BWD_TAIL_FIN, K_ADAIR, K_SUMSQ, K_ADAMW_CLIP, K_ADAMW_EMA,
   K_TKSA_ATTN, K_TKSA_FOLD, K_TKSA_BWD, K_TKSA_DWO, K_MSFN_S1, K_MSFN_S2, K_MSFN_S1_BWD, K_MSFN_S2_BWD,
   K_MEFC_STA, K_MEFC_STB, K_MEFC_STA_BWD, K_MEFC_STB_BWD, K_MEFC_WGRAD, K_MEFC_FOLD, K_MEFC_FOLD_BWD, K_MEFC_HEAD, K_MEFC_HEAD_BWD,
-  K_MEFC_EW, K_DK_GATE_FWD, K_DK_GATE_BWD_DZ, K_DK_GATE_BWD_DX, K_DK_PAIR, K_DK_PAIR_WGRAD, K_DK_FOLD, K_DK_FOLD_BWD, K_COUNT
+  K_MEFC_EW, K_DK_GATE_FWD, K_DK_GATE_BWD_DZ, K_DK_GATE_BWD_DX, K_DK_PAIR, K_DK_PAIR_WGRAD, K_DK_FOLD, K_DK_FOLD_BWD, K_DY_ONCE, K_COUNT
 };
 struct ProfScope {
   hipStream_t st; int kid; bool on;
diff --git a/image_restoration_amd/csrc/dyonce.hip b/image_restoration_amd/csrc/dyonce.hip
--- /dev/null
+++ b/image_restoration_amd/csrc/dyonce.hip
@@ -0,0 +1,321 @@
+#include <limits.h>
+#include <stdlib.h>
+
+#include "internal.h"
+#include "fused_common.h"
+
+namespace mi {
+namespace {
+using namespace fz;
+
+constexpr int DY_PS = 72;
+
+struct DyArgs {
+  const bf16* s; int64_t s_bs;
+  const bf16* r; int64_t r_bs;
+  const float* wf; int64_t wf_sr, wf_sk;
+  const bf16* wb; int64_t wb_bs, wb_ld;
+  bf16* o; int64_t o_bs;
+  float* part;
+  int Mr; unsigned N;
+  int tpi, ntiles, wpi, B;
+  int stream_st;
+};
+
+template <int KS, int NW, int F>
+__global__ __launch_bounds__(64 * NW) void dy_once_kernel(DyArgs a) {
+  constexpr int CT = KS / 16, KST = (KS + 31) / 32, SROWS = 32 * KST, PS = DY_PS;
+  constexpr int SBUF = SROWS * PS, NT = 64 * NW, CH = KS * 8, SLD = (CH + NT - 1) / NT;
+  __shared__ __attribute__((aligned(16))) bf16 Sl[2 * SBUF];
+  __shared__ __attribute__((aligned(16))) bf16 Pl[NW * 16 * PS];
+  const int t = threadIdx.x, lane = t & 63, li = lane & 15, g = lane >> 4;
+  const int wv = __builtin_amdgcn_readfirstlane(t >> 6);
+  const int row0 = wv * 16 * F;
+  const bool active = row0 < a.Mr;
+  bf16* const patch = Pl + wv * 16 * PS;
+  const u32x4 zero4 = {0u, 0u, 0u, 0u};
+
+  int tile, stride, end, pslot;
+  if (a.wpi) {
+    const int b = blockIdx.x / a.wpi, j = blockIdx.x - b * a.wpi;
+    tile = b * a.tpi + j; stride = a.wpi; end = (b + 1) * a.tpi; pslot = j * a.B + b;
+  } else {
+    tile = blockIdx.x; stride = gridDim.x; end = a.ntiles; pslot = blockIdx.x;
+  }
+
+  s16x8 wt[F][KST];
+  {
+    const int wimg = a.wpi ? blockIdx.x / a.wpi : 0;
+#pragma unroll
+    for (int f = 0; f < F; ++f)
+#pragma unroll
+      for (int ks = 0; ks < KST; ++ks)
+#pragma unroll
+        for (int j = 0; j < 8; ++j) {
+          const int k = 32 * ks + (j < 4 ? 4 * g + j : 16 + 4 * g + j - 4), r = row0 + 16 * f + li;
+          const bool ok = r < a.Mr && k < KS;
+          short v = 0;
+          if (ok) {
+            if (a.wb) v = (short)reinterpret_cast<const u16*>(a.wb)[wimg * a.wb_bs + r * a.wb_ld + k];
+            else v = bf_bits(a.wf[r * a.wf_sr + k * a.wf_sk]);
+          }
+          wt[f][ks][j] = v;
+        }
+  }
+  if (SROWS > KS) {
+    for (int i = t; i < 2 * (SROWS - KS) * 8; i += NT) {
+      const int bsel = i / ((SROWS - KS) * 8), e = i - bsel * (SROWS - KS) * 8;
+      *reinterpret_cast<u32x4*>(&Sl[bsel * SBUF + (KS + (e >> 3)) * PS + 8 * (e & 7)]) = zero4;
+    }
+  }
+
+  f32x4 G[F][CT];
+#pragma unroll
+  for (int f = 0; f < F; ++f)
+#pragma unroll
+    for (int ct = 0; ct < CT; ++ct) G[f][ct] = (f32x4){0.f, 0.f, 0.f, 0.f};
+
+  u32x4 sreg[SLD], rr[F][2];
+  auto s_request = [&](int tl) {
+    const int b = tl / a.tpi, p0 = (tl - b * a.tpi) * 64;
+    const bf16* sb = a.s + b * a.s_bs + p0;
+    int tt = t;
+    asm volatile("" : "+v"(tt));
+#pragma unroll
+    for (int i = 0; i < SLD; ++i) {
+      const int idx = tt + NT * i;
+      if (idx < CH) sreg[i] = *reinterpret_cast<const u32x4*>(sb + (unsigned)(idx >> 3) * a.N + 8u * (idx & 7));
+    }
+  };
+  auto s_commit = [&](int buf) {
+    int tt = t;
+    asm volatile("" : "+v"(tt));
+#pragma unroll
+    for (int i = 0; i < SLD; ++i) {
+      const int idx = tt + NT * i;
+      if (idx < CH) *reinterpret_cast<u32x4*>(&Sl[buf * SBUF + (idx >> 3) * PS + 8 * (idx & 7)]) = sreg[i];
+    }
+  };
+  auto r_request = [&](int tl) {
+    const int b = tl / a.tpi, p0 = (tl - b * a.tpi) * 64;
+    const bf16* rb = a.r + b * a.r_bs + p0;
+    int ln = lane;
+    asm volatile("" : "+v"(ln));
+#pragma unroll
+    for (int f = 0; f < F; ++f) {
+      const int r = min(row0 + 16 * f + (ln & 15), a.Mr - 1);
+      const u32x4* q = reinterpret_cast<const u32x4*>(rb + (unsigned)r * a.N + 8u * (ln >> 4));
+      rr[f][0] = q[0];
+      rr[f][1] = q[4];
+    }
+  };
+
+  if (tile < end) {
+    s_request(tile);
+    if (active) r_request(tile);
+    s_commit(0);
+  }
+  __syncthreads();
+  int buf = 0;
+  for (; tile < end; tile += stride, buf ^= 1) {
+    const int nxt = tile + stride;
+    const int b = tile / a.tpi, p0 = (tile - b * a.tpi) * 64;
+    const bf16* const Sb = Sl + buf * SBUF;
+    if (nxt < end) s_request(nxt);
+    if (active) {
+      int ln = lane;
+      asm volatile("" : "+v"(ln));
+      const int li_ = ln & 15, g_ = ln >> 4;
+#pragma unroll
+      for (int h = 0; h < 2; ++h) {
+        const bf16* bp = Sb + li_ * PS + 32 * h + 8 * g_;
+#pragma unroll
+        for (int ct = 0; ct < CT; ++ct) {
+          const s16x8 Bv = *reinterpret_cast<const s16x8*>(bp + 16 * ct * PS);
+#pragma unroll
+          for (int f = 0; f < F; ++f) G[f][ct] = mfma32(__builtin_bit_cast(s16x8, rr[f][h]), Bv, G[f][ct]);
+        }
+      }
+      if (nxt < end) r_request(nxt);
+      const bf16* tr0 = Sb + (4 * g_ + (li_ >> 2)) * PS + 4 * (li_ & 3);
+      const int e_row = ln >> 3, e_col = (ln & 7) * 8;
+      bf16* const ob = a.o + b * a.o_bs + p0 + e_col;
+#pragma unroll
+      for (int f = 0; f < F; ++f) {
+        if (row0 + 16 * f < a.Mr) {
+          f32x4 d[4];
+#pragma unroll
+          for (int nt = 0; nt < 4; ++nt) d[nt] = (f32x4){0.f, 0.f, 0.f, 0.f};
+#pragma unroll
+          for (int ks = 0; ks < KST; ++ks) {
+            s16x4 lo[4], hi[4];
+#pragma unroll
+            for (int nt = 0; nt < 4; ++nt) {
+              lo[nt] = tr_b16(tr0 + (32 * ks) * PS + 16 * nt);
+              hi[nt] = tr_b16(tr0 + (32 * ks + 16) * PS + 16 * nt);
+            }
+            lds_wait(lo[0], hi[0], lo[1], hi[1], lo[2], hi[2], lo[3], hi[3]);
+#pragma unroll
+            for (int nt = 0; nt < 4; ++nt) d[nt] = mfma32(cat8(lo[nt], hi[nt]), wt[f][ks], d[nt]);
+          }
+#pragma unroll
+          for (int nt = 0; nt < 4; ++nt)
+            *reinterpret_cast<u32x2*>(&patch[li_ * PS + 16 * nt + 4 * g_]) =
+                (u32x2){cvt_pk_bf16(d[nt][0], d[nt][1]), cvt_pk_bf16(d[nt][2], d[nt][3])};
+          wave_sync();
+#pragma unroll
+          for (int it = 0; it < 2; ++it) {
+            const int row = row0 + 16 * f + 8 * it + e_row;
+            const u32x4 v = *reinterpret_cast<const u32x4*>(&patch[(8 * it + e_row) * PS + e_col]);
+            if (row < a.Mr) {
+              u32x4* dst = reinterpret_cast<u32x4*>(ob + (unsigned)row * a.N);
+              if (a.stream_st) MI_STREAM_ST(dst, v);
+              else *dst = v;
+            }
+          }
+          wave_sync();
+        }
+      }
+    }
+    if (nxt < end) s_commit(buf ^ 1);
+    __syncthreads();
+  }
+
+  if (active) {
+    float* const gp = a.part + (int64_t)pslot * KS * a.Mr;
+#pragma unroll
+    for (int f = 0; f < F; ++f)
+#pragma unroll
+      for (int ct = 0; ct < CT; ++ct)
+#pragma unroll
+        for (int q = 0; q < 4; ++q) {
+          const int r = row0 + 16 * f + 4 * g + q;
+          if (r < a.Mr) gp[(16 * ct + li) * a.Mr + r] = G[f][ct][q];
+        }
+  }
+}
+
+struct DyForm { int max_mr, nw, f; };
+const DyForm DY_FORMS[] = {{48, 3, 1}, {96, 6, 1}, {128, 8, 1}, {256, 8, 2}};
+
+using DyFn = void (*)(DyArgs);
+struct DyInst { int ks, nw, f; DyFn fn; };
+const DyInst DY_TABLE[] = {
+    {48, 3, 1, dy_once_kernel<48, 3, 1>}, {48, 6, 1, dy_once_kernel<48, 6, 1>}, {48, 8, 1, dy_once_kernel<48, 8, 1>},
+    {48, 8, 2, dy_once_kernel<48, 8, 2>}, {96, 3, 1, dy_once_kernel<96, 3, 1>}, {96, 6, 1, dy_once_kernel<96, 6, 1>},
+    {96, 8, 1, dy_once_kernel<96, 8, 1>}, {96, 8, 2, dy_once_kernel<96, 8, 2>}};
+}
+
+DyOncePlan dy_once_plan(int Mr, int Ks, int B, int64_t N, int dtype, int per_image) {
+  DyOncePlan p = {};
+  if (!(dtype == MI_BF16 && (Ks == 48 || Ks == 96) && Mr >= 16 && Mr <= 256 && B > 0 && N > 0 && N % 64 == 0)) return p;
+  if ((int64_t)Mr * N >= (1ll << 31) || (int64_t)Ks * N >= (1ll << 31) || (int64_t)B * (N / 64) > INT_MAX) return p;
+  for (const DyForm& f : DY_FORMS)
+    if (Mr <= f.max_mr) { p.NW = f.nw; p.F = f.f; break; }
+  p.covered = true;
+  p.pays = true;
+  p.Ks = Ks; p.Mr = Mr; p.rows = 16 * p.F; p.mpad = p.rows * p.NW;
+  p.active = (Mr + p.rows - 1) / p.rows;
+  p.per_image = per_image ? 1 : 0;
+  p.tiles_per_image = N / 64;
+  p.tiles = (int64_t)B * p.tiles_per_image;
+  const int target = p.F == 2 ? 256 : (p.NW == 3 ? 1024 : 512);
+  if (p.per_image) {
+    int64_t wpi = target / B;
+    wpi = wpi < 1 ? 1 : (wpi > p.tiles_per_image ? p.tiles_per_image : wpi);
+    p.wpi = (int)wpi;
+    p.grid = B * p.wpi;
+    p.passes = (int)((p.tiles_per_image + p.wpi - 1) / p.wpi);
+    p.part_rows = p.wpi;
+  } else {
+    p.wpi = 0;
+    p.grid = (int)(p.tiles < target ? p.tiles : target);
+    p.passes = (int)((p.tiles + p.grid - 1) / p.grid);
+    p.part_rows = p.grid;
+  }
+  const int kst = (Ks + 31) / 32;
+  p.lds = (size_t)(2 * 32 * kst + 16 * p.NW) * DY_PS * 2;
+  const size_t per = (size_t)Ks * Mr * (p.per_image ? B : 1);
+  p.part_bytes = align_up((size_t)p.part_rows * per * 4, 256);
+  p.ws_bytes = p.part_bytes + (reduce_rows_two_stage(p.part_rows) ? align_up((size_t)REDUCE_GROUPS * per * 4, 256) : 0);
+  return p;
+}
+
+static int dy_once_check(const mi_dy_once_desc* d) {
+  MI_CHECK_ARG(d, "dy_once: null descriptor");
+  MI_CHECK_ARG(d->mr > 0 && d->ks > 0 && d->n > 0 && d->batch > 0, "dy_once: bad shape");
+  MI_CHECK_ARG(d->dtype == MI_F32 || d->dtype == MI_BF16, "dy_once: bad dtype %d", d->dtype);
+  return MI_OK;
+}
+static bool dy_once_aligned(const mi_dy_once_desc* d) {
+  return aligned16(d->s) && aligned16(d->r) && aligned16(d->o) && d->s_bs % 8 == 0 && d->r_bs % 8 == 0 && d->o_bs % 8 == 0;
+}
+
+}
+
+using namespace mi;
+
+extern "C" int mi_dy_once_ok(const mi_dy_once_desc* d) {
+  if (!d || d->mr <= 0 || d->ks <= 0 || d->n <= 0 || d->batch <= 0) return 0;
+  return dy_once_plan(d->mr, d->ks, d->batch, d->n, d->dtype, d->per_image).covered && dy_once_aligned(d) ? 1 : 0;
+}
+extern "C" size_t mi_dy_once_workspace(const mi_dy_once_desc* d) {
+  if (!d || d->mr <= 0 || d->ks <= 0 || d->n <= 0 || d->batch <= 0) return 0;
+  return dy_once_plan(d->mr, d->ks, d->batch, d->n, d->dtype, d->per_image).ws_bytes;
+}
+extern "C" int mi_dy_once_plan(const mi_dy_once_desc* d, int64_t* out) {
+  MI_TRY(dy_once_check(d));
+  MI_CHECK_ARG(out, "dy_once_plan: null pointer");
+  const DyOncePlan p = dy_once_plan(d->mr, d->ks, d->batch, d->n, d->dtype, d->per_image);
+  const int64_t v[16] = {p.covered, p.pays, p.NW, p.F, p.rows, p.mpad, p.active, p.per_image, p.wpi, p.grid, p.tiles, p.passes,
+                         p.part_rows, (int64_t)p.lds, (int64_t)p.part_bytes, (int64_t)p.ws_bytes};
+  memcpy(out, v, sizeof(v));
+  return MI_OK;
+}
+extern "C" int mi_dy_once_instances(int* out, int cap) {
+  int n = 0;
+  for (const DyInst& e : DY_TABLE) {
+    if (out && n < cap) { out[3 * n] = e.ks; out[3 * n + 1] = e.nw; out[3 * n + 2] = e.f; }
+    ++n;
+  }
+  return n;
+}
+
+extern "C" int mi_dy_once(const mi_dy_once_desc* d, void* ws, void* stream) {
+  MI_TRY(dy_once_check(d));
+  hipStream_t st = (hipStream_t)stream;
+  const DyOncePlan p = dy_once_plan(d->mr, d->ks, d->batch, d->n, d->dtype, d->per_image);
+  MI_CHECK_ARG(p.covered, "dy_once: not covered (bf16, Ks 48 / 96, 16 <= Mr <= 256, N %% 64 == 0): Mr=%d Ks=%d N=%lld", d->mr, d->ks,
+               (long long)d->n);
+  MI_CHECK_ARG(d->s && d->r && d->o && d->g && ws, "dy_once: null pointer");
+  MI_CHECK_ARG(dy_once_aligned(d), "dy_once: operands and batch strides must be 16-byte aligned");
+  MI_CHECK_ARG(p.per_image ? d->w_b16 != nullptr : d->w != nullptr, "dy_once: %s", p.per_image ? "per-image mode needs w_b16" : "shared mode needs w");
+  DyFn fn = nullptr;
+  for (const DyInst& e : DY_TABLE)
+    if (e.ks == p.Ks && e.nw == p.NW && e.f == p.F) fn = e.fn;
+  MI_CHECK_ARG(fn, "dy_once: no kernel for Ks=%d with %d waves x %d fragments", p.Ks, p.NW, p.F);
+  const int64_t per = (int64_t)p.Ks * p.Mr * (p.per_image ? d->batch : 1);
+  float* part = (float*)ws;
+  float* tmp = reduce_rows_two_stage(p.part_rows) ? (float*)((char*)ws + p.part_bytes) : nullptr;
+  const int acc = p.per_image ? 0 : d->accumulate;
+  if (acc) {
+    float* arena = deferred_take((size_t)p.part_rows * per, st);
+    if (arena) part = arena;
+  }
+  DyArgs a;
+  a.s = (const bf16*)d->s; a.s_bs = d->s_bs;
+  a.r = (const bf16*)d->r; a.r_bs = d->r_bs;
+  a.wf = p.per_image ? nullptr : d->w; a.wf_sr = d->w_sr; a.wf_sk = d->w_sk;
+  a.wb = p.per_image ? (const bf16*)d->w_b16 : nullptr; a.wb_bs = d->w_b16_bs; a.wb_ld = d->w_b16_ld;
+  a.o = (bf16*)d->o; a.o_bs = d->o_bs;
+  a.part = part; a.Mr = p.Mr; a.N = (unsigned)d->n;
+  a.tpi = (int)p.tiles_per_image; a.ntiles = (int)p.tiles; a.wpi = p.wpi; a.B = d->batch;
+  a.stream_st = d->n >= 128;
+  {
+    const double px = (double)d->batch * d->n;
+    ProfScope ps(st, K_DY_ONCE, (p.Ks + 2.0 * p.Mr) * px * 2 + 4.0 * p.part_rows * per, 4.0 * p.Mr * p.Ks * px);
+    hipLaunchKernelGGL(fn, dim3(p.grid), dim3(64 * p.NW), 0, st, a);
+  }
+  MI_LAUNCH_CHECK();
+  return launch_reduce_rows(part, d->g, p.part_rows, per, per, acc, 1.0f, st, tmp);
+}
diff --git a/image_restoration_amd/csrc/internal.h b/image_restoration_amd/csrc/internal.h
--- a/image_restoration_amd/csrc/internal.h
+++ b/image_restoration_amd/csrc/internal.h
@@ -129,6 +129,16 @@
 int launch_bwd_tail(const void* dy, int M, const void* x, int C, const void* dres, const float* mean, const float* rstd,
                     const float* w, const float* gamma, const float* beta, void* dx, float* dw, float* dgamma, float* dbeta,
                     int B, int64_t N, int accumulate, void* ws, hipStream_t st);
+struct DyOncePlan {
+  bool covered, pays;
+  int Ks, Mr, NW, F, rows, mpad;
+  int active;
+  int per_image, wpi, grid;
+  int64_t tiles_per_image, tiles;
+  int passes, part_rows;
+  size_t lds, part_bytes, ws_bytes;
+};
+DyOncePlan dy_once_plan(int Mr, int Ks, int B, int64_t N, int dtype, int per_image);
 #define MI_HIDDEN __attribute__((visibility("hidden")))
 MI_HIDDEN int pw_lds_tm(int M);
 MI_HIDDEN size_t pw_lds_lds_bytes(int tm);
diff --git a/image_restoration_amd/csrc/modules.hip b/image_restoration_amd/csrc/modules.hip
--- a/image_restoration_amd/csrc/modules.hip
+++ b/image_restoration_amd/csrc/modules.hip
@@ -50,9 +50,32 @@
   const int joined = co_join(sd, st);
   return rc != MI_OK ? rc : joined;
 }
+static mi_dy_once_desc dy_once_desc(const void* dy, int Ks, int64_t dy_bs, const void* x, int Mr, int64_t x_bs, void* dx, int64_t dx_bs,
+                                    float* g, int B, int64_t N, int dtype, int per_image, int accumulate) {
+  mi_dy_once_desc d;
+  memset(&d, 0, sizeof(d));
+  d.s = dy; d.s_bs = dy_bs ? dy_bs : (int64_t)Ks * N; d.ks = Ks;
+  d.r = x; d.r_bs = x_bs ? x_bs : (int64_t)Mr * N; d.mr = Mr;
+  d.o = dx; d.o_bs = dx_bs ? dx_bs : (int64_t)Mr * N;
+  d.g = g; d.n = N; d.batch = B; d.dtype = dtype; d.per_image = per_image; d.accumulate = accumulate;
+  return d;
+}
+static bool dy_once_use(const mi_dy_once_desc& d) {
+  const char* off = MI_ENV(MI_NO_DY_ONCE);
+  if (off && atoi(off) != 0) return false;
+  const DyOncePlan p = dy_once_plan(d.mr, d.ks, d.batch, d.n, d.dtype, d.per_image);
+  return p.covered && p.pays && mi_dy_once_ok(&d);
+}
+static size_t dy_once_ws_bytes(int Mr, int Ks, int B, int64_t N, int dtype, int per_image) {
+  return dy_once_plan(Mr, Ks, B, N, dtype, per_image).ws_bytes;
+}
+
 static int conv1x1_bwd_output(const void* dy, int M, const void* x, int K, const float* w, float* dw, float* db, void* dx, int B,
                               int64_t N, int dtype, int accumulate, void* gram_ws, void* cs_ws, void* pw_ws, hipStream_t st) {
   if (db) MI_TRY(launch_chan_sum(dy, db, B, M, N, dtype, accumulate, cs_ws, st));
+  mi_dy_once_desc o = dy_once_desc(dy, M, 0, x, K, 0, dx, 0, dw, B, N, dtype, 0, accumulate);
+  o.w = w; o.w_sr = 1; o.w_sk = K;
+  if (dy_once_use(o)) return mi_dy_once(&o, gram_ws, st);
   const mi_gram_desc g = wgrad_gram(dy, M, x, K, B, N, dtype, dw, accumulate);
   MI_TRY(mi_gram(&g, gram_ws, st));
   const mi_pw_desc d = conv1x1(dy, M, w, true, K, nullptr, nullptr, dx, K, B, N, dtype);
@@ -132,7 +155,8 @@
 static const QkvView PROBE_QKV{PROBE_PTR, 0, PROBE_PTR, 0, PROBE_PTR, 0};
 static size_t attn_gram_ws_bytes(const AttnDims& d) {
   float* const p = (float*)PROBE_PTR;
-  return max_of({gram_ws_bytes(attn_qk_gram(d, PROBE_QKV, p, p)), gram_ws_bytes(attn_dm_gram(d, PROBE_PTR, PROBE_QKV, p))});
+  return max_of({gram_ws_bytes(attn_qk_gram(d, PROBE_QKV, p, p)), gram_ws_bytes(attn_dm_gram(d, PROBE_PTR, PROBE_QKV, p)),
+                 dy_once_ws_bytes(d.C, d.C, d.B, d.N, d.dtype, 1)});
 }
 static size_t attn_pw_ws_bytes(const AttnDims& d) {
   const float* const p = (const float*)PROBE_PTR;
@@ -166,8 +190,15 @@
   hipStream_t st = (hipStream_t)stream;
   const int B = d.B, C = d.C, hd = d.heads;
   if (g_proj_b) MI_TRY(launch_chan_sum(dout, g_proj_b, B, C, d.N, d.dtype, acc, w.cs_ws, st));
-  mi_gram_desc g1 = attn_dm_gram(d, dout, v, w.dM);
-  MI_TRY(mi_gram(&g1, w.gram_ws, stream));
+  mi_dy_once_desc once = dy_once_desc(dout, C, 0, v.v, C, v.v_bs, dv, dv_bs, w.dM, B, d.N, d.dtype, 1, 0);
+  once.w_b16 = sv.Mtb; once.w_b16_bs = (int64_t)C * C; once.w_b16_ld = C;
+  const bool dy_once = dy_once_use(once);
+  if (dy_once) {
+    MI_TRY(mi_dy_once(&once, w.gram_ws, stream));
+  } else {
+    mi_gram_desc g1 = attn_dm_gram(d, dout, v, w.dM);
+    MI_TRY(mi_gram(&g1, w.gram_ws, stream));
+  }
   float* dwo_part = w.dwo_part;
   float* dtemp_part = w.dtemp_part;
   if (acc) {
@@ -196,6 +227,7 @@
     dd = attn_dqk_desc(d, v, w.wd, c, c, dk, dk_bs, w.wdb);
     MI_TRY(mi_pw_gemm(&dd, w.pw_ws, stream));
   }
+  if (dy_once) return MI_OK;
   mi_pw_desc dvd = per_image(conv1x1(dout, C, sv.M, true, C, nullptr, nullptr, dv, C, B, d.N, d.dtype, 0, dv_bs), sv.Mtb);
   return mi_pw_gemm(&dvd, w.pw_ws, stream);
 }
@@ -320,7 +352,8 @@
   const int64_t N = (int64_t)s->H * s->W;
   Carver cv(base);
   GdfnWs w;
-  w.gram_ws = cv.take(max_of({gram_ws_bytes(probe_wgrad(C, h, B, N, dt)), gram_ws_bytes(probe_wgrad(2 * h, C, B, N, dt))}));
+  w.gram_ws = cv.take(max_of({gram_ws_bytes(probe_wgrad(C, h, B, N, dt)), gram_ws_bytes(probe_wgrad(2 * h, C, B, N, dt)),
+                              dy_once_ws_bytes(h, C, B, N, dt, 0)}));
   w.pw_ws = cv.take(max_of({pw_ws_bytes(probe1x1(C, 2 * h, false, B, N, dt)), pw_ws_bytes(probe1x1(2 * h, C, true, B, N, dt))}));
   w.dw_ws = cv.take(mi_dwconv_bwd_workspace(B, 2 * h, s->H, s->W, s->ks));
   w.cs_ws = cv.take(chan_sum_workspace(2 * h > C ? 2 * h : C, N));
@@ -727,7 +760,8 @@
   const int64_t N = (int64_t)s->H * s->W;
   Carver cv(base);
   MsfnWs w;
-  w.gram_ws = cv.take(max_of({gram_ws_bytes(probe_wgrad(C, h2, B, N, dt)), gram_ws_bytes(probe_wgrad(h2, C, B, N, dt))}));
+  w.gram_ws = cv.take(max_of({gram_ws_bytes(probe_wgrad(C, h2, B, N, dt)), gram_ws_bytes(probe_wgrad(h2, C, B, N, dt)),
+                              dy_once_ws_bytes(h2, C, B, N, dt, 0)}));
   w.pw_ws = cv.take(max_of({pw_ws_bytes(probe1x1(C, h2, false, B, N, dt)), pw_ws_bytes(probe1x1(h2, C, false, B, N, dt)),
                             pw_ws_bytes(probe1x1(C, h2, true, B, N, dt)), pw_ws_bytes(probe1x1(h2, C, true, B, N, dt))}));
   w.cs_ws = cv.take(chan_sum_workspace(h2 > C ? h2 : C, N));
diff --git a/image_restoration_amd/csrc/util.hip b/image_restoration_amd/csrc/util.hip
--- a/image_restoration_amd/csrc/util.hip
+++ b/image_restoration_amd/csrc/util.hip
@@ -52,7 +52,7 @@
     "msfn_stencil1_bwd", "msfn_stencil2_bwd", "mefc_stencil_a", "mefc_stencil_b", "mefc_stencil_a_bwd", "mefc_stencil_b_bwd",
     "mefc_dw_wgrad", "mefc_fold", "mefc_fold_bwd", "mefc_head", "mefc_head_bwd", "mefc_ewise",
     "darkir_dilgate_fwd", "darkir_dilgate_bwd_dz", "darkir_dilgate_bwd_dx", "darkir_pairconv", "darkir_pairconv_wgrad", "darkir_fold",
-    "darkir_fold_bwd"};
+    "darkir_fold_bwd", "dy_once"};
 
 ProfScope::ProfScope(hipStream_t stream, int kernel_id, double bytes, double flops)
     : st(stream), kid(kernel_id), on(g_prof_on.load(std::memory_order_relaxed) != 0) {
diff --git a/image_restoration_amd/ops.py b/image_restoration_amd/ops.py
--- a/image_restoration_amd/ops.py
+++ b/image_restoration_amd/ops.py
@@ -334,6 +334,82 @@
     return (out, ss) if want_sumsq else out
 
 
+DY_ONCE_PLAN_FIELDS = ("covered", "pays", "waves", "fragments", "rows_per_wave", "mpad", "active_waves", "per_image",
+                       "workgroups_per_image", "workgroups", "tiles", "passes", "part_rows", "lds", "part_bytes", "workspace")
+
+
+def dy_once_probe(Mr: int, Ks: int, N: int, dtype: torch.dtype, B: int = 1, per_image: bool = False, accumulate: bool = False,
+                  misalign: int = 0) -> "L.DyOnceDesc":
+    d = L.DyOnceDesc()
+    d.s, d.s_bs, d.ks = PW_PROBE + misalign, Ks * N, Ks
+    d.r, d.r_bs, d.mr = PW_PROBE, Mr * N, Mr
+    d.o, d.o_bs, d.g = PW_PROBE, Mr * N, PW_PROBE
+    if per_image:
+        d.w_b16, d.w_b16_bs, d.w_b16_ld = PW_PROBE, Mr * Ks, Ks
+    else:
+        d.w, d.w_sr, d.w_sk = PW_PROBE, Ks, 1
+    d.n, d.batch, d.dtype, d.per_image, d.accumulate = N, B, _dtype_code(dtype), int(per_image), int(accumulate)
+    return d
+
+
+def dy_once_plan(d: "L.DyOnceDesc") -> dict:
+    out = (L.c_i64 * 16)()
+    L.check(L.lib().mi_dy_once_plan(C.byref(d), out), "dy_once_plan")
+    p = dict(zip(DY_ONCE_PLAN_FIELDS, out))
+    for k in ("covered", "pays", "per_image"):
+        p[k] = bool(p[k])
+    return p
+
+
+def dy_once_instances() -> set:
+    n = L.lib().mi_dy_once_instances(None, 0)
+    buf = (C.c_int * (3 * n))()
+    L.lib().mi_dy_once_instances(buf, n)
+    return {(buf[3 * i], buf[3 * i + 1], buf[3 * i + 2]) for i in range(n)}
+
+
+def _plane_view(t: Tensor, what: str) -> int:
+    B, Cc, H, W = t.shape
+    if t.stride(3) != 1 or t.stride(2) != W or t.stride(1) != H * W:
+        raise RuntimeError(f"dy_once: {what} must be an NCHW tensor or a channel slice of one")
+    return t.stride(0)
+
+
+def dy_once(s: Tensor, r: Tensor, wt: Tensor, o: Optional[Tensor] = None, g: Optional[Tensor] = None, per_image: bool = False,
+            accumulate: bool = False):
+    B, Ks, H, W = s.shape
+    Mr = r.shape[1]
+    if o is None:
+        o = torch.empty((B, Mr, H, W), dtype=s.dtype, device=s.device)
+    gshape = (B, Ks, Mr) if per_image else (Ks, Mr)
+    if g is None:
+        if accumulate:
+            raise ValueError("dy_once: accumulate needs the output buffer")
+        g = torch.empty(gshape, dtype=torch.float32, device=s.device)
+    elif g.dtype != torch.float32 or tuple(g.shape) != gshape or not g.is_contiguous():
+        raise ValueError(f"dy_once: g must be a dense float32 {gshape}")
+    d = L.DyOnceDesc()
+    d.s, d.s_bs, d.ks = _p(s), _plane_view(s, "s"), Ks
+    d.r, d.r_bs, d.mr = _p(r), _plane_view(r, "r"), Mr
+    d.o, d.o_bs, d.g = _p(o), _plane_view(o, "o"), _p(g)
+    if per_image:
+        if wt.dtype != torch.bfloat16 or tuple(wt.shape) != (B, Mr, Ks) or wt.stride(2) != 1:
+            raise ValueError("dy_once: per-image weights must be bfloat16 [B, Mr, Ks] with unit inner stride")
+        d.w_b16, d.w_b16_bs, d.w_b16_ld = _p(wt), wt.stride(0), wt.stride(1)
+    else:
+        _f32(wt, "dy_once weights")
+        if tuple(wt.shape) != (Mr, Ks):
+            raise ValueError("dy_once: shared weights must be [Mr, Ks]")
+        d.w, d.w_sr, d.w_sk = _p(wt), wt.stride(0), wt.stride(1)
+    d.n, d.batch, d.dtype, d.per_image, d.accumulate = H * W, B, _dt(s), int(per_image), int(accumulate)
+    lib = L.lib()
+    if not lib.mi_dy_once_ok(C.byref(d)):
+        raise RuntimeError("dy_once: not covered (bf16, Ks 48 / 96, 16 <= Mr <= 256, H*W % 64 == 0, 16-byte aligned slices)")
+    ws = _ws(lib.mi_dy_once_workspace(C.byref(d)), s.device)
+    L.check(lib.mi_dy_once(C.byref(d), _p(ws), _stream()), "dy_once")
+    return o, g
+
+
 def conv1x1_dgrad_panel(dy: Tensor, w2: Tensor, k0: int, k: int) -> Tensor:
     B, M, H, W = dy.shape
     N = H * W
diff --git a/include/mi_restore.h b/include/mi_restore.h
--- a/include/mi_restore.h
+++ b/include/mi_restore.h
@@ -298,6 +298,20 @@
 int mi_bwd_tail(const void* dy, int M, const void* x, int C, const void* dres, const float* mean, const float* rstd,
                 const float* w, const float* gamma, const float* beta, void* dx, float* dw, float* dgamma, float* dbeta,
                 int B, int64_t N, int accumulate, int dtype, void* ws, void* stream);
+typedef struct {
+  const void* s; int64_t s_bs; int ks;
+  const void* r; int64_t r_bs; int mr;
+  const float* w; int64_t w_sr, w_sk;
+  const void* w_b16; int64_t w_b16_bs, w_b16_ld;
+  void* o; int64_t o_bs;
+  float* g;
+  int64_t n; int batch; int dtype; int per_image; int accumulate;
+} mi_dy_once_desc;
+int mi_dy_once_ok(const mi_dy_once_desc* d);
+size_t mi_dy_once_workspace(const mi_dy_once_desc* d);
+int mi_dy_once_plan(const mi_dy_once_desc* d, int64_t* out);
+int mi_dy_once_instances(int* out, int cap);
+int mi_dy_once(const mi_dy_once_desc* d, void* ws, void* stream);
 int mi_mdta_bwd_ln_ok(const mi_mdta_shape* s, int qkv_bias);
 size_t mi_mdta_bwd_ln_workspace(const mi_mdta_shape* s);
 int mi_mdta_bwd_ln(const mi_mdta_shape* s, const mi_mdta_params* p, const mi_ln_tail* ln, const void* x, const void* dout,
```

Result: no change. 16.05 Mpixels/s (median of 6 runs) (+0.8%).
